# hila-chefer/Transformer-Explainability

Measured on AMD Instinct MI355X. Metric: relevance maps/sec (ViT-B/16 224^2, batch 64 per GPU, generate_LRP transformer_attribution), higher is better.
Workload: dtype f32 (3xbf16 split operands, 6 products, fp32 accumulate)

## Files before the change

### include/te_relprop.h

```cpp
#ifndef TE_RELPROP_H
#define TE_RELPROP_H

#include <stddef.h>
#include <stdint.h>

#ifdef __cplusplus
extern "C" {
#endif

typedef void* te_stream_t;
typedef uint16_t te_bf16_t;

enum {
  TE_OK = 0,
  TE_ERR_INVALID_ARG = -1,
  TE_ERR_WORKSPACE = -2,
  TE_ERR_UNSUPPORTED = -3,
  TE_ERR_NO_DEVICE = -4
};

enum { TE_VARIANT_OURS = 0, TE_VARIANT_LRP = 1, TE_IMPL_SIMPLE = 0x100 };

enum { TE_ROLLOUT_NORMALISE = 1, TE_ROLLOUT_CLS_FIXUP = 2, TE_ROLLOUT_ROW0 = 4 };

// ... 64 lines not shown
                                        const float* q, int64_t q_sb, int64_t q_sh, int64_t q_sn,
                                        const float* k, int64_t k_sb, int64_t k_sh, int64_t k_sn,
                                        const float* Z,
                                        float* cam_q, int64_t cq_sb, int64_t cq_sh, int64_t cq_sn,
                                        float* cam_k, int64_t ck_sb, int64_t ck_sh, int64_t ck_sn,
                                        int64_t B, int64_t H, int64_t N, int64_t D, float out_scale, int variant,
                                        void* ws, size_t ws_bytes, te_stream_t stream);
int te_matmul_relprop_qk_f32(const float* R_nn,
                             const float* q, int64_t q_sb, int64_t q_sh, int64_t q_sn,
                             const float* k, int64_t k_sb, int64_t k_sh, int64_t k_sn,
                             float* cam_q, int64_t cq_sb, int64_t cq_sh, int64_t cq_sn,
                             float* cam_k, int64_t ck_sb, int64_t ck_sh, int64_t ck_sn,
                             int64_t B, int64_t H, int64_t N, int64_t D, float out_scale, int variant,
                             void* ws, size_t ws_bytes, te_stream_t stream);

size_t te_add_relprop_workspace_bytes(int64_t B, int64_t n);
int te_add_relprop_f32(const float* R, const float* X0, const float* X1, float* out0, float* out1,
                       int64_t B, int64_t n, int64_t x1_batch_stride, int variant,
                       void* ws, size_t ws_bytes, te_stream_t stream);

size_t te_add_relprop_deferred_workspace_bytes(int64_t B, int64_t n);
int te_add_relprop_deferred_f32(const float* R, const float* X0, const float* X1, float* a, float* b, float* fac,
                                int64_t B, int64_t n, int64_t x1_batch_stride,
                                void* ws, size_t ws_bytes, te_stream_t stream);

size_t te_add_bcast_relprop_workspace_bytes(int64_t B, int64_t H, int64_t N);
int te_add_bcast_relprop_f32(const float* R, const float* X0, const float* mask, float* out0,
                             float* out1, int64_t B, int64_t H, int64_t N, int variant,
                             void* ws, size_t ws_bytes, te_stream_t stream);

int te_add_bcast_relprop_deferred_f32(const float* R, const float* X0, const float* mask, float* a, float* out1,
                                      float* fac, int64_t B, int64_t H, int64_t N,
                                      void* ws, size_t ws_bytes, te_stream_t stream);

int te_clone_relprop_f32(const float* R0, const float* R1, const float* R2, const float* X,
                         float* out, int64_t n, te_stream_t stream);

int te_clone_relprop_scaled_f32(const float* R0, const float* s0, int64_t s0_stride,
                                const float* R1, const float* s1, int64_t s1_stride,
                                const float* R2, const float* s2, int64_t s2_stride,
                                const float* X, float* out, int64_t B, int64_t n, te_stream_t stream);

int te_index_select_relprop_f32(const float* R, const float* X, float* out,
                                int64_t B, int64_t N, int64_t C, int64_t index, te_stream_t stream);

int te_gradcam_headmean_f32(const float* grad, const float* cam, float* out,
                            int64_t B, int64_t H, int64_t N, te_stream_t stream);

size_t te_rollout_workspace_bytes(int64_t L, int64_t B, int64_t N);
size_t te_rollout_row0_workspace_bytes(int64_t B, int64_t N);
int te_rollout_f32(const float* cams, int64_t L, int64_t start_layer, int64_t B, int64_t N,
                   int flags, float* joint, void* ws, size_t ws_bytes, te_stream_t stream);

#define TE_X6_TILE_AUTO 0
#define TE_X6_TILE_128 1
#define TE_X6_TILE_256 2
#define TE_X6_TILE_128x128 3
#define TE_X6_TEST_DROP_HANDOVER 0x200
#define TE_X6_WHOLE_TILES 0x10000
#define TE_X6_TEST_SMALL_GRID 0x4000
#define TE_X6_TILE_Z_SHIFT 10
#define TE_X6_TILE_C_SHIFT 12
#define TE_X6_PHASE_SPLIT 4
#define TE_X6_PHASE_Z 8
#define TE_X6_PHASE_C 16
#define TE_X6_PHASE_MASK 28
int te_linear_relprop_x6_supported(int64_t T, int64_t in_f, int64_t out_f);
size_t te_linear_relprop_x6_workspace_bytes(int64_t T, int64_t in_f, int64_t out_f);
size_t te_linear_x6_weight_planes_bytes(int64_t in_f, int64_t out_f);
size_t te_linear_x6_planes_bytes(int64_t rows, int64_t K);
int te_linear_x6_prepare_weights_f32(const float* W, int64_t in_f, int64_t out_f, void* planes, size_t planes_bytes,
                                     te_stream_t stream);
int te_linear_x6_split_abs_f32(const float* X, int64_t rows, int64_t K, void* planes, size_t planes_bytes,
                               te_stream_t stream);
int te_linear_relprop_x6_f32(const float* R, const float* r_scale, int64_t r_scale_stride, int64_t rows_per_sample,
                             const float* X, const float* W, const void* w_planes, const void* x_planes,
                             const float* Y, const float* bias, float* out,
                             int64_t T, int64_t in_f, int64_t out_f, int flags, unsigned* status, void* ws,
                             size_t ws_bytes, te_stream_t stream);
int te_linear_relprop_x6_check(const void* ws, int64_t T, int64_t in_f, int64_t out_f, te_stream_t stream);

int te_linear_relprop_x6_general_supported(int64_t T, int64_t in_f, int64_t out_f, int variant);
size_t te_linear_x6_weight_planes_lrp_bytes(int64_t in_f, int64_t out_f);
int te_linear_x6_prepare_weights_lrp_f32(const float* W, int64_t in_f, int64_t out_f, void* planes, size_t planes_bytes,
                                         te_stream_t stream);
size_t te_linear_relprop_x6_general_workspace_bytes(int64_t T, int64_t in_f, int64_t out_f, int variant);
int te_linear_relprop_x6_general_f32(const float* R, const float* r_scale, int64_t r_scale_stride, int64_t rows_per_sample,
                                     const float* X, const float* W, const void* w_planes, const void* w_planes_lrp,
                                     const void* x_abs_planes, const float* Y, const float* bias, float* out,
                                     int64_t T, int64_t in_f, int64_t out_f, float alpha, int variant, int flags,
                                     unsigned* status, void* ws, size_t ws_bytes, te_stream_t stream);

int te_gemm_x6_supported(int64_t T, int64_t K, int64_t M);
size_t te_gemm_x6_workspace_bytes(int64_t T, int64_t K, int64_t M);
int te_linear_x6_split_matrix_f32(const float* A, int64_t rows, int64_t K, int transposed, void* planes,
                                  size_t planes_bytes, te_stream_t stream);
int te_gemm_x6_f32(const float* X, const void* x_planes, const void* w_planes, const float* bias, float* out,
                   int64_t T, int64_t K, int64_t M, int flags, unsigned* status, void* ws, size_t ws_bytes,
                   te_stream_t stream);
int te_linear_x6_split_dual_f32(const float* A, int64_t rows, int64_t K, void* planes, void* planes_abs,
                                size_t planes_bytes, te_stream_t stream);
int te_gelu_backward_x6_planes_f32(const float* dy, const float* x, int64_t rows, int64_t K, void* planes,
                                   size_t planes_bytes, te_stream_t stream);
int te_gelu_forward_x6_planes_f32(const float* x, float* y, int64_t rows, int64_t K, void* planes, void* planes_abs,
                                  size_t planes_bytes, te_stream_t stream);

int te_attention_forward_supported(int64_t N, int64_t D);
int te_attention_forward_f32(const float* qkv, float* z_qk, float* attn, float* out,
                             int64_t B, int64_t H, int64_t N, int64_t D, float scale, te_stream_t stream);
int te_attention_forward_planes_f32(const float* qkv, float* z_qk, float* attn, float* out, void* out_planes,
                                    void* out_abs_planes, size_t planes_bytes, int64_t B, int64_t H, int64_t N, int64_t D,
                                    float scale, te_stream_t stream);
int te_attention_backward_f32(const float* d_out, const float* qkv, const float* attn, float* d_attn, float* d_qkv,
                              int64_t B, int64_t H, int64_t N, int64_t D, float scale, int need_qk, te_stream_t stream);
int te_attention_backward_out_f32(const float* d_out, const float* out, const float* qkv, const float* attn, float* d_attn,
                                  float* d_qkv, int64_t B, int64_t H, int64_t N, int64_t D, float scale, int need_qk,
                                  te_stream_t stream);

int te_attention_strided_supported(int64_t N, int64_t D);
size_t te_attention_backward_strided_workspace_bytes(int64_t B, int64_t H, int64_t N);
int te_attention_forward_strided_f32(const float* q, int64_t q_sb, int64_t q_sh, int64_t q_sn,
                                     const float* k, int64_t k_sb, int64_t k_sh, int64_t k_sn,
                                     const float* v, int64_t v_sb, int64_t v_sh, int64_t v_sn,
                                     const float* mask, float* z_qk, float* x_scaled, float* attn,
                                     float* out, int64_t o_sb, int64_t o_sh, int64_t o_sn,
                                     int64_t B, int64_t H, int64_t N, int64_t D, float scale, te_stream_t stream);
int te_attention_backward_strided_f32(const float* d_out, int64_t do_sb, int64_t do_sh, int64_t do_sn,
                                      const float* q, int64_t q_sb, int64_t q_sh, int64_t q_sn,
                                      const float* k, int64_t k_sb, int64_t k_sh, int64_t k_sn,
                                      const float* v, int64_t v_sb, int64_t v_sh, int64_t v_sn,
                                      const float* attn, float* d_attn,
                                      float* d_q, int64_t dq_sb, int64_t dq_sh, int64_t dq_sn,
                                      float* d_k, int64_t dk_sb, int64_t dk_sh, int64_t dk_sn,
                                      float* d_v, int64_t dv_sb, int64_t dv_sh, int64_t dv_sn,
                                      int64_t B, int64_t H, int64_t N, int64_t D, float scale, int need_qk,
                                      void* ws, size_t ws_bytes, te_stream_t stream);
int te_attention_backward_strided_out_f32(const float* d_out, int64_t do_sb, int64_t do_sh, int64_t do_sn,
                                          const float* out, int64_t o_sb, int64_t o_sh, int64_t o_sn,
                                          const float* q, int64_t q_sb, int64_t q_sh, int64_t q_sn,
                                          const float* k, int64_t k_sb, int64_t k_sh, int64_t k_sn,
                                          const float* v, int64_t v_sb, int64_t v_sh, int64_t v_sn,
                                          const float* attn, float* d_attn,
                                          float* d_q, int64_t dq_sb, int64_t dq_sh, int64_t dq_sn,
                                          float* d_k, int64_t dk_sb, int64_t dk_sh, int64_t dk_sn,
                                          float* d_v, int64_t dv_sb, int64_t dv_sh, int64_t dv_sn,
                                          int64_t B, int64_t H, int64_t N, int64_t D, float scale, int need_qk,
                                          void* ws, size_t ws_bytes, te_stream_t stream);

int te_layernorm_supported(int64_t C);
int te_layernorm_forward_f32(const float* x, const float* weight, const float* bias, float* y, float* mean, float* rstd,
                             int64_t T, int64_t C, float eps, te_stream_t stream);
int te_layernorm_backward_f32(const float* dy, const float* x, const float* weight, const float* mean, const float* rstd,
                              const float* add, float* dx, int64_t T, int64_t C, te_stream_t stream);
int te_gelu_forward_f32(const float* x, float* y, int64_t n, te_stream_t stream);
int te_gelu_backward_f32(const float* dy, const float* x, float* dx, int64_t n, te_stream_t stream);

int te_heatmap_f32(const float* maps, float* heat, float* fg_mask, int64_t B, int64_t g, int64_t scale,
                   int normalise, te_stream_t stream);

size_t te_seg_metrics_workspace_bytes(int64_t B, int64_t H, int64_t W);
int te_seg_metrics_f32(const float* heat, const float* fg_mask, const int64_t* labels, int64_t* counts, double* ap,
                       double* f1, int64_t B, int64_t H, int64_t W, void* ws, size_t ws_bytes, te_stream_t stream);

#define TE_RATIONALE_MAX_KS 16
#define TE_RATIONALE_CLAMP 1
size_t te_rationale_metrics_workspace_bytes(int64_t B, int64_t N, int64_t Wmax);
int te_rationale_metrics_f32(const float* scores, const int32_t* word_ids, const uint8_t* truth, float* word_scores,
                             int32_t* n_words, int32_t* order, int32_t* counts, double* soft, int64_t B, int64_t N,
                             int64_t Wmax, const int64_t* ks, int64_t n_ks, int flags, void* ws, size_t ws_bytes,
                             te_stream_t stream);

#define TE_TOKEN_ERASE_MAX_FRACTIONS 8
int te_token_erase(const int64_t* input_ids, const int64_t* attention_mask, const int32_t* word_ids,
                   const int32_t* order, const int32_t* n_words, int64_t* ids_out, int64_t* mask_out,
                   int32_t* n_rationale, int64_t B, int64_t N, int64_t Wmax, const double* fractions, int64_t n_t,
                   int64_t pad_id, te_stream_t stream);

size_t te_conv2d_zb_relprop_workspace_bytes(int64_t B, int64_t C, int64_t H, int64_t W, int64_t E, int64_t p);
int te_conv2d_zb_relprop_f32(const float* R, int64_t r_bs, const float* X, const float* W, const float* Y,
                             const float* bias, float* out, int64_t B, int64_t C, int64_t H, int64_t W_, int64_t E,
                             int64_t p, int flags, void* ws, size_t ws_bytes, te_stream_t stream);

#define TE_PERTURB_MAX_STEPS 16
#define TE_PERTURB_MAX_CHANNELS 4
size_t te_perturb_workspace_bytes(int64_t B, int64_t n_steps);
int te_perturb_f32(const float* vis, const float* data, float* out, int64_t B, int64_t C, int64_t HW,
                   const int64_t* ks, int64_t n_steps, const float* mean, const float* std_, void* ws,
                   size_t ws_bytes, te_stream_t stream);

int te_linear_relprop_bf16_supported(int64_t T, int64_t in_f, int64_t out_f);
size_t te_linear_relprop_bf16_workspace_bytes(int64_t T, int64_t in_f, int64_t out_f);
size_t te_linear_bf16_weight_planes_bytes(int64_t in_f, int64_t out_f);
int te_linear_bf16_prepare_weights(const te_bf16_t* W, int64_t in_f, int64_t out_f, void* planes, size_t planes_bytes,
                                   te_stream_t stream);
int te_linear_relprop_bf16(const float* R, int64_t r_ld, const float* r_scale, int64_t r_scale_stride,
                           int64_t rows_per_scale, const te_bf16_t* X, int64_t x_ld, const void* w_planes, float* out,
                           int64_t T, int64_t in_f, int64_t out_f, void* ws, size_t ws_bytes, te_stream_t stream);
int te_matmul_relprop_bf16_supported(int64_t N, int64_t D);
size_t te_matmul_relprop_av_bf16_workspace_bytes(int64_t B, int64_t H, int64_t N, int64_t D);
size_t te_matmul_relprop_qk_bf16_workspace_bytes(int64_t B, int64_t H, int64_t N, int64_t D);
int te_matmul_relprop_av_bf16(const float* R, int64_t r_sb, int64_t r_sh, int64_t r_sn,
                              const te_bf16_t* attn,
                              const te_bf16_t* v, int64_t v_sb, int64_t v_sh, int64_t v_sn,
                              const te_bf16_t* Z, int64_t z_sb, int64_t z_sh, int64_t z_sn,
                              float* cam_attn,
                              float* cam_v, int64_t cv_sb, int64_t cv_sh, int64_t cv_sn,
                              int64_t B, int64_t H, int64_t N, int64_t D, float out_scale, int variant,
                              void* ws, size_t ws_bytes, te_stream_t stream);
int te_matmul_relprop_qk_bf16(const float* R_nn, const float* r_scale, int64_t r_scale_stride,
                              const te_bf16_t* q, int64_t q_sb, int64_t q_sh, int64_t q_sn,
                              const te_bf16_t* k, int64_t k_sb, int64_t k_sh, int64_t k_sn,
                              const te_bf16_t* Z,
                              float* cam_q, int64_t cq_sb, int64_t cq_sh, int64_t cq_sn,
                              float* cam_k, int64_t ck_sb, int64_t ck_sh, int64_t ck_sn,
                              int64_t B, int64_t H, int64_t N, int64_t D, float out_scale, int variant,
                              void* ws, size_t ws_bytes, te_stream_t stream);
int te_add_relprop_bf16(const float* R, const te_bf16_t* X0, const te_bf16_t* X1, float* out0, float* out1, int64_t B,
                        int64_t n, int64_t x1_batch_stride, int variant, void* ws, size_t ws_bytes, te_stream_t stream);
int te_add_relprop_deferred_bf16(const float* R, const te_bf16_t* X0, const te_bf16_t* X1, float* a, float* b,
                                 float* fac, int64_t B, int64_t n, int64_t x1_batch_stride, void* ws, size_t ws_bytes,
                                 te_stream_t stream);
int te_add_bcast_relprop_bf16(const float* R, const te_bf16_t* X0, const te_bf16_t* mask, float* out0, float* out1,
                              int64_t B, int64_t H, int64_t N, int variant, void* ws, size_t ws_bytes,
                              te_stream_t stream);
int te_add_bcast_relprop_deferred_bf16(const float* R, const te_bf16_t* X0, const te_bf16_t* mask, float* a,
                                       float* out1, float* fac, int64_t B, int64_t H, int64_t N, void* ws,
                                       size_t ws_bytes, te_stream_t stream);
int te_clone_relprop_bf16(const float* R0, const float* R1, const float* R2, const te_bf16_t* X, float* out, int64_t n,
                          te_stream_t stream);
int te_clone_relprop_scaled_bf16(const float* R0, const float* s0, int64_t s0_stride, const float* R1, const float* s1,
                                 int64_t s1_stride, const float* R2, const float* s2, int64_t s2_stride,
                                 const te_bf16_t* X, float* out, int64_t B, int64_t n, te_stream_t stream);
int te_index_select_relprop_bf16(const float* R, const te_bf16_t* X, float* out, int64_t B, int64_t N, int64_t C,
                                 int64_t index, te_stream_t stream);
int te_gradcam_headmean_bf16(const te_bf16_t* grad, const float* cam, float* out, int64_t B, int64_t H, int64_t N,
                             te_stream_t stream);
enum { TE_HEADMEAN_CLAMP = 1, TE_HEADMEAN_ROW0 = 2 };
int te_attn_headmean_bf16(const te_bf16_t* attn, int64_t a_sb, int64_t a_sh, float* out, int64_t B, int64_t H, int64_t N,
                          int flags, te_stream_t stream);
int te_perturb_bf16(const float* vis, const float* data, te_bf16_t* out, int64_t B, int64_t C, int64_t HW,
                    const int64_t* ks, int64_t n_steps, const float* mean, const float* std_, void* ws,
                    size_t ws_bytes, te_stream_t stream);
int te_attention_bf16_supported(int64_t N, int64_t D);
size_t te_attention_backward_strided_bf16_workspace_bytes(int64_t B, int64_t H, int64_t N);
int te_attention_forward_strided_bf16(const te_bf16_t* q, int64_t q_sb, int64_t q_sh, int64_t q_sn,
                                      const te_bf16_t* k, int64_t k_sb, int64_t k_sh, int64_t k_sn,
                                      const te_bf16_t* v, int64_t v_sb, int64_t v_sh, int64_t v_sn,
                                      const te_bf16_t* mask, te_bf16_t* z_qk, te_bf16_t* x_scaled, te_bf16_t* attn,
                                      te_bf16_t* out, int64_t o_sb, int64_t o_sh, int64_t o_sn,
                                      int64_t B, int64_t H, int64_t N, int64_t D, float scale, te_stream_t stream);
int te_attention_backward_strided_bf16(const te_bf16_t* d_out, int64_t do_sb, int64_t do_sh, int64_t do_sn,
                                       const te_bf16_t* q, int64_t q_sb, int64_t q_sh, int64_t q_sn,
                                       const te_bf16_t* k, int64_t k_sb, int64_t k_sh, int64_t k_sn,
                                       const te_bf16_t* v, int64_t v_sb, int64_t v_sh, int64_t v_sn,
                                       const te_bf16_t* attn, te_bf16_t* d_attn,
                                       te_bf16_t* d_q, int64_t dq_sb, int64_t dq_sh, int64_t dq_sn,
                                       te_bf16_t* d_k, int64_t dk_sb, int64_t dk_sh, int64_t dk_sn,
                                       te_bf16_t* d_v, int64_t dv_sb, int64_t dv_sh, int64_t dv_sn,
                                       int64_t B, int64_t H, int64_t N, int64_t D, float scale, int need_qk,
                                       void* ws, size_t ws_bytes, te_stream_t stream);
int te_conv2d_zb_relprop_bf16_supported(int64_t C, int64_t E, int64_t p);
size_t te_conv2d_zb_relprop_bf16_workspace_bytes(int64_t B, int64_t C, int64_t H, int64_t W, int64_t E, int64_t p);
size_t te_conv2d_zb_bf16_weight_planes_bytes(int64_t C, int64_t E, int64_t p);
int te_conv2d_zb_bf16_prepare_weights(const te_bf16_t* W, int64_t C, int64_t E, int64_t p, void* planes,
                                      size_t planes_bytes, te_stream_t stream);
int te_conv2d_zb_relprop_bf16(const float* R, int64_t r_bs, const te_bf16_t* X, const te_bf16_t* W, const void* w_planes,
                              float* out, int64_t B, int64_t C, int64_t H, int64_t W_, int64_t E, int64_t p, void* ws,
                              size_t ws_bytes, te_stream_t stream);

size_t te_linear_relprop_f64_workspace_bytes(int64_t T, int64_t in_f, int64_t out_f);
int te_linear_relprop_f64(const double* R, int64_t r_ld, const double* X, int64_t x_ld, const double* W, int64_t w_ld,
                          double* out, int64_t T, int64_t in_f, int64_t out_f, void* ws, size_t ws_bytes,
                          te_stream_t stream);
size_t te_matmul_relprop_av_f64_workspace_bytes(int64_t B, int64_t H, int64_t N, int64_t D);
size_t te_matmul_relprop_qk_f64_workspace_bytes(int64_t B, int64_t H, int64_t N, int64_t D);
int te_matmul_relprop_av_f64(const double* R, int64_t r_sb, int64_t r_sh, int64_t r_sn, const double* attn,
                             const double* v, int64_t v_sb, int64_t v_sh, int64_t v_sn,
                             const double* Z, int64_t z_sb, int64_t z_sh, int64_t z_sn,
                             double* cam_attn, double* cam_v, int64_t cv_sb, int64_t cv_sh, int64_t cv_sn,
                             int64_t B, int64_t H, int64_t N, int64_t D, double out_scale,
                             void* ws, size_t ws_bytes, te_stream_t stream);
int te_matmul_relprop_qk_f64(const double* R, const double* q, int64_t q_sb, int64_t q_sh, int64_t q_sn,
                             const double* k, int64_t k_sb, int64_t k_sh, int64_t k_sn, const double* Z,
                             double* cam_q, int64_t cq_sb, int64_t cq_sh, int64_t cq_sn,
                             double* cam_k, int64_t ck_sb, int64_t ck_sh, int64_t ck_sn,
                             int64_t B, int64_t H, int64_t N, int64_t D, double out_scale,
                             void* ws, size_t ws_bytes, te_stream_t stream);
size_t te_add_relprop_f64_workspace_bytes(int64_t B, int64_t n);
int te_add_relprop_f64(const double* R, const double* X0, const double* X1, double* out0, double* out1, int64_t B,
                       int64_t n, int64_t x1_batch_stride, void* ws, size_t ws_bytes, te_stream_t stream);
size_t te_add_bcast_relprop_f64_workspace_bytes(int64_t B, int64_t H, int64_t N);
int te_add_bcast_relprop_f64(const double* R, const double* X0, const double* mask, int64_t mask_batch_stride,
                             double* out0, double* out1, int64_t B, int64_t H, int64_t N, void* ws, size_t ws_bytes,
                             te_stream_t stream);
int te_clone_relprop_f64(const double* R0, const double* R1, const double* R2, const double* X, double* out, int64_t n,
                         te_stream_t stream);
int te_index_select_relprop_f64(const double* R, const double* X, double* out, int64_t B, int64_t N, int64_t C,
                                int64_t index, te_stream_t stream);
int te_gradcam_headmean_f64(const double* grad, const double* cam, double* out, int64_t B, int64_t H, int64_t N,
                            te_stream_t stream);

#ifdef __cplusplus
}
#endif
#endif
```

### transformer-explainability_amd/_lib.py

```python
from __future__ import annotations

import ctypes
import os
from ctypes import c_char_p, c_double, c_float, c_int, c_int64, c_size_t, c_void_p

import torch

_PKG = os.path.dirname(os.path.abspath(__file__))
LIB_PATH = os.environ.get("TE_RELPROP_LIB") or os.path.join(_PKG, "lib", "libte_relprop.so")

TE_OK = 0
MIN_LIB_VERSION = 700
TE_ERR_UNSUPPORTED = -3
TE_VARIANT_OURS = 0
TE_VARIANT_LRP = 1
TE_IMPL_SIMPLE = 0x100
TE_ROLLOUT_NORMALISE = 1
TE_ROLLOUT_CLS_FIXUP = 2
TE_ROLLOUT_ROW0 = 4
TE_HEADMEAN_CLAMP = 1
TE_HEADMEAN_ROW0 = 2
TE_RATIONALE_CLAMP = 1
TE_RATIONALE_MAX_KS = 16
TE_TOKEN_ERASE_MAX_FRACTIONS = 8

_P, _I64, _F, _I, _SZ, _D = c_void_p, c_int64, c_float, c_int, c_size_t, c_double

SIGNATURES = {
    "te_version": (_I, []),
    "te_status_string": (c_char_p, [_I]),
    "te_device_check": (_I, []),
    "te_build_id": (c_char_p, []),
    "te_linear_relprop_workspace_bytes": (_SZ, [_I64, _I64, _I64, _I]),
    "te_linear_relprop_f32": (_I, [_P, _P, _P, _P, _I64, _I64, _I64, _F, _I, _P, _SZ, _P]),
    "te_linear_zpass_f32": (_I, [_P, _P, _P, _P, _I64, _I64, _I64, _P]),
    "te_linear_cpass_f32": (_I, [_P, _P, _P, _P, _I64, _I64, _I64, _P]),
    "te_linear_zpass_fwd_f32": (_I, [_P, _P, _P, _P, _P, _P, _I64, _I64, _I64, _P]),
    "te_linear_relprop_fwd_f32": (_I, [_P, _P, _P, _P, _P, _P, _I64, _I64, _I64, _P, _SZ, _P]),
    "te_linear_zpass_fwd_scaled_f32": (_I, [_P, _P, _I64, _I64, _P, _P, _P, _P, _P, _I64, _I64, _I64, _P]),
    "te_linear_relprop_fwd_scaled_f32": (_I, [_P, _P, _I64, _I64, _P, _P, _P, _P, _P, _I64, _I64, _I64, _P, _SZ, _P]),
    "te_matmul_relprop_av_workspace_bytes": (_SZ, [_I64, _I64, _I64, _I64]),
    "te_matmul_relprop_av_f32": (_I, [_P, _I64, _I64, _I64, _P, _P, _I64, _I64, _I64, _P, _P, _I64, _I64, _I64,
                                      _I64, _I64, _I64, _I64, _F, _I, _P, _SZ, _P]),
    "te_matmul_relprop_qk_workspace_bytes": (_SZ, [_I64, _I64, _I64, _I64]),
    "te_matmul_relprop_av_fwd_f32": (_I, [_P, _I64, _I64, _I64, _P, _P, _I64, _I64, _I64, _P, _P, _P, _I64, _I64, _I64,
                                          _I64, _I64, _I64, _I64, _F, _I, _P, _SZ, _P]),
    "te_matmul_relprop_av_fwdz_f32": (_I, [_P, _I64, _I64, _I64, _P, _P, _I64, _I64, _I64, _P, _I64, _I64, _I64, _P, _P,
                                           _I64, _I64, _I64, _I64, _I64, _I64, _I64, _F, _I, _P, _SZ, _P]),
    "te_attention_forward_supported": (_I, [_I64, _I64]),
    "te_attention_forward_f32": (_I, [_P, _P, _P, _P, _I64, _I64, _I64, _I64, _F, _P]),
    "te_attention_forward_planes_f32": (_I, [_P, _P, _P, _P, _P, _P, _SZ, _I64, _I64, _I64, _I64, _F, _P]),
    "te_attention_backward_f32": (_I, [_P, _P, _P, _P, _P, _I64, _I64, _I64, _I64, _F, _I, _P]),
    "te_attention_backward_out_f32": (_I, [_P, _P, _P, _P, _P, _P, _I64, _I64, _I64, _I64, _F, _I, _P]),
    "te_attention_strided_supported": (_I, [_I64, _I64]),
    "te_attention_backward_strided_workspace_bytes": (_SZ, [_I64, _I64, _I64]),
    "te_attention_forward_strided_f32": (_I, [_P, _I64, _I64, _I64, _P, _I64, _I64, _I64, _P, _I64, _I64, _I64, _P, _P, _P,
                                              _P, _P, _I64, _I64, _I64, _I64, _I64, _I64, _I64, _F, _P]),
    "te_attention_backward_strided_f32": (_I, [_P, _I64, _I64, _I64, _P, _I64, _I64, _I64, _P, _I64, _I64, _I64, _P, _I64,
                                               _I64, _I64, _P, _P, _P, _I64, _I64, _I64, _P, _I64, _I64, _I64, _P, _I64,
                                               _I64, _I64, _I64, _I64, _I64, _I64, _F, _I, _P, _SZ, _P]),
    "te_attention_backward_strided_out_f32": (_I, [_P, _I64, _I64, _I64, _P, _I64, _I64, _I64, _P, _I64, _I64, _I64, _P, _I64, _I64, _I64,
                                                   _P, _I64, _I64, _I64, _P, _P, _P, _I64, _I64, _I64, _P, _I64, _I64, _I64, _P,
                                                   _I64, _I64, _I64, _I64, _I64, _I64, _I64, _F, _I, _P, _SZ, _P]),
    "te_linear_relprop_x6_supported": (_I, [_I64, _I64, _I64]),
    "te_linear_relprop_x6_workspace_bytes": (_SZ, [_I64, _I64, _I64]),
    "te_linear_x6_weight_planes_bytes": (_SZ, [_I64, _I64]),
    "te_linear_x6_planes_bytes": (_SZ, [_I64, _I64]),
    "te_linear_x6_prepare_weights_f32": (_I, [_P, _I64, _I64, _P, _SZ, _P]),
    "te_linear_x6_split_abs_f32": (_I, [_P, _I64, _I64, _P, _SZ, _P]),
    "te_linear_relprop_x6_f32": (_I, [_P, _P, _I64, _I64, _P, _P, _P, _P, _P, _P, _P, _I64, _I64, _I64, _I, _P, _P, _SZ,
                                      _P]),
    "te_linear_relprop_x6_check": (_I, [_P, _I64, _I64, _I64, _P]),
    "te_linear_relprop_x6_general_supported": (_I, [_I64, _I64, _I64, _I]),
    "te_linear_x6_weight_planes_lrp_bytes": (_SZ, [_I64, _I64]),
    "te_linear_x6_prepare_weights_lrp_f32": (_I, [_P, _I64, _I64, _P, _SZ, _P]),
    "te_linear_relprop_x6_general_workspace_bytes": (_SZ, [_I64, _I64, _I64, _I]),
    "te_linear_relprop_x6_general_f32": (_I, [_P, _P, _I64, _I64, _P, _P, _P, _P, _P, _P, _P, _P, _I64, _I64, _I64, _F, _I,
                                              _I, _P, _P, _SZ, _P]),
    "te_gemm_x6_supported": (_I, [_I64, _I64, _I64]),
    "te_gemm_x6_workspace_bytes": (_SZ, [_I64, _I64, _I64]),
    "te_linear_x6_split_matrix_f32": (_I, [_P, _I64, _I64, _I, _P, _SZ, _P]),
    "te_linear_x6_split_dual_f32": (_I, [_P, _I64, _I64, _P, _P, _SZ, _P]),
    "te_gemm_x6_f32": (_I, [_P, _P, _P, _P, _P, _I64, _I64, _I64, _I, _P, _P, _SZ, _P]),
    "te_layernorm_supported": (_I, [_I64]),
    "te_layernorm_forward_f32": (_I, [_P, _P, _P, _P, _P, _P, _I64, _I64, _F, _P]),
    "te_layernorm_backward_f32": (_I, [_P, _P, _P, _P, _P, _P, _P, _I64, _I64, _P]),
    "te_gelu_forward_f32": (_I, [_P, _P, _I64, _P]),
    "te_gelu_backward_f32": (_I, [_P, _P, _P, _I64, _P]),
    "te_gelu_backward_x6_planes_f32": (_I, [_P, _P, _I64, _I64, _P, _SZ, _P]),
    "te_gelu_forward_x6_planes_f32": (_I, [_P, _P, _I64, _I64, _P, _P, _SZ, _P]),
    "te_matmul_relprop_qk_fwd_f32": (_I, [_P, _P, _I64, _I64, _I64, _P, _I64, _I64, _I64, _P, _P, _I64, _I64, _I64,
                                          _P, _I64, _I64, _I64, _I64, _I64, _I64, _I64, _F, _I, _P, _SZ, _P]),
    "te_matmul_relprop_qk_fwd_scaled_f32": (_I, [_P, _P, _I64, _P, _I64, _I64, _I64, _P, _I64, _I64, _I64, _P, _P, _I64,
                                                 _I64, _I64, _P, _I64, _I64, _I64, _I64, _I64, _I64, _I64, _F, _I, _P,
                                                 _SZ, _P]),
    "te_matmul_relprop_qk_f32": (_I, [_P, _P, _I64, _I64, _I64, _P, _I64, _I64, _I64, _P, _I64, _I64, _I64,
                                      _P, _I64, _I64, _I64, _I64, _I64, _I64, _I64, _F, _I, _P, _SZ, _P]),
    "te_add_relprop_workspace_bytes": (_SZ, [_I64, _I64]),
    "te_add_relprop_f32": (_I, [_P, _P, _P, _P, _P, _I64, _I64, _I64, _I, _P, _SZ, _P]),
    "te_add_relprop_deferred_workspace_bytes": (_SZ, [_I64, _I64]),
    "te_add_relprop_deferred_f32": (_I, [_P, _P, _P, _P, _P, _P, _I64, _I64, _I64, _P, _SZ, _P]),
    "te_add_bcast_relprop_workspace_bytes": (_SZ, [_I64, _I64, _I64]),
    "te_add_bcast_relprop_f32": (_I, [_P, _P, _P, _P, _P, _I64, _I64, _I64, _I, _P, _SZ, _P]),
    "te_add_bcast_relprop_deferred_f32": (_I, [_P, _P, _P, _P, _P, _P, _I64, _I64, _I64, _P, _SZ, _P]),
    "te_clone_relprop_f32": (_I, [_P, _P, _P, _P, _P, _I64, _P]),
    "te_clone_relprop_scaled_f32": (_I, [_P, _P, _I64, _P, _P, _I64, _P, _P, _I64, _P, _P, _I64, _I64, _P]),
    "te_index_select_relprop_f32": (_I, [_P, _P, _P, _I64, _I64, _I64, _I64, _P]),
    "te_gradcam_headmean_f32": (_I, [_P, _P, _P, _I64, _I64, _I64, _P]),
    "te_heatmap_f32": (_I, [_P, _P, _P, _I64, _I64, _I64, _I, _P]),
    "te_seg_metrics_workspace_bytes": (_SZ, [_I64, _I64, _I64]),
    "te_seg_metrics_f32": (_I, [_P, _P, _P, _P, _P, _P, _I64, _I64, _I64, _P, _SZ, _P]),
    "te_rationale_metrics_workspace_bytes": (_SZ, [_I64, _I64, _I64]),
    "te_rationale_metrics_f32": (_I, [_P, _P, _P, _P, _P, _P, _P, _P, _I64, _I64, _I64, _P, _I64, _I, _P, _SZ, _P]),
    "te_token_erase": (_I, [_P, _P, _P, _P, _P, _P, _P, _P, _I64, _I64, _I64, _P, _I64, _I64, _P]),
    "te_conv2d_zb_relprop_workspace_bytes": (_SZ, [_I64] * 6),
    "te_conv2d_zb_relprop_f32": (_I, [_P, _I64, _P, _P, _P, _P, _P, _I64, _I64, _I64, _I64, _I64, _I64, _I, _P, _SZ,
                                      _P]),
    "te_perturb_workspace_bytes": (_SZ, [_I64, _I64]),
    "te_perturb_f32": (_I, [_P, _P, _P, _I64, _I64, _I64, _P, _I64, _P, _P, _P, _SZ, _P]),
    "te_rollout_workspace_bytes": (_SZ, [_I64, _I64, _I64]),
    "te_rollout_row0_workspace_bytes": (_SZ, [_I64, _I64]),
    "te_rollout_f32": (_I, [_P, _I64, _I64, _I64, _I64, _I, _P, _P, _SZ, _P]),
    "te_linear_relprop_bf16_supported": (_I, [_I64, _I64, _I64]),
    "te_linear_relprop_bf16_workspace_bytes": (_SZ, [_I64, _I64, _I64]),
    "te_linear_bf16_weight_planes_bytes": (_SZ, [_I64, _I64]),
    "te_linear_bf16_prepare_weights": (_I, [_P, _I64, _I64, _P, _SZ, _P]),
    "te_linear_relprop_bf16": (_I, [_P, _I64, _P, _I64, _I64, _P, _I64, _P, _P, _I64, _I64, _I64, _P, _SZ, _P]),
    "te_matmul_relprop_bf16_supported": (_I, [_I64, _I64]),
    "te_matmul_relprop_av_bf16_workspace_bytes": (_SZ, [_I64, _I64, _I64, _I64]),
    "te_matmul_relprop_qk_bf16_workspace_bytes": (_SZ, [_I64, _I64, _I64, _I64]),
    "te_matmul_relprop_av_bf16": (_I, [_P, _I64, _I64, _I64, _P, _P, _I64, _I64, _I64, _P, _I64, _I64, _I64, _P, _P,
                                       _I64, _I64, _I64, _I64, _I64, _I64, _I64, _F, _I, _P, _SZ, _P]),
    "te_matmul_relprop_qk_bf16": (_I, [_P, _P, _I64, _P, _I64, _I64, _I64, _P, _I64, _I64, _I64, _P, _P, _I64, _I64,
                                       _I64, _P, _I64, _I64, _I64, _I64, _I64, _I64, _I64, _F, _I, _P, _SZ, _P]),
    "te_add_relprop_bf16": (_I, [_P, _P, _P, _P, _P, _I64, _I64, _I64, _I, _P, _SZ, _P]),
    "te_add_relprop_deferred_bf16": (_I, [_P, _P, _P, _P, _P, _P, _I64, _I64, _I64, _P, _SZ, _P]),
    "te_add_bcast_relprop_bf16": (_I, [_P, _P, _P, _P, _P, _I64, _I64, _I64, _I, _P, _SZ, _P]),
    "te_add_bcast_relprop_deferred_bf16": (_I, [_P, _P, _P, _P, _P, _P, _I64, _I64, _I64, _P, _SZ, _P]),
    "te_clone_relprop_bf16": (_I, [_P, _P, _P, _P, _P, _I64, _P]),
    "te_clone_relprop_scaled_bf16": (_I, [_P, _P, _I64, _P, _P, _I64, _P, _P, _I64, _P, _P, _I64, _I64, _P]),
    "te_index_select_relprop_bf16": (_I, [_P, _P, _P, _I64, _I64, _I64, _I64, _P]),
    "te_gradcam_headmean_bf16": (_I, [_P, _P, _P, _I64, _I64, _I64, _P]),
    "te_attn_headmean_bf16": (_I, [_P, _I64, _I64, _P, _I64, _I64, _I64, _I, _P]),
    "te_perturb_bf16": (_I, [_P, _P, _P, _I64, _I64, _I64, _P, _I64, _P, _P, _P, _SZ, _P]),
    "te_linear_relprop_f64_workspace_bytes": (_SZ, [_I64, _I64, _I64]),
    "te_linear_relprop_f64": (_I, [_P, _I64, _P, _I64, _P, _I64, _P, _I64, _I64, _I64, _P, _SZ, _P]),
    "te_matmul_relprop_av_f64_workspace_bytes": (_SZ, [_I64, _I64, _I64, _I64]),
    "te_matmul_relprop_qk_f64_workspace_bytes": (_SZ, [_I64, _I64, _I64, _I64]),
    "te_matmul_relprop_av_f64": (_I, [_P, _I64, _I64, _I64, _P, _P, _I64, _I64, _I64, _P, _I64, _I64, _I64, _P, _P,
                                      _I64, _I64, _I64, _I64, _I64, _I64, _I64, _D, _P, _SZ, _P]),
    "te_matmul_relprop_qk_f64": (_I, [_P, _P, _I64, _I64, _I64, _P, _I64, _I64, _I64, _P, _P, _I64, _I64, _I64, _P,
                                      _I64, _I64, _I64, _I64, _I64, _I64, _I64, _D, _P, _SZ, _P]),
    "te_add_relprop_f64_workspace_bytes": (_SZ, [_I64, _I64]),
    "te_add_relprop_f64": (_I, [_P, _P, _P, _P, _P, _I64, _I64, _I64, _P, _SZ, _P]),
    "te_add_bcast_relprop_f64_workspace_bytes": (_SZ, [_I64, _I64, _I64]),
    "te_add_bcast_relprop_f64": (_I, [_P, _P, _P, _I64, _P, _P, _I64, _I64, _I64, _P, _SZ, _P]),
    "te_clone_relprop_f64": (_I, [_P, _P, _P, _P, _P, _I64, _P]),
    "te_index_select_relprop_f64": (_I, [_P, _P, _P, _I64, _I64, _I64, _I64, _P]),
    "te_gradcam_headmean_f64": (_I, [_P, _P, _P, _I64, _I64, _I64, _P]),
    "te_conv2d_zb_relprop_bf16_supported": (_I, [_I64, _I64, _I64]),
    "te_conv2d_zb_relprop_bf16_workspace_bytes": (_SZ, [_I64] * 6),
    "te_conv2d_zb_bf16_weight_planes_bytes": (_SZ, [_I64, _I64, _I64]),
    "te_conv2d_zb_bf16_prepare_weights": (_I, [_P, _I64, _I64, _I64, _P, _SZ, _P]),
    "te_conv2d_zb_relprop_bf16": (_I, [_P, _I64, _P, _P, _P, _P, _I64, _I64, _I64, _I64, _I64, _I64, _P, _SZ, _P]),
    "te_attention_bf16_supported": (_I, [_I64, _I64]),
    "te_attention_backward_strided_bf16_workspace_bytes": (_SZ, [_I64, _I64, _I64]),
    "te_attention_forward_strided_bf16": (_I, [_P, _I64, _I64, _I64, _P, _I64, _I64, _I64, _P, _I64, _I64, _I64, _P, _P, _P,
                                               _P, _P, _I64, _I64, _I64, _I64, _I64, _I64, _I64, _F, _P]),
    "te_attention_backward_strided_bf16": (_I, [_P, _I64, _I64, _I64, _P, _I64, _I64, _I64, _P, _I64, _I64, _I64, _P, _I64,
                                                _I64, _I64, _P, _P, _P, _I64, _I64, _I64, _P, _I64, _I64, _I64, _P, _I64,
                                                _I64, _I64, _I64, _I64, _I64, _I64, _F, _I, _P, _SZ, _P]),
}


class TeError(RuntimeError):
    pass


_lib = None


def hip_runtimes_loaded():
    seen = set()
    try:
        with open("/proc/self/maps") as f:
            for line in f:
                if "libamdhip64" in line:
                    seen.add(line.split()[-1])
    except OSError:
        pass
    return sorted(seen)


def load():
    global _lib
    if _lib is not None:
        return _lib
    if not os.path.exists(LIB_PATH):
        raise TeError(
            f"{LIB_PATH} is missing: build the HIP extension first "
            f"(python transformer-explainability_amd/build.py or __graft_entry__.build()); there is no CPU fallback")
    lib = ctypes.CDLL(LIB_PATH)
    for name, (res, args) in SIGNATURES.items():
        fn = getattr(lib, name)
        fn.restype = res
        fn.argtypes = args
    if lib.te_version() < MIN_LIB_VERSION:
        raise TeError(f"{LIB_PATH} is version {lib.te_version()}, this package needs >= {MIN_LIB_VERSION}: rebuild it "
                      f"(python transformer-explainability_amd/build.py --force)")
    from ._buildid import source_hash
    bid = (lib.te_build_id() or b"").decode()
    want = source_hash()
    if bid.split("-")[0] != want and not (os.environ.get("TE_RELPROP_LIB") or os.environ.get("TE_ALLOW_STALE_LIB") == "1"):
        raise TeError(f"{LIB_PATH} was built from other sources (te_build_id() = {bid!r}, this tree hashes to {want!r}): "
                      f"rebuild it (python transformer-explainability_amd/build.py)")
    _lib = lib
    return lib


def build_id() -> str:
    return (load().te_build_id() or b"").decode()


def check(status: int, what: str):
    if status != TE_OK:
        msg = load().te_status_string(status)
        raise TeError(f"{what} failed with status {status}: {msg.decode() if msg else '?'}")


def require_device():
    if not torch.cuda.is_available():
        raise TeError("no HIP device visible to PyTorch: the relprop hot path runs only on MI355X (gfx950); "
                      "there is no CPU fallback")
    lib = load()
    rts = hip_runtimes_loaded()
    if len(rts) > 1:
        raise TeError(f"two HIP runtimes are mapped into this process: {rts}; import torch before loading "
                      f"libte_relprop so that both share torch's libamdhip64")
    check(lib.te_device_check(), "te_device_check")
# ... 1 lines not shown
```

### transformer-explainability_amd/bert.py

```python
from __future__ import annotations

import math
from types import SimpleNamespace

import torch
import torch.nn as nn

from . import ops
from . import rules as R_ours

__all__ = ["BertConfigLite", "make_bert_module", "BertModel", "BertForSequenceClassification"]


def BertConfigLite(**kw):
    d = dict(vocab_size=30522, hidden_size=768, num_hidden_layers=12, num_attention_heads=12,
             intermediate_size=3072, hidden_act="gelu", hidden_dropout_prob=0.1,
             attention_probs_dropout_prob=0.1, max_position_embeddings=512, type_vocab_size=2,
             layer_norm_eps=1e-12, pad_token_id=0, num_labels=2)
    d.update(kw)
    return SimpleNamespace(**d)


class _FusedSelfAttention(torch.autograd.Function):

    @staticmethod
    def forward(ctx, q, k, v, mask, num_heads, scale, module):
        out, attn, zqk, xsc = ops.attention_forward_qkv(q, k, v, num_heads, scale, mask=mask, want_z=True,
                                                        want_x=mask is not None)
        ctx.save_for_backward(q, k, v, attn, out)
        ctx.num_heads, ctx.scale, ctx.module = num_heads, scale, module
        if xsc is None:
            xsc = zqk.new_empty(0)
        ctx.mark_non_differentiable(attn, zqk, xsc)
        ctx.set_materialize_grads(False)
        return out, attn, zqk, xsc

    @staticmethod
    def backward(ctx, d_out, _a, _z, _x):
        q, k, v, attn, out = ctx.saved_tensors
        if d_out is None:
            return None, None, None, None, None, None, None
        stop = bool(getattr(ctx.module, "_fused_stop_backward", False))
        d_v = torch.empty_like(v)
        d_q = None if stop else torch.empty_like(q)
        d_k = None if stop else torch.empty_like(k)
        d_attn = ops.attention_backward_qkv(d_out, q, k, v, attn, ctx.num_heads, ctx.scale, d_q, d_k, d_v, need_qk=not stop, out=out)
        ctx.module.save_attn_gradients(d_attn)
        if stop:
            return None, None, None, None, None, None, None
        return d_q, d_k, d_v, None, None, None, None


def make_bert_module(L):
    ACT = {"relu": L.ReLU, "tanh": L.Tanh, "gelu": L.GELU}

    class BertEmbeddings(nn.Module):
        def __init__(self, config):
            super().__init__()
            self.word_embeddings = nn.Embedding(config.vocab_size, config.hidden_size,
                                                padding_idx=getattr(config, "pad_token_id", 0))
            self.position_embeddings = nn.Embedding(config.max_position_embeddings, config.hidden_size)
            self.token_type_embeddings = nn.Embedding(config.type_vocab_size, config.hidden_size)
            self.LayerNorm = L.LayerNorm(config.hidden_size, eps=config.layer_norm_eps)
            self.dropout = L.Dropout(config.hidden_dropout_prob)
            self.register_buffer("position_ids", torch.arange(config.max_position_embeddings).expand((1, -1)))
            self.add1 = L.Add()
            self.add2 = L.Add()

        def forward(self, input_ids=None, token_type_ids=None, position_ids=None, inputs_embeds=None):
            shape = input_ids.size() if input_ids is not None else inputs_embeds.size()[:-1]
            if position_ids is None:
                position_ids = self.position_ids[:, :shape[1]]
            if token_type_ids is None:
                token_type_ids = torch.zeros(shape, dtype=torch.long, device=self.position_ids.device)
            if inputs_embeds is None:
                inputs_embeds = self.word_embeddings(input_ids)
            pos = self.position_embeddings(position_ids).expand(shape[0], -1, -1)
            emb = self.add1([self.token_type_embeddings(token_type_ids), pos])
            emb = self.add2([emb, inputs_embeds])
            return self.dropout(self.LayerNorm(emb))

        def relprop(self, cam, **kwargs):
            return self.add2.relprop(cam, **kwargs)

    class BertSelfAttention(nn.Module):
        def __init__(self, config):
            super().__init__()
            if config.hidden_size % config.num_attention_heads != 0:
                raise ValueError("hidden size must be a multiple of the number of attention heads")
            self.num_attention_heads = config.num_attention_heads
            self.attention_head_size = config.hidden_size // config.num_attention_heads
            self.all_head_size = config.hidden_size
            self.query = L.Linear(config.hidden_size, self.all_head_size)
            self.key = L.Linear(config.hidden_size, self.all_head_size)
            self.value = L.Linear(config.hidden_size, self.all_head_size)
            self.dropout = L.Dropout(config.attention_probs_dropout_prob)
            self.matmul1 = L.MatMul()
            self.matmul2 = L.MatMul()
            self.softmax = L.Softmax(dim=-1)
            self.add = L.Add()
            self.mul = L.Mul()
            self.clone = L.Clone()
            self.head_mask = self.attention_mask = None
            self.attn_cam = self.attn = self.attn_gradients = None

        def get_attn(self): return self.attn
        def save_attn(self, attn): self.attn = attn
        def save_attn_cam(self, cam): self.attn_cam = cam
        def get_attn_cam(self): return self.attn_cam
        def save_attn_gradients(self, g): self.attn_gradients = g
        def get_attn_gradients(self): return self.attn_gradients

        def transpose_for_scores(self, x):
            return x.view(*x.shape[:-1], self.num_attention_heads, self.attention_head_size).permute(0, 2, 1, 3)

        def transpose_for_scores_relprop(self, x):
            return x.permute(0, 2, 1, 3).flatten(2)

        def forward(self, hidden_states, attention_mask=None, head_mask=None, **unused):
            if head_mask is not None:
                raise NotImplementedError("head_mask is off the accelerated path")
            self.head_mask, self.attention_mask = head_mask, attention_mask
            h1, h2, h3 = self.clone(hidden_states, 3)
            self._fused_anchor = None
            B, N, _ = hidden_states.shape
            dt = hidden_states.dtype
            if (ops.USE_FUSED_PRODUCERS and hidden_states.is_cuda and not self.training
                    and ((dt == torch.float32 and ops.attention_forward_supported(N, self.attention_head_size))
                         or (dt == torch.bfloat16 and ops.attention_forward_bf16_supported(N, self.attention_head_size)))
                    and (attention_mask is None
                         or (tuple(attention_mask.shape) == (B, 1, 1, N)
                             and (dt == torch.float32 or attention_mask.dtype == dt)))):
                return self._forward_fused(h1, h2, h3, attention_mask)
            q = self.transpose_for_scores(self.query(h1))
            k = self.transpose_for_scores(self.key(h2))
            v = self.transpose_for_scores(self.value(h3))
            scores = self.matmul1([q, k.transpose(-1, -2)]) / math.sqrt(self.attention_head_size)
            if attention_mask is not None:
                scores = self.add([scores, attention_mask])
            probs = self.softmax(scores)
            self.save_attn(probs)
            if probs.requires_grad:
                probs.register_hook(self.save_attn_gradients)
            ctx = self.matmul2([self.dropout(probs), v])
            ctx = ctx.permute(0, 2, 1, 3).contiguous()
            return (ctx.view(*ctx.shape[:-2], self.all_head_size),)

        def _forward_fused(self, h1, h2, h3, attention_mask):
            B, N, C = h1.shape
            H, D = self.num_attention_heads, self.attention_head_size
            ql, kl, vl = self.query(h1), self.key(h2), self.value(h3)
            ctx, probs, zqk, xsc = _FusedSelfAttention.apply(ql, kl, vl, attention_mask, H, 1.0 / math.sqrt(D), self)
            self._fused_anchor = ql if ql.requires_grad else None
            heads = lambda t: t.detach().view(B, N, H, D).permute(0, 2, 1, 3)
            q, k, v = heads(ql), heads(kl), heads(vl)
            self.save_attn(probs)
            caches = [(self.matmul1, [q, k.transpose(-1, -2)], zqk), (self.matmul2, [probs, v], heads(ctx))]
            if attention_mask is not None:
                caches.append((self.add, [xsc, attention_mask], None))
            for mod, X, Y in caches:
                mod.X, mod.Y = X, Y
                mod._y_version = Y._version if Y is not None else None
                mod._w_version = (None, None)
            return (ctx,)

        def relprop(self, cam, **kwargs):
            B, N, C = cam.shape
            H, D = self.num_attention_heads, self.attention_head_size
            var = self.matmul2.variant
            probs, v = self.matmul2.X
            q, kt = self.matmul1.X
            rq = torch.empty((B, N, C), dtype=cam.dtype, device=cam.device)
            rk, rv = torch.empty_like(rq), torch.empty_like(rq)
            as_heads = lambda t: t.view(B, N, H, D).permute(0, 2, 1, 3)
            cam1, _ = ops.matmul_relprop_av(as_heads(cam), probs, v, out_scale=0.5, cam_v_out=as_heads(rv), variant=var,
                                            z=R_ours._cached_y(self.matmul2))
            self.save_attn_cam(cam1)
            if getattr(self, "_stop_after_attn_cam", False):
                raise L.StopRelprop()
            if self.attention_mask is not None:
                cam1, _ = self.add.relprop(cam1, deferred=True, **kwargs)
            ops.matmul_relprop_qk(cam1, q, kt.transpose(-1, -2), out_scale=0.5, cam_q_out=as_heads(rq),
                                  cam_k_out=as_heads(rk), variant=var, z=R_ours._cached_y(self.matmul1))
            rq = self.query.relprop(rq, **kwargs)
            rk = self.key.relprop(rk, **kwargs)
            rv = self.value.relprop(rv, **kwargs)
            return self.clone.relprop((rq, rk, rv), **kwargs)

    class BertSelfOutput(nn.Module):
        def __init__(self, config):
            super().__init__()
            self.dense = L.Linear(config.hidden_size, config.hidden_size)
            self.LayerNorm = L.LayerNorm(config.hidden_size, eps=config.layer_norm_eps)
            self.dropout = L.Dropout(config.hidden_dropout_prob)
            self.add = L.Add()

        def forward(self, hidden_states, input_tensor):
            return self.LayerNorm(self.add([self.dropout(self.dense(hidden_states)), input_tensor]))

        def relprop(self, cam, **kwargs):
            cam1, cam2 = self.add.relprop(cam, deferred=True, **kwargs)
            return self.dense.relprop(cam1, **kwargs), cam2

    class BertAttention(nn.Module):
        def __init__(self, config):
            super().__init__()
            self.self = BertSelfAttention(config)
            self.output = BertSelfOutput(config)
            self.clone = L.Clone()

        def forward(self, hidden_states, attention_mask=None, head_mask=None, **unused):
            h1, h2 = self.clone(hidden_states, 2)
            return (self.output(self.self(h1, attention_mask, head_mask)[0], h2),)

        def relprop(self, cam, **kwargs):
            cam1, cam2 = self.output.relprop(cam, **kwargs)
            cam1 = self.self.relprop(cam1, **kwargs)
            return self.clone.relprop((cam1, cam2), **kwargs)

    class BertIntermediate(nn.Module):
        def __init__(self, config):
            super().__init__()
            self.dense = L.Linear(config.hidden_size, config.intermediate_size)
            act = config.hidden_act
            self.intermediate_act_fn = ACT[act]() if isinstance(act, str) else act

        def forward(self, hidden_states):
            return self.intermediate_act_fn(self.dense(hidden_states))

        def relprop(self, cam, **kwargs):
            return self.dense.relprop(cam, **kwargs)

    class BertOutput(nn.Module):
        def __init__(self, config):
            super().__init__()
            self.dense = L.Linear(config.intermediate_size, config.hidden_size)
            self.LayerNorm = L.LayerNorm(config.hidden_size, eps=config.layer_norm_eps)
            self.dropout = L.Dropout(config.hidden_dropout_prob)
            self.add = L.Add()

        def forward(self, hidden_states, input_tensor):
            return self.LayerNorm(self.add([self.dropout(self.dense(hidden_states)), input_tensor]))

        def relprop(self, cam, **kwargs):
            cam1, cam2 = self.add.relprop(cam, deferred=True, **kwargs)
            return self.dense.relprop(cam1, **kwargs), cam2

    class BertLayer(nn.Module):
        def __init__(self, config):
            super().__init__()
            self.attention = BertAttention(config)
            self.intermediate = BertIntermediate(config)
            self.output = BertOutput(config)
            self.clone = L.Clone()
            act = self.intermediate.intermediate_act_fn
            if hasattr(act, "feeds"):
                act.feeds(self.output.dense)

        def forward(self, hidden_states, attention_mask=None, head_mask=None, **unused):
            att = self.attention(hidden_states, attention_mask, head_mask)[0]
            a1, a2 = self.clone(att, 2)
            return (self.output(self.intermediate(a1), a2),)

        def relprop(self, cam, **kwargs):
            cam1, cam2 = self.output.relprop(cam, **kwargs)
            cam1 = self.intermediate.relprop(cam1, **kwargs)
            cam = self.clone.relprop((cam1, cam2), **kwargs)
            return self.attention.relprop(cam, **kwargs)

        def relprop_cls_only(self, cam_cls, **kwargs):
            alpha = kwargs.get("alpha", 1)
            var = self.clone.variant
            cls = lambda t: t[:, :1]
            dfr = ops.USE_DEFERRED_ADD
            c1, c2 = ops.add_relprop(cam_cls, cls(self.output.add.X[0]), cls(self.output.add.X[1]), variant=var,
                                     deferred=dfr)
            c1 = R_ours.linear_rule(self.output.dense, c1, alpha, cls, var)
            c1 = R_ours.linear_rule(self.intermediate.dense, c1, alpha, cls, var)
            cam = ops.clone_relprop((c1, c2), cls(self.clone.X))
            att = self.attention
            a1, a2 = ops.add_relprop(cam, cls(att.output.add.X[0]), cls(att.output.add.X[1]), variant=var, deferred=dfr)
            a1 = R_ours.linear_rule(att.output.dense, a1, alpha, cls, var)
            B, N, C = att.clone.X.shape
            dense = torch.zeros((2, B, N, C), dtype=a1.dtype, device=a1.device)
            dense[0, :, 0] = a1[:, 0]
            if isinstance(a2, ops.Deferred):
                a2 = a2.materialise()
            dense[1, :, 0] = a2[:, 0]
            cam1 = att.self.relprop(dense[0], **kwargs)
            return att.clone.relprop((cam1, dense[1]), **kwargs)

    class BertEncoder(nn.Module):
        def __init__(self, config):
            super().__init__()
            self.config = config
            self.layer = nn.ModuleList([BertLayer(config) for _ in range(config.num_hidden_layers)])

        def forward(self, hidden_states, attention_mask=None, head_mask=None, **unused):
            for i, layer in enumerate(self.layer):
                hidden_states = layer(hidden_states, attention_mask, None if head_mask is None else head_mask[i])[0]
            return (hidden_states,)

        def relprop(self, cam, **kwargs):
            for layer in reversed(self.layer):
                cam = layer.relprop(cam, **kwargs)
            return cam

    class BertPooler(nn.Module):
        def __init__(self, config):
            super().__init__()
            self.dense = L.Linear(config.hidden_size, config.hidden_size)
            self.activation = L.Tanh()
            self.pool = L.IndexSelect()
            self.register_buffer("_cls_index", torch.zeros((), dtype=torch.long), persistent=False)

        def forward(self, hidden_states):
            first = self.pool(hidden_states, 1, self._cls_index).squeeze(1)
            return self.activation(self.dense(first))

        def relprop(self, cam, **kwargs):
            cam = self.dense.relprop(cam, **kwargs)
            return self.pool.relprop(cam.unsqueeze(1), **kwargs)

    class BertModel(nn.Module):
        def __init__(self, config):
            super().__init__()
            self.config = config
            self.embeddings = BertEmbeddings(config)
            self.encoder = BertEncoder(config)
            self.pooler = BertPooler(config)

        def get_input_embeddings(self):
            return self.embeddings.word_embeddings

        def forward(self, input_ids=None, attention_mask=None, token_type_ids=None, position_ids=None,
                    head_mask=None, inputs_embeds=None, **unused):
            shape = input_ids.size() if input_ids is not None else inputs_embeds.size()[:-1]
            device = input_ids.device if input_ids is not None else inputs_embeds.device
            if attention_mask is None:
                attention_mask = torch.ones(shape, device=device)
            ext = (1.0 - attention_mask[:, None, None, :].to(next(self.parameters()).dtype)) * -10000.0
            emb = self.embeddings(input_ids=input_ids, position_ids=position_ids, token_type_ids=token_type_ids,
                                  inputs_embeds=inputs_embeds)
            seq = self.encoder(emb, attention_mask=ext, head_mask=head_mask)[0]
            return (seq, self.pooler(seq))

        exploit_cls_sparsity = True

        def relprop(self, cam, **kwargs):
            if not self.exploit_cls_sparsity:
                return self.encoder.relprop(self.pooler.relprop(cam, **kwargs), **kwargs)
            cam = self.pooler.dense.relprop(cam, **kwargs)
            cam = ops.index_select_relprop(cam.unsqueeze(1), self.pooler.pool.X[:, :1], 0)
            layers = list(self.encoder.layer)
            cam = layers[-1].relprop_cls_only(cam, **kwargs)
            for layer in reversed(layers[:-1]):
                cam = layer.relprop(cam, **kwargs)
            return cam

    class BertForSequenceClassification(nn.Module):
        def __init__(self, config):
            super().__init__()
            self.config = config
            self.num_labels = config.num_labels
            self.bert = BertModel(config)
            self.dropout = L.Dropout(config.hidden_dropout_prob)
            self.classifier = L.Linear(config.hidden_size, config.num_labels)
            self.apply(self._init_weights)

        def _init_weights(self, m):
            if isinstance(m, (nn.Linear, nn.Embedding)):
                m.weight.data.normal_(mean=0.0, std=getattr(self.config, "initializer_range", 0.02))
            elif isinstance(m, nn.LayerNorm):
                m.bias.data.zero_()
                m.weight.data.fill_(1.0)
            if isinstance(m, nn.Linear) and m.bias is not None:
                m.bias.data.zero_()

        def forward(self, input_ids=None, attention_mask=None, token_type_ids=None, position_ids=None,
                    head_mask=None, inputs_embeds=None, labels=None, **unused):
            pooled = self.bert(input_ids, attention_mask=attention_mask, token_type_ids=token_type_ids,
                               position_ids=position_ids, head_mask=head_mask, inputs_embeds=inputs_embeds)[1]
            logits = self.classifier(self.dropout(pooled))
            if labels is not None:
                if self.num_labels == 1:
                    loss = nn.functional.mse_loss(logits.view(-1), labels.view(-1))
                else:
                    loss = nn.functional.cross_entropy(logits.view(-1, self.num_labels), labels.view(-1))
                return (loss, logits)
            return (logits,)

        def relprop(self, cam=None, **kwargs):
            cam = self.classifier.relprop(cam, **kwargs)
            return self.bert.relprop(cam, **kwargs)

    return dict(BertEmbeddings=BertEmbeddings, BertSelfAttention=BertSelfAttention, BertSelfOutput=BertSelfOutput,
                BertAttention=BertAttention, BertIntermediate=BertIntermediate, BertOutput=BertOutput,
                BertLayer=BertLayer, BertEncoder=BertEncoder, BertPooler=BertPooler, BertModel=BertModel,
                BertForSequenceClassification=BertForSequenceClassification)


_ns = make_bert_module(R_ours)
BertModel = _ns["BertModel"]
BertForSequenceClassification = _ns["BertForSequenceClassification"]
```

### transformer-explainability_amd/csrc/te_linear_x6.hip

```cpp
#include <algorithm>
#include <cmath>
#include <type_traits>

#include "te_x6.h"

namespace {

constexpr int kRB = 3 * kFrag;
constexpr int kMinFrag = 4;
constexpr float kCancelTol = 0.0078125f;
constexpr int kSpinMillis = 250;
constexpr int kErrWord = 1023;


enum { MODE_Z = 0, MODE_C = 1, MODE_G = 2, MODE_ZI = 3, MODE_Z1 = 4, MODE_CI = 5, MODE_X = 6 };

__device__ __forceinline__ float bf16_f32(unsigned b) { return __uint_as_float(b << 16); }

enum { OP_ABS = 0, OP_POS = 1, OP_NEG = 2, OP_ID = 3 };
template <int OP>
__device__ __forceinline__ float apply_op(float x) {
  if constexpr (OP == OP_ID) return x;
  if constexpr (OP == OP_ABS) return __int_as_float(__float_as_int(x) & 0x7fffffff);
  const int b = __float_as_int(x);
  if constexpr (OP == OP_POS) return __int_as_float(b > 0 ? b : 0);
  return __int_as_float(b < 0 ? b : 0);
}

template <int OP, bool TRANSPOSE>
__global__ __launch_bounds__(256) void split_kernel(const float* __restrict__ src, unsigned char* __restrict__ dst,
                                                    int64_t R, int64_t K, int group, int sign,
                                                    unsigned char* __restrict__ dst_abs = nullptr) {
  const int r = threadIdx.x & 31, sl = threadIdx.x >> 5;
  const int64_t rb = blockIdx.x;
  const int64_t ks = (int64_t)blockIdx.y * 8 + sl;
  const int64_t nks = K >> 4;
  if (ks >= nks) return;
  const int64_t row = rb * 32 + r;
  float v[16];
  if (row < R) {
    if constexpr (!TRANSPOSE) {
      const float* s = src + row * K + ks * 16;
#pragma unroll
      for (int c = 0; c < 4; ++c) {
        const f32x4 q = *reinterpret_cast<const f32x4*>(s + 4 * c);
#pragma unroll
        for (int e = 0; e < 4; ++e) v[4 * c + e] = q[e];
      }
    } else {
#pragma unroll
      for (int e = 0; e < 16; ++e) v[e] = src[(ks * 16 + e) * R + row];
    }
  } else {
#pragma unroll
    for (int e = 0; e < 16; ++e) v[e] = 0.0f;
  }
  unsigned p[8][3];
#pragma unroll
  for (int e = 0; e < 8; ++e) split3_pk(apply_op<OP>(v[2 * e]), apply_op<OP>(v[2 * e + 1]), p[e]);
  unsigned char* d = dst + ((rb * nks + ks) * group + sign * 3) * kFrag + r * 16;
#pragma unroll
  for (int q = 0; q < 3; ++q)
#pragma unroll
    for (int kh = 0; kh < 2; ++kh) {
      u32x4 w;
#pragma unroll
      for (int e = 0; e < 4; ++e) w[e] = p[4 * kh + e][q];
      *reinterpret_cast<u32x4*>(d + q * kFrag + kh * 512) = w;
    }
  if constexpr (OP == OP_ID) {
    if (dst_abs) {
#pragma unroll
      for (int e = 0; e < 8; ++e) {
        const unsigned m = p[e][0] & 0x80008000u;
        p[e][0] &= 0x7fff7fffu;
        p[e][1] ^= m & (((p[e][1] & 0x7fff7fffu) + 0x7fff7fffu) & 0x80008000u);
        p[e][2] ^= m & (((p[e][2] & 0x7fff7fffu) + 0x7fff7fffu) & 0x80008000u);
      }
      unsigned char* da = dst_abs + ((rb * nks + ks) * 3) * kFrag + r * 16;
#pragma unroll
      for (int q = 0; q < 3; ++q)
#pragma unroll
        for (int kh = 0; kh < 2; ++kh) {
          u32x4 w;
#pragma unroll
          for (int e = 0; e < 4; ++e) w[e] = p[4 * kh + e][q];
          *reinterpret_cast<u32x4*>(da + q * kFrag + kh * 512) = w;
        }
    }
  }
}

enum { SRC_GELU_BWD = 0, SRC_GELU_FWD = 1 };
constexpr int kGsPitch = 132;
template <int SRC>
__global__ __launch_bounds__(256) void gelu_split_lds_kernel(const float* __restrict__ g, const float* __restrict__ x,
                                                             float* __restrict__ y, unsigned char* __restrict__ dst,
                                                             unsigned char* __restrict__ dst_abs, int64_t R, int64_t K) {
  __shared__ __attribute__((aligned(16))) float tile[32 * kGsPitch];
  const int64_t rb = blockIdx.x;
  const int64_t k0 = (int64_t)blockIdx.y * 128;
#pragma unroll
  for (int j = 0; j < 4; ++j) {
    const int i = threadIdx.x + 256 * j;
    const int tr = i >> 5, c4 = i & 31;
    const int64_t row = rb * 32 + tr, col = k0 + 4 * c4;
    f32x4 o = {0.0f, 0.0f, 0.0f, 0.0f};
    if (row < R && col < K) {
      const int64_t at = row * K + col;
      const f32x4 xv = __builtin_nontemporal_load(reinterpret_cast<const f32x4*>(x + at));
      if constexpr (SRC == SRC_GELU_BWD) {
        const f32x4 gv = __builtin_nontemporal_load(reinterpret_cast<const f32x4*>(g + at));
#pragma unroll
        for (int e = 0; e < 4; ++e) o[e] = te_gelu_grad(gv[e], xv[e]);
      } else {
#pragma unroll
        for (int e = 0; e < 4; ++e) o[e] = te_gelu(xv[e]);
        *reinterpret_cast<f32x4*>(y + at) = o;
      }
    }
    *reinterpret_cast<f32x4*>(&tile[tr * kGsPitch + 4 * c4]) = o;
  }
  __syncthreads();
  const int r = threadIdx.x & 31, sl = threadIdx.x >> 5;
  const int64_t ks = (int64_t)blockIdx.y * 8 + sl;
  const int64_t nks = K >> 4;
  if (ks >= nks) return;
  float v[16];
#pragma unroll
  for (int c = 0; c < 4; ++c) {
    const f32x4 q = *reinterpret_cast<const f32x4*>(&tile[r * kGsPitch + sl * 16 + 4 * c]);
#pragma unroll
    for (int e = 0; e < 4; ++e) v[4 * c + e] = q[e];
  }
  unsigned p[8][3];
#pragma unroll
  for (int e = 0; e < 8; ++e) split3_pk(v[2 * e], v[2 * e + 1], p[e]);
  auto store = [&](unsigned char* d) __attribute__((always_inline)) {
#pragma unroll
    for (int q = 0; q < 3; ++q)
#pragma unroll
      for (int kh = 0; kh < 2; ++kh) {
        u32x4 w;
#pragma unroll
        for (int e = 0; e < 4; ++e) w[e] = p[4 * kh + e][q];
        *reinterpret_cast<u32x4*>(d + q * kFrag + kh * 512) = w;
      }
  };
  store(dst + ((rb * nks + ks) * 3) * kFrag + r * 16);
  if constexpr (SRC == SRC_GELU_FWD) {
#pragma unroll
    for (int e = 0; e < 8; ++e) {
      const unsigned m = p[e][0] & 0x80008000u;
      p[e][0] &= 0x7fff7fffu;
      p[e][1] ^= m & (((p[e][1] & 0x7fff7fffu) + 0x7fff7fffu) & 0x80008000u);
      p[e][2] ^= m & (((p[e][2] & 0x7fff7fffu) + 0x7fff7fffu) & 0x80008000u);
    }
    store(dst_abs + ((rb * nks + ks) * 3) * kFrag + r * 16);
  }
}

__global__ __launch_bounds__(256) void zero_words_kernel(u32x4* __restrict__ p) {
  p[(size_t)blockIdx.x * 256 + threadIdx.x] = u32x4{0u, 0u, 0u, 0u};
}

__device__ __forceinline__ float exact_z(const float* __restrict__ x, const float* __restrict__ w, int64_t K) {
  float z1 = 0.0f, z2 = 0.0f;
  for (int64_t k = 0; k < K; ++k) {
    const float xv = x[k], wv = w[k];
    z1 = fmaf(fmaxf(xv, 0.0f), fmaxf(wv, 0.0f), z1);
    z2 = fmaf(fminf(xv, 0.0f), fminf(wv, 0.0f), z2);
  }
  return z1 + z2;
}

__device__ __forceinline__ float exact_zi(const float* __restrict__ x, const float* __restrict__ w, int64_t K) {
  float z1 = 0.0f, z2 = 0.0f;
  for (int64_t k = 0; k < K; ++k) {
    const float xv = x[k], wv = w[k];
    z1 = fmaf(fmaxf(xv, 0.0f), fminf(wv, 0.0f), z1);
    z2 = fmaf(fminf(xv, 0.0f), fmaxf(wv, 0.0f), z2);
  }
  return z1 + z2;
}

struct X6Params {
  const unsigned char* A;
  const unsigned char* B;
  int64_t a_group_stride;
  int64_t b_rb_stride;
  int nks;
  unsigned char pad0_[20];
  int ntm, ntn;
  int rows_w;
  int t_fast;
  int whole_tiles;
  int pad1_;
  int ncb;
  int64_t T;
  int in_f, out_f;
  float* partial;
  unsigned* flags;
  unsigned* status;
  long long spin_ticks;
  int drop_handover;
  int small_grid;
  int prefer_whole;
  const float* R;
  const float* Y;
  const float* bias;
  const float* X;
  const float* W;
  unsigned char* S;
  const float* rs;
  int64_t rs_stride;
  int rps;
  float* out;
  float scale;
  int accum;
  int x_sign;
};

#if defined(__HIP_DEVICE_COMPILE__)
#define X6_PASS4(a, b, c, d) asm volatile("" : "+v"(a), "+v"(b), "+v"(c), "+v"(d))
#else
#define X6_PASS4(a, b, c, d) (void)0
#endif

__device__ __forceinline__ void glds16(const unsigned char* src, unsigned char* lds_wave_base) {
  __builtin_amdgcn_global_load_lds((const __attribute__((address_space(1))) void*)src,
                                   (__attribute__((address_space(3))) void*)lds_wave_base, 16, 0, 0);
}

constexpr int kStages = 2;
template <int WM>
struct X6Geo {
  static constexpr int NWM = (WM == 1) ? 1 : 2, NWN = (WM == 0) ? 2 : 4, MI = (WM == 0) ? 2 : 4;
  static constexpr int NW = NWM * NWN, THREADS = 64 * NW, WPS = (WM == 0) ? 3 : 2;
  static constexpr int TM = NWM * MI * 32, TT = NWN * 64;
  static constexpr int NPA = 3 * NWM * MI, NPB = 3 * NWN * 2;
  static constexpr int ACC = MI * 2 * 16;
  static constexpr int MAX_SPX = (WM == 2) ? 32 : (WM == 1) ? 64 : 96;
};

template <int WM, int MODE>
struct X6Lds {
  using GEO = X6Geo<WM>;
  static constexpr bool STAGED = (MODE == MODE_Z || MODE == MODE_ZI || MODE == MODE_Z1) && GEO::MI == 4;
  static constexpr int STAGES = kStages * (GEO::NPA + GEO::NPB) * kFrag;
  static constexpr int MAIN = (STAGED && GEO::NW * 16384 > STAGES) ? GEO::NW * 16384 : STAGES;
  static constexpr int TOTAL = MAIN + GEO::NW * 512 + 16;
};

template <int WM, int MODE>
__global__ __launch_bounds__(X6Geo<WM>::THREADS, X6Geo<WM>::WPS) void x6_kernel(const X6Params p) {
  using GEO = X6Geo<WM>;
  constexpr int NW = GEO::NW, NWM = GEO::NWM, NWN = GEO::NWN, MI = GEO::MI;
  constexpr bool IS_Z = (MODE == MODE_Z || MODE == MODE_ZI || MODE == MODE_Z1);
  constexpr bool IS_C = (MODE == MODE_C || MODE == MODE_CI);
  constexpr int G = IS_C ? 6 : 3;
  constexpr int NPA = GEO::NPA, NPB = GEO::NPB;
  constexpr int NP = NPA + NPB;
  static_assert(NPA / 3 == NW, "each wave stages one weight-side block");
  constexpr int PBW = NPB / 3 / NW;
  constexpr int STAGE = NP * kFrag;
  constexpr int GROUPS = NPA / G;
  constexpr int LDS_MAIN = X6Lds<WM, MODE>::MAIN;
  extern __shared__ __attribute__((aligned(16))) unsigned char smem[];

  const int lane = threadIdx.x & 63;
  const int wave = __builtin_amdgcn_readfirstlane(threadIdx.x >> 6);
  const int wm = wave / NWN, wn = wave % NWN;
  const int lane16 = lane * 16;

  const int bid = blockIdx.x, spx = gridDim.x >> 3;
  const int xcd = bid & 7, slot = bid >> 3;
  const int nks = p.nks;
  const int tiles = p.ntm * p.ntn;
  const int tx0 = (int)((int64_t)tiles * xcd / 8), tx1 = (int)((int64_t)tiles * (xcd + 1) / 8);
  const int ntx = tx1 - tx0;
  const int64_t iters = (int64_t)ntx * nks;
  auto cut = [&](int s) -> int64_t {
    int64_t b = iters * s / spx;
    const int r = (int)(b % nks);
    if (p.whole_tiles) return (2 * r < nks) ? b - r : b + (nks - r);
    if (r < kMinFrag) b -= r;
    else if (nks - r < kMinFrag) b += nks - r;
    return b;
  };
  const int64_t ib = cut(slot), ie = cut(slot + 1);
  if (ib >= ie) return;
  const int f_tile = (int)(ib / nks), kb = (int)(ib - (int64_t)f_tile * nks);
  const int l_tile = (int)((ie - 1) / nks), ke = (int)(ie - (int64_t)l_tile * nks);
  const bool tail = kb > 0;
  const bool head = (ke < nks) && !(f_tile == l_tile && tail);
  const int full0 = tail ? f_tile + 1 : f_tile, full1 = (ke < nks) ? l_tile - 1 : l_tile;
  const int nseq = (head ? 1 : 0) + (full1 >= full0 ? full1 - full0 + 1 : 0) + (tail ? 1 : 0);

  float* my_part = p.partial + (size_t)bid * GEO::THREADS * GEO::ACC;
  const float* in_part = p.partial + (size_t)(bid - 8) * GEO::THREADS * GEO::ACC;

  for (int seq = 0; seq < nseq; ++seq) {
    int tile, k0, k1;
    if (head && seq == 0) {
      tile = l_tile, k0 = 0, k1 = ke;
    } else if (tail && seq == nseq - 1) {
      tile = f_tile, k0 = kb, k1 = (f_tile == l_tile) ? ke : nks;
    } else {
      tile = full0 + seq - (head ? 1 : 0), k0 = 0, k1 = nks;
    }
    tile += tx0;
// ... 1065 lines not shown
```

### transformer-explainability_amd/csrc/te_norm_act.hip

```cpp
#include "te_common.h"

namespace {

constexpr int kThreads = 256;
constexpr int kRowsPerBlock = kThreads / 64;
constexpr int kMaxChunks = 8;

__device__ __forceinline__ float wave_sum_all(float v) {
#pragma unroll
  for (int off = 32; off > 0; off >>= 1) v = v + __shfl_xor(v, off, 64);
  return v;
}

template <int NV>
__global__ __launch_bounds__(kThreads) void ln_fwd_kernel(const float* __restrict__ x, const float* __restrict__ w,
                                                          const float* __restrict__ b, float* __restrict__ y,
                                                          float* __restrict__ mean, float* __restrict__ rstd, int64_t T,
                                                          int C, float eps) {
  const int lane = threadIdx.x & 63;
  const int64_t row = (int64_t)blockIdx.x * kRowsPerBlock + (threadIdx.x >> 6);
  if (row >= T) return;
  const int nc = C >> 2;
  const float* xr = x + row * C;
  f32x4 v[NV];
  float s = 0.0f;
#pragma unroll
  for (int i = 0; i < NV; ++i) {
    const int c = lane + 64 * i;
    v[i] = f32x4{0.f, 0.f, 0.f, 0.f};
    if (c < nc) v[i] = *reinterpret_cast<const f32x4*>(xr + (c << 2));
    s = s + ((v[i][0] + v[i][1]) + (v[i][2] + v[i][3]));
  }
  const float m = wave_sum_all(s) / (float)C;
  float q = 0.0f;
#pragma unroll
  for (int i = 0; i < NV; ++i) {
    const int c = lane + 64 * i;
    if (c < nc) {
#pragma unroll
      for (int e = 0; e < 4; ++e) {
        const float d = v[i][e] - m;
        q = q + d * d;
      }
    }
  }
  const float r = 1.0f / sqrtf(wave_sum_all(q) / (float)C + eps);
  float* yr = y + row * C;
#pragma unroll
  for (int i = 0; i < NV; ++i) {
    const int c = lane + 64 * i;
    if (c < nc) {
      const f32x4 wv = *reinterpret_cast<const f32x4*>(w + (c << 2));
      const f32x4 bv = b ? *reinterpret_cast<const f32x4*>(b + (c << 2)) : f32x4{0.f, 0.f, 0.f, 0.f};
      f32x4 o;
#pragma unroll
      for (int e = 0; e < 4; ++e) o[e] = ((v[i][e] - m) * r) * wv[e] + bv[e];
      __builtin_nontemporal_store(o, reinterpret_cast<f32x4*>(yr + (c << 2)));
    }
  }
  if (lane == 0) {
    mean[row] = m;
    rstd[row] = r;
  }
}

template <int NV>
__global__ __launch_bounds__(kThreads) void ln_bwd_kernel(const float* __restrict__ dy, const float* __restrict__ x,
                                                          const float* __restrict__ w, const float* __restrict__ mean,
                                                          const float* __restrict__ rstd, const float* __restrict__ add,
                                                          float* __restrict__ dx, int64_t T, int C) {
  const int lane = threadIdx.x & 63;
  const int64_t row = (int64_t)blockIdx.x * kRowsPerBlock + (threadIdx.x >> 6);
  if (row >= T) return;
  const int nc = C >> 2;
  const float m = mean[row], r = rstd[row];
  const float* xr = x + row * C;
  const float* gr = dy + row * C;
  f32x4 a[NV], xh[NV];
  float s1 = 0.0f, s2 = 0.0f;
#pragma unroll
  for (int i = 0; i < NV; ++i) {
    const int c = lane + 64 * i;
    a[i] = f32x4{0.f, 0.f, 0.f, 0.f};
    xh[i] = f32x4{0.f, 0.f, 0.f, 0.f};
    if (c < nc) {
      const f32x4 g = __builtin_nontemporal_load(reinterpret_cast<const f32x4*>(gr + (c << 2)));
      const f32x4 xv = __builtin_nontemporal_load(reinterpret_cast<const f32x4*>(xr + (c << 2)));
      const f32x4 wv = *reinterpret_cast<const f32x4*>(w + (c << 2));
#pragma unroll
      for (int e = 0; e < 4; ++e) {
        a[i][e] = g[e] * wv[e];
        xh[i][e] = (xv[e] - m) * r;
        s1 = s1 + a[i][e];
        s2 = s2 + a[i][e] * xh[i][e];
      }
    }
  }
  const float c1 = wave_sum_all(s1) / (float)C, c2 = wave_sum_all(s2) / (float)C;
  float* dr = dx + row * C;
#pragma unroll
  for (int i = 0; i < NV; ++i) {
    const int c = lane + 64 * i;
    if (c < nc) {
      f32x4 o;
#pragma unroll
      for (int e = 0; e < 4; ++e) o[e] = r * ((a[i][e] - c1) - xh[i][e] * c2);
      if (add) {
        const f32x4 av = __builtin_nontemporal_load(reinterpret_cast<const f32x4*>(add + row * C + (c << 2)));
#pragma unroll
        for (int e = 0; e < 4; ++e) o[e] = av[e] + o[e];
      }
      __builtin_nontemporal_store(o, reinterpret_cast<f32x4*>(dr + (c << 2)));
    }
  }
}

__global__ __launch_bounds__(kThreads) void gelu_fwd_kernel(const float* __restrict__ x, float* __restrict__ y, int64_t n4) {
  const int64_t i = (int64_t)blockIdx.x * kThreads + threadIdx.x;
  if (i >= n4) return;
  const f32x4 v = __builtin_nontemporal_load(reinterpret_cast<const f32x4*>(x) + i);
  f32x4 o;
#pragma unroll
  for (int e = 0; e < 4; ++e) o[e] = te_gelu(v[e]);
  __builtin_nontemporal_store(o, reinterpret_cast<f32x4*>(y) + i);
}

__global__ __launch_bounds__(kThreads) void gelu_bwd_kernel(const float* __restrict__ dy, const float* __restrict__ x,
                                                            float* __restrict__ dx, int64_t n4) {
  const int64_t i = (int64_t)blockIdx.x * kThreads + threadIdx.x;
  if (i >= n4) return;
  const f32x4 g = __builtin_nontemporal_load(reinterpret_cast<const f32x4*>(dy) + i);
  const f32x4 v = __builtin_nontemporal_load(reinterpret_cast<const f32x4*>(x) + i);
  f32x4 o;
#pragma unroll
  for (int e = 0; e < 4; ++e) o[e] = te_gelu_grad(g[e], v[e]);
  __builtin_nontemporal_store(o, reinterpret_cast<f32x4*>(dx) + i);
}

template <typename F>
inline int for_chunks(int64_t C, F&& launch) {
  const int nv = (int)((C / 4 + 63) / 64);
  switch (nv) {
    case 1: launch(std::integral_constant<int, 1>{}); break;
    case 2: launch(std::integral_constant<int, 2>{}); break;
    case 3: launch(std::integral_constant<int, 3>{}); break;
    case 4: launch(std::integral_constant<int, 4>{}); break;
    case 5: case 6: launch(std::integral_constant<int, 6>{}); break;
    case 7: case 8: launch(std::integral_constant<int, 8>{}); break;
    default: return TE_ERR_UNSUPPORTED;
  }
  return TE_OK;
}

}

extern "C" int te_layernorm_supported(int64_t C) { return (C >= 4 && C % 4 == 0 && C <= 64 * 4 * kMaxChunks) ? 1 : 0; }

extern "C" int te_layernorm_forward_f32(const float* x, const float* weight, const float* bias, float* y, float* mean,
                                        float* rstd, int64_t T, int64_t C, float eps, te_stream_t stream_) {
  if (!x || !weight || !y || !mean || !rstd || T <= 0) return TE_ERR_INVALID_ARG;
  if (!te_layernorm_supported(C) || (T + kRowsPerBlock - 1) / kRowsPerBlock > 0x7fffffff) return TE_ERR_UNSUPPORTED;
  if (!te_aligned16(x) || !te_aligned16(weight) || !te_aligned16(y) || (bias && !te_aligned16(bias))) return TE_ERR_UNSUPPORTED;
  hipStream_t stream = (hipStream_t)stream_;
  const dim3 grid((unsigned)((T + kRowsPerBlock - 1) / kRowsPerBlock)), blk(kThreads);
  const int rc = for_chunks(C, [&](auto nv) {
    ln_fwd_kernel<decltype(nv)::value><<<grid, blk, 0, stream>>>(x, weight, bias, y, mean, rstd, T, (int)C, eps);
  });
  if (rc != TE_OK) return rc;
  TE_RETURN_IF_LAUNCH_FAILED();
  return TE_OK;
}

extern "C" int te_layernorm_backward_f32(const float* dy, const float* x, const float* weight, const float* mean,
                                         const float* rstd, const float* add, float* dx, int64_t T, int64_t C,
                                         te_stream_t stream_) {
  if (!dy || !x || !weight || !mean || !rstd || !dx || T <= 0) return TE_ERR_INVALID_ARG;
  if (!te_layernorm_supported(C) || (T + kRowsPerBlock - 1) / kRowsPerBlock > 0x7fffffff) return TE_ERR_UNSUPPORTED;
  if (!te_aligned16(dy) || !te_aligned16(x) || !te_aligned16(weight) || !te_aligned16(dx) || (add && !te_aligned16(add)))
    return TE_ERR_UNSUPPORTED;
  hipStream_t stream = (hipStream_t)stream_;
  const dim3 grid((unsigned)((T + kRowsPerBlock - 1) / kRowsPerBlock)), blk(kThreads);
  const int rc = for_chunks(C, [&](auto nv) {
    ln_bwd_kernel<decltype(nv)::value><<<grid, blk, 0, stream>>>(dy, x, weight, mean, rstd, add, dx, T, (int)C);
  });
  if (rc != TE_OK) return rc;
  TE_RETURN_IF_LAUNCH_FAILED();
  return TE_OK;
}

extern "C" int te_gelu_forward_f32(const float* x, float* y, int64_t n, te_stream_t stream_) {
  if (!x || !y || n <= 0) return TE_ERR_INVALID_ARG;
  if (n % 4 || !te_aligned16(x) || !te_aligned16(y) || n / 4 / kThreads > 0x7ffffffe) return TE_ERR_UNSUPPORTED;
  const int64_t n4 = n / 4;
  gelu_fwd_kernel<<<dim3((unsigned)((n4 + kThreads - 1) / kThreads)), dim3(kThreads), 0, (hipStream_t)stream_>>>(x, y, n4);
  TE_RETURN_IF_LAUNCH_FAILED();
  return TE_OK;
}

extern "C" int te_gelu_backward_f32(const float* dy, const float* x, float* dx, int64_t n, te_stream_t stream_) {
  if (!dy || !x || !dx || n <= 0) return TE_ERR_INVALID_ARG;
  if (n % 4 || !te_aligned16(dy) || !te_aligned16(x) || !te_aligned16(dx) || n / 4 / kThreads > 0x7ffffffe) return TE_ERR_UNSUPPORTED;
  const int64_t n4 = n / 4;
  gelu_bwd_kernel<<<dim3((unsigned)((n4 + kThreads - 1) / kThreads)), dim3(kThreads), 0, (hipStream_t)stream_>>>(dy, x, dx, n4);
  TE_RETURN_IF_LAUNCH_FAILED();
  return TE_OK;
}
```

### transformer-explainability_amd/csrc/te_x6.h

```cpp
#pragma once

#include "te_common.h"

#define TE_MFMA_BF16(a, b, c) __builtin_amdgcn_mfma_f32_32x32x16_bf16((a), (b), (c), 0, 0, 0)

constexpr int kFrag = 1024;

__device__ __forceinline__ void split3_pk(float x0, float x1, unsigned (&p)[3]) {
#pragma unroll
  for (int q = 0; q < 3; ++q) {
    const unsigned u = __builtin_bit_cast(unsigned, __builtin_convertvector(f32x2{x0, x1}, bf16x2));
    p[q] = u;
    x0 = x0 - __uint_as_float(u << 16);
    x1 = x1 - __uint_as_float(u & 0xffff0000u);
  }
}
__device__ __forceinline__ void split3(float x, unsigned (&p)[3]) {
  unsigned pk[3];
  split3_pk(x, 0.0f, pk);
#pragma unroll
  for (int q = 0; q < 3; ++q) p[q] = pk[q] & 0xffffu;
}
__device__ __forceinline__ void planes_of8(const float (&x)[8], bf16x8 (&b)[3]) {
  unsigned pk[4][3];
#pragma unroll
  for (int t2 = 0; t2 < 4; ++t2) split3_pk(x[2 * t2], x[2 * t2 + 1], pk[t2]);
#pragma unroll
  for (int q = 0; q < 3; ++q) b[q] = __builtin_bit_cast(bf16x8, u32x4{pk[0][q], pk[1][q], pk[2][q], pk[3][q]});
}

constexpr int PA[6] = {1, 0, 2, 0, 1, 0}, PB[6] = {1, 2, 0, 1, 0, 0};
__device__ __forceinline__ void mfma_x6(f32x16& acc, const bf16x8 (&a)[3], const bf16x8 (&b)[3]) {
#pragma unroll
  for (int i = 0; i < 6; ++i) acc = TE_MFMA_BF16(a[PA[i]], b[PB[i]], acc);
}

__device__ __forceinline__ f32x2 sd2(f32x2 a, f32x2 b) {
  f32x2 den = b + f32x2{1e-9f, 1e-9f};
  den[0] = (den[0] == 0.0f) ? 1e-9f : den[0];
  den[1] = (den[1] == 0.0f) ? 1e-9f : den[1];
  f32x2 rc = {__builtin_amdgcn_rcpf(den[0]), __builtin_amdgcn_rcpf(den[1])};
  const f32x2 e = __builtin_elementwise_fma(-den, rc, f32x2{1.0f, 1.0f});
  rc = __builtin_elementwise_fma(e, rc, rc);
  f32x2 q = a * rc;
  const f32x2 r = __builtin_elementwise_fma(-den, q, a);
  q = __builtin_elementwise_fma(r, rc, q);
  q[0] = (b[0] != 0.0f) ? q[0] : 0.0f;
  q[1] = (b[1] != 0.0f) ? q[1] : 0.0f;
  return q;
}

__device__ __forceinline__ f32x2 div2(f32x2 e, float s, float rcs) {
  f32x2 q = e * f32x2{rcs, rcs};
  const f32x2 r = __builtin_elementwise_fma(f32x2{-s, -s}, q, e);
  return __builtin_elementwise_fma(r, f32x2{rcs, rcs}, q);
}

__device__ __forceinline__ void swap_halves(unsigned& lo_keep, unsigned& hi_keep) {
  const u32x2 r = __builtin_amdgcn_permlane32_swap(lo_keep, hi_keep, false, false);
  lo_keep = r[0];
  hi_keep = r[1];
}
```

### transformer-explainability_amd/ops.py

```python
from __future__ import annotations

import contextlib
import os
from typing import Optional, Sequence, Tuple

import torch

from . import _lib
from ._lib import (TE_HEADMEAN_CLAMP, TE_HEADMEAN_ROW0, TE_IMPL_SIMPLE, TE_RATIONALE_CLAMP, TE_ROLLOUT_CLS_FIXUP,
                   TE_ROLLOUT_NORMALISE, TE_ROLLOUT_ROW0, TE_VARIANT_LRP, TE_VARIANT_OURS)

Tensor = torch.Tensor
_VARIANTS = {"ours": TE_VARIANT_OURS, "lrp": TE_VARIANT_LRP}

FORCE_SIMPLE = False
KERNEL_TIMER = None
_NULL = contextlib.nullcontext()


def _timed(name: str, flops: float = 0.0, nbytes: float = 0.0):
    return _NULL if KERNEL_TIMER is None else KERNEL_TIMER(name, float(flops), float(nbytes))


class Deferred:
# ... 174 lines not shown
        raise _lib.TeError("an x6 Linear kernel waited in vain for the accumulators of a tile it shares with another "
                           "workgroup (bounded stream-K hand-over expired): the affected outputs were poisoned with NaN and "
                           "every map computed since the last check is invalid.  Typical causes: several persistent x6 "
                           "launches competing for the CUs (more than one step in flight), a profiler or another process "
                           "holding CUs.  Re-run the step; set TE_LINEAR_X6=0 to use the fp32-MFMA kernels instead")


_x6_posted = {}


def x6_post(device):
    if not torch.cuda.is_available() or torch.cuda.is_current_stream_capturing():
        return
    idx = _x6_device_index(device)
    t = _x6_status.get(idx)
    if t is None:
        return
    ent = _x6_posted.get(idx)
    if ent is None:
        ent = _x6_posted[idx] = [torch.zeros(4, dtype=torch.int32).pin_memory(), torch.cuda.Event(), False]
    elif ent[2] and not ent[1].query():
        return
    with torch.cuda.device(idx):
        ent[0].copy_(t, non_blocking=True)
        ent[1].record()
    ent[2] = True


def x6_poll(device):
    if not _x6_posted or torch.cuda.is_current_stream_capturing():
        return
    ent = _x6_posted.get(_x6_device_index(device))
    if ent is None or not ent[2] or not ent[1].query():
        return
    ent[2] = False
    if int(ent[0][0]) != 0:
        x6_raise_if_failed(device)


def _weight_key(W: Tensor):
    return (W.data_ptr(), W._version, tuple(W.shape), tuple(W.stride()), str(W.device))


def x6_invalidate(obj) -> int:
    mods = obj.modules() if hasattr(obj, "modules") else [obj]
    n = 0
    for m in mods:
        c = getattr(m, "__dict__", {}).get("_te_cache")
        if c:
            c.clear()
            n += 1
    return n


def _cached_planes(W: Tensor, cache: Optional[dict], name: str, build) -> tuple:
    key = _weight_key(W)
    hit = None if cache is None else cache.get(name)
    if hit is None or hit[0] != key:
        hit = (key, *build(W.detach()))
        if cache is not None:
            cache[name] = hit
    return hit[1:]


def _prepare_planes(Wc: Tensor, bytes_fn: str, prepare_fn: str, dims: tuple, *extra) -> Tensor:
    with _on_device(Wc) as lib:
        planes = _ws(getattr(lib, bytes_fn)(*dims), Wc)
        _lib.check(getattr(lib, prepare_fn)(_ptr(Wc), *dims, *extra, _ptr(planes), planes.numel(), _stream(Wc)), prepare_fn)
    return planes


def x6_weight_planes(W: Tensor, cache: Optional[dict] = None) -> Tensor:
    out_f, in_f = W.shape
    return _cached_planes(W, cache, "x6_planes", lambda Wd: (_prepare_planes(
        _c(Wd), "te_linear_x6_weight_planes_bytes", "te_linear_x6_prepare_weights_f32", (in_f, out_f)),))[0]


X6_GEMM = {"": "all", "1": "all", "0": "off"}.get(os.environ.get("TE_X6_GEMM", "all"), os.environ.get("TE_X6_GEMM", "all"))
if X6_GEMM not in ("all", "auto", "off"):
    raise ValueError(f"TE_X6_GEMM={X6_GEMM!r}: expected all / auto / off (or 1 / 0)")


def gemm_x6_wanted(T: int, K: int, M: int) -> bool:
    if X6_GEMM == "off" or T < 256 or not gemm_x6_supported(T, K, M):
        return False
    return X6_GEMM == "all" or (K <= 1024 and M >= 2 * K)


def x6_weight_planes_lrp(W: Tensor, cache: Optional[dict] = None) -> Tensor:
    out_f, in_f = W.shape
    return _cached_planes(W, cache, "x6_planes_lrp", lambda Wd: (_prepare_planes(
        _c(Wd), "te_linear_x6_weight_planes_lrp_bytes", "te_linear_x6_prepare_weights_lrp_f32", (in_f, out_f)),))[0]


def x6_matrix_planes(W: Tensor, transposed: bool, cache: Optional[dict] = None) -> Tensor:
    out_f, in_f = W.shape
    dims = (in_f, out_f) if transposed else (out_f, in_f)
    return _cached_planes(W, cache, "x6_gemm_planes_T" if transposed else "x6_gemm_planes", lambda Wd: (_prepare_planes(
        _c(Wd), "te_linear_x6_planes_bytes", "te_linear_x6_split_matrix_f32", dims, int(transposed)),))[0]


def linear_relprop_x6_supported(T: int, in_f: int, out_f: int) -> bool:
    return bool(_lib.load().te_linear_relprop_x6_supported(int(T), int(in_f), int(out_f)))


def gemm_x6_supported(T: int, K: int, M: int) -> bool:
    return bool(_lib.load().te_gemm_x6_supported(int(T), int(K), int(M)))


X6_KEEP_ABS = os.environ.get("TE_X6_KEEP_ABS", "1") not in ("", "0")


def _x_abs_key(X: Tensor, T: int, K: int):
    return (X.data_ptr(), X._version, T, K, str(X.device))


def post_x_planes(cache: dict, X: Tensor, xs: Tensor, xa: Tensor):
    K = X.shape[-1]
    cache["x_planes_from_producer"] = (_x_abs_key(X, X.numel() // K, K), xs, xa, X)


def take_x_planes(cache: dict, X: Tensor, T: int, K: int):
    hit = cache.pop("x_planes_from_producer", None)
    if hit is not None and hit[0] == _x_abs_key(X, T, K) and hit[3].data_ptr() == X.data_ptr():
        return hit[1], hit[2]
    return None


def drop_x_planes(cache: dict, with_abs: bool = False):
    cache.pop("x_planes_from_producer", None)
    if with_abs:
        cache.pop("x_abs_planes", None)


def post_x_abs_planes(cache: dict, X: Tensor, T: int, K: int, xa: Tensor):
    cache["x_abs_planes"] = (_x_abs_key(X, T, K), xa)


def take_x_abs_planes(cache: dict, X: Tensor, T: int, K: int) -> Optional[Tensor]:
    hit = cache.pop("x_abs_planes", None)
    return hit[1] if hit is not None and hit[0] == _x_abs_key(X, T, K) else None


def post_dy_planes(cache: dict, planes: Tensor, like: Tensor) -> Tensor:
    base = torch.full((1,), float("nan"), dtype=like.dtype, device=like.device)
    cache["dy_planes_from_consumer"] = (base, tuple(like.shape), planes)
    return base.expand(like.shape)


def take_dy_planes(cache: dict, dy: Tensor) -> Optional[Tensor]:
    hit = cache.pop("dy_planes_from_consumer", None)
    if hit is not None and dy.data_ptr() == hit[0].data_ptr() and tuple(dy.shape) == hit[1] and not any(dy.stride()):
        return hit[2]
    return None


def rule_takes_abs_planes(T: int, in_f: int, out_f: int) -> bool:
    return bool(USE_LINEAR_X6 and X6_KEEP_ABS and linear_relprop_x6_supported(T, in_f, out_f))


def gemm_x6(X: Tensor, w_planes: Tensor, bias: Optional[Tensor], M: int, timer_name: str = "gemm_x6",
            keep_abs: Optional[dict] = None, x_planes: Optional[Tensor] = None) -> Tensor:
    K = X.shape[-1]
    lead = X.shape[:-1]
    T = X.numel() // K
    Xc = None if x_planes is not None else _c(X).reshape(-1, K)
    like = X if Xc is None else Xc
    out = torch.empty((T, M), dtype=torch.float32, device=X.device)
    bc = None if bias is None else _c(bias.detach())
    with _on_device(like) as lib:
        ws = _ws(lib.te_gemm_x6_workspace_bytes(T, K, M), like)
        x_bytes = (6.0 if x_planes is not None else 10.0) * T * K
        xs = x_planes
        if xs is None and keep_abs is not None:
            got = take_x_planes(keep_abs, X, T, K)
            if got is not None:
                xs, x_bytes = got[0], 6.0 * T * K
                post_x_abs_planes(keep_abs, X, T, K, got[1])
        if xs is not None and xs.numel() * xs.element_size() < lib.te_linear_x6_planes_bytes(T, K):
            raise _lib.TeError(f"gemm_x6: the operand planes handed in hold {xs.numel() * xs.element_size()} bytes, "
                               f"[{T}, {K}] needs {lib.te_linear_x6_planes_bytes(T, K)}")
        with _timed(timer_name, 12.0 * T * K * M, x_bytes + 6.0 * K * M + 4.0 * T * M):
            if xs is None and keep_abs is not None and rule_takes_abs_planes(T, K, M):
                nb = lib.te_linear_x6_planes_bytes(T, K)
                xs, xa = _ws(nb, Xc), _ws(nb, Xc)
                _lib.check(lib.te_linear_x6_split_dual_f32(_ptr(Xc), T, K, _ptr(xs), _ptr(xa), nb, _stream(Xc)),
                           "te_linear_x6_split_dual_f32")
                post_x_abs_planes(keep_abs, X, T, K, xa)
            _lib.check(lib.te_gemm_x6_f32(_ptr(Xc) if Xc is not None else None, _ptr(xs), _ptr(w_planes), _ptr(bc), _ptr(out),
                                          T, K, M, (X6_TILE | X6_FLAGS) & ~0x3c00, _ptr(x6_status(X.device)), _ptr(ws),
                                          ws.numel(), _stream(like)), "te_gemm_x6_f32")
    return out.reshape(*lead, M)


def linear_relprop(R: Tensor, X: Tensor, W: Tensor, alpha: float = 1.0, variant="ours",
                   Y: Optional[Tensor] = None, bias: Optional[Tensor] = None, cache: Optional[dict] = None) -> Tensor:
    if _any_f64(R, X, W):
        return linear_relprop_f64(R, X, W, alpha=alpha, variant=variant)
    if _is_bf16(X) or _is_bf16(W):
        return linear_relprop_bf16(R, X, W, alpha=alpha, variant=variant, cache=cache)
    out_f, in_f = W.shape
    lead = X.shape[:-1]
    R, r_scale = _split_deferred(R)
    Rc, Xc, Wc = _c(R).reshape(-1, out_f), _c(X).reshape(-1, in_f), _c(W)
    T = Xc.shape[0]
    if Rc.shape[0] != T:
        raise _lib.TeError(f"Linear.relprop: R has {Rc.shape[0]} rows, X has {T}")
    out = torch.empty((T, in_f), dtype=torch.float32, device=X.device)
    var = _variant(variant)
    fast_ok = (var == TE_VARIANT_OURS and alpha == 1 and in_f % 4 == 0 and out_f % 4 == 0 and
               all(t.data_ptr() % 16 == 0 for t in (Rc, Xc, Wc)))
    fwd = fast_ok and USE_FORWARD_OUTPUT and Y is not None
    if r_scale is not None and not fwd:
        Rc = _c(Deferred(R, r_scale).materialise()).reshape(-1, out_f)
        r_scale = None
    rs_ptr, rs_stride, rps = None, 0, 1
    if r_scale is not None:
        rs_ptr, rs_stride, rps = r_scale.data_ptr(), r_scale.stride(0), T // r_scale.shape[0]
    var_code = var & 0xff
    general = (USE_LINEAR_X6 and not (var & TE_IMPL_SIMPLE) and not (var_code == TE_VARIANT_OURS and alpha == 1)
               and all(t.data_ptr() % 16 == 0 for t in (Rc, Xc, Wc))
               and (var_code == TE_VARIANT_LRP or (USE_FORWARD_OUTPUT and Y is not None))
               and bool(_lib.load().te_linear_relprop_x6_general_supported(T, in_f, out_f, var_code)))
    if general:
        Yg = bg = None
        if var_code == TE_VARIANT_OURS:
            Yg = _c(Y.detach()).reshape(-1, out_f)
            bg = None if bias is None else _c(bias.detach())
            general = Yg.shape[0] == T and Yg.data_ptr() % 16 == 0 and (bg is None or bg.data_ptr() % 16 == 0)
    if general:
        wp = x6_weight_planes(W, cache) if var_code == TE_VARIANT_OURS else None
        wpl = x6_weight_planes_lrp(W, cache) if var_code == TE_VARIANT_LRP else None
        xa = take_x_abs_planes(cache, X, T, in_f) if cache is not None and var_code == TE_VARIANT_OURS else None
        gemm = 2.0 * T * in_f * out_f
        halves = 2 if alpha != 1 else 1
        units = (18.0 if var_code == TE_VARIANT_OURS else 24.0) * halves
        with _on_device(Xc) as lib, _timed("linear_x6_general", units * gemm,
                                           halves * (6.0 * (2 * T * in_f + 3 * in_f * out_f + 2 * T * out_f) + 16.0 * T * in_f)):
            ws = _ws(lib.te_linear_relprop_x6_general_workspace_bytes(T, in_f, out_f, var_code), Xc)
            _lib.check(lib.te_linear_relprop_x6_general_f32(_ptr(Rc), rs_ptr, rs_stride, rps, _ptr(Xc), _ptr(Wc), _ptr(wp),
                                                            _ptr(wpl), _ptr(xa), _ptr(Yg), _ptr(bg), _ptr(out), T, in_f,
                                                            out_f, float(alpha), var_code, (X6_TILE | X6_FLAGS) & ~0x3c00,
                                                            _ptr(x6_status(Xc.device)), _ptr(ws), ws.numel(), _stream(Xc)),
                       "te_linear_relprop_x6_general_f32")
            if X6_CHECK:
                x6_raise_if_failed(Xc.device)
        return out.reshape(*lead, in_f)
    if fwd:
        Yc = _c(Y.detach()).reshape(-1, out_f)
        bc = None if bias is None else _c(bias.detach())
        if Yc.shape[0] != T:
            raise _lib.TeError(f"Linear.relprop: Y has {Yc.shape[0]} rows, X has {T}")
    if (fwd and USE_LINEAR_X6 and Yc.data_ptr() % 16 == 0 and (bc is None or bc.data_ptr() % 16 == 0)
            and _lib.load().te_linear_relprop_x6_supported(T, in_f, out_f)):
        planes = x6_weight_planes(W, cache)
        xa = take_x_abs_planes(cache, X, T, in_f) if cache is not None else None
        with _on_device(Xc) as lib:
            ws = _ws(lib.te_linear_relprop_x6_workspace_bytes(T, in_f, out_f), Xc)
            status = x6_status(Xc.device)

            def call(flags):
                _lib.check(lib.te_linear_relprop_x6_f32(_ptr(Rc), rs_ptr, rs_stride, rps, _ptr(Xc), _ptr(Wc), _ptr(planes),
                                                        _ptr(xa), _ptr(Yc), _ptr(bc), _ptr(out), T, in_f, out_f,
                                                        X6_TILE | X6_FLAGS | flags, _ptr(status), _ptr(ws), ws.numel(),
                                                        _stream(Xc)),
                           "te_linear_relprop_x6_f32")
            if KERNEL_TIMER is None:
                call(0)
            else:
                gemm = 2.0 * T * in_f * out_f
                if xa is None:
                    with _timed("linear_x6_split", 0.0, 10.0 * T * in_f):
                        call(TE_X6_PHASE_SPLIT)
                else:
                    call(TE_X6_PHASE_SPLIT)
                with _timed("linear_x6_zpass", 6.0 * gemm, 6.0 * (T * in_f + in_f * out_f + T * out_f) + 8.0 * T * out_f):
                    call(TE_X6_PHASE_Z)
                with _timed("linear_x6_cpass", 12.0 * gemm, 6.0 * (T * out_f + 2 * in_f * out_f) + 8.0 * T * in_f):
                    call(TE_X6_PHASE_C)
            if X6_CHECK:
                rc = lib.te_linear_relprop_x6_check(_ptr(ws), T, in_f, out_f, _stream(Xc))
                if rc != 0:
                    status.zero_()
                    raise _lib.TeError(f"te_linear_relprop_x6_f32({T},{in_f},{out_f}): a workgroup waited in vain for the "
                                       f"accumulators of a shared tile (status {rc}); the result is invalid")
                x6_raise_if_failed(Xc.device)
        return out.reshape(*lead, in_f)
    if KERNEL_TIMER is not None and fast_ok:
        with _on_device(Xc) as lib:
            S = torch.empty((T, out_f), dtype=torch.float32, device=X.device)
            st = _stream(Xc)
            if fwd:
                with _timed("linear_zpass_fwd", 2.0 * T * in_f * out_f, 4.0 * (T * in_f + 3 * T * out_f + in_f * out_f)):
                    _lib.check(lib.te_linear_zpass_fwd_scaled_f32(_ptr(Rc), rs_ptr, rs_stride, rps, _ptr(Xc), _ptr(Wc),
                                                                  _ptr(Yc), _ptr(bc), _ptr(S), T, in_f, out_f, st),
                               "te_linear_zpass_fwd_scaled_f32")
            else:
                with _timed("linear_zpass", 2.0 * T * (2 * in_f) * out_f, 4.0 * (T * in_f + 2 * T * out_f + in_f * out_f)):
                    _lib.check(lib.te_linear_zpass_f32(_ptr(Rc), _ptr(Xc), _ptr(Wc), _ptr(S), T, in_f, out_f, st),
                               "te_linear_zpass_f32")
            with _timed("linear_cpass", 2.0 * T * (2 * in_f) * out_f, 4.0 * (T * out_f + 2 * T * in_f + in_f * out_f)):
                _lib.check(lib.te_linear_cpass_f32(_ptr(S), _ptr(Xc), _ptr(Wc), _ptr(out), T, in_f, out_f, st),
                           "te_linear_cpass_f32")
        return out.reshape(*lead, in_f)
    with _on_device(Xc) as lib:
        ws = _ws(lib.te_linear_relprop_workspace_bytes(T, in_f, out_f, var), Xc)
# ... 166 lines not shown
    d_attn = torch.empty_like(attn)
    hd = lambda t: (None, 0, 0, 0) if t is None else _heads(_prep_bf16(t), H)
    (q, qb, qh, qn), (k, kb, kh, kn), (v, vb, vh, vn) = hd(q), hd(k), hd(v)
    (dq, dqb, dqh, dqn), (dk, dkb, dkh, dkn), (dv, dvb, dvh, dvn) = hd(d_q), hd(d_k), hd(d_v)
    with _on_device(d_out) as lib, _timed("attention_backward", (8.0 if need_qk else 4.0) * B * H * N * N * D,
                                          2.0 * B * ((5 if need_qk else 2) * H * N * N + 8 * N * C)):
        ws = _ws(lib.te_attention_backward_strided_bf16_workspace_bytes(B, H, N), d_out)
        _lib.check(lib.te_attention_backward_strided_bf16(_ptr(d_out), N * C, 64, C, _ptr(q), qb, qh, qn, _ptr(k), kb, kh, kn,
                                                          _ptr(v), vb, vh, vn, _ptr(attn), _ptr(d_attn), _ptr(dq), dqb, dqh,
                                                          dqn, _ptr(dk), dkb, dkh, dkn, _ptr(dv), dvb, dvh, dvn, B, H, N, D,
                                                          float(scale), int(bool(need_qk)), _ptr(ws), ws.numel(),
                                                          _stream(d_out)), "te_attention_backward_strided_bf16")
    return d_attn


def attention_backward_qkv(d_out: Tensor, q: Tensor, k: Tensor, v: Tensor, attn: Tensor, num_heads: int, scale: float,
                           d_q: Optional[Tensor], d_k: Optional[Tensor], d_v: Tensor, need_qk: bool = True,
                           out: Optional[Tensor] = None) -> Tensor:
    if any(_is_bf16(t) for t in (d_out, q, k, v, attn)):
        return attention_backward_qkv_bf16(d_out, q, k, v, attn, num_heads, scale, d_q, d_k, d_v, need_qk=need_qk)
    B, N, C = d_out.shape
    H, D = num_heads, C // num_heads
    d_out, attn = _c(d_out), _c(attn)
    d_attn = torch.empty_like(attn)
    hd = lambda t: (None, 0, 0, 0) if t is None else _heads(_prep(t), H)
    (q, qb, qh, qn), (k, kb, kh, kn), (v, vb, vh, vn) = hd(q), hd(k), hd(v)
    (dq, dqb, dqh, dqn), (dk, dkb, dkh, dkn), (dv, dvb, dvh, dvn) = hd(d_q), hd(d_k), hd(d_v)
    with _on_device(d_out) as lib, _timed("attention_backward", (8.0 if need_qk else 4.0) * B * H * N * N * D,
                                          4.0 * B * ((4 if need_qk else 2) * H * N * N + 8 * N * C)):
        ws = _ws(lib.te_attention_backward_strided_workspace_bytes(B, H, N), d_out)
        if out is not None and tuple(out.shape) == (B, N, C) and out.dtype == d_out.dtype and out.stride(-1) == 1:
            (o, ob, oh, on) = _heads(_prep(out), H)
            _lib.check(lib.te_attention_backward_strided_out_f32(_ptr(d_out), N * C, 64, C, _ptr(o), ob, oh, on, _ptr(q), qb, qh, qn,
                                                                 _ptr(k), kb, kh, kn, _ptr(v), vb, vh, vn, _ptr(attn), _ptr(d_attn),
                                                                 _ptr(dq), dqb, dqh, dqn, _ptr(dk), dkb, dkh, dkn, _ptr(dv), dvb, dvh,
                                                                 dvn, B, H, N, D, float(scale), int(bool(need_qk)), _ptr(ws),
                                                                 ws.numel(), _stream(d_out)), "te_attention_backward_strided_out_f32")
            return d_attn
        _lib.check(lib.te_attention_backward_strided_f32(_ptr(d_out), N * C, 64, C, _ptr(q), qb, qh, qn, _ptr(k), kb, kh, kn,
                                                         _ptr(v), vb, vh, vn, _ptr(attn), _ptr(d_attn), _ptr(dq), dqb, dqh,
                                                         dqn, _ptr(dk), dkb, dkh, dkn, _ptr(dv), dvb, dvh, dvn, B, H, N, D,
                                                         float(scale), int(bool(need_qk)), _ptr(ws), ws.numel(),
                                                         _stream(d_out)), "te_attention_backward_strided_f32")
    return d_attn


def attention_forward_planes_supported(qkv: Tensor, num_heads: int) -> bool:
    B, N, C3 = qkv.shape
    C = C3 // 3
    return (qkv.is_cuda and qkv.dtype == torch.float32 and C % num_heads == 0 and C // num_heads == 64 and N <= 224
            and bool(_lib.load().te_attention_forward_supported(N, 64)))


def attention_forward(qkv: Tensor, num_heads: int, scale: float, planes: bool = False):
    if _is_bf16(qkv):
        if planes:
            raise _lib.TeError("attention_forward(planes=True): operand planes are emitted from float32 activations only")
        qkv = _c16(qkv)
        C = qkv.shape[-1] // 3
        out, attn, zqk, _ = attention_forward_qkv_bf16(qkv[..., :C], qkv[..., C:2 * C], qkv[..., 2 * C:], num_heads, scale)
        return out, attn, zqk
    qkv = _c(qkv)
    B, N, C3 = qkv.shape
    C = C3 // 3
    H, D = num_heads, C // num_heads
    if not _lib.load().te_attention_forward_supported(N, D):
        if planes:
            raise _lib.TeError("attention_forward(planes=True): shape not served by te_attention_forward_planes_f32")
        out, attn, zqk, _ = attention_forward_qkv(qkv[..., :C], qkv[..., C:2 * C], qkv[..., 2 * C:], num_heads, scale)
        return out, attn, zqk
    out = torch.empty((B, N, C), dtype=torch.float32, device=qkv.device)
    attn = torch.empty((B, H, N, N), dtype=torch.float32, device=qkv.device)
    zqk = torch.empty((B, H, N, N), dtype=torch.float32, device=qkv.device)
    extra = 12.0 * B * N * C if planes else 0.0
    with _on_device(qkv) as lib, _timed("attention_forward", 4.0 * B * H * N * N * D, 4.0 * B * (2 * H * N * N + 4 * N * C) + extra):
        if planes:
            nb = lib.te_linear_x6_planes_bytes(B * N, C)
            xs, xa = _ws(nb, qkv), _ws(nb, qkv)
            _lib.check(lib.te_attention_forward_planes_f32(_ptr(qkv), _ptr(zqk), _ptr(attn), _ptr(out), _ptr(xs), _ptr(xa), nb,
                                                           B, H, N, D, float(scale), _stream(qkv)),
                       "te_attention_forward_planes_f32")
            return out, attn, zqk, xs, xa
        _lib.check(lib.te_attention_forward_f32(_ptr(qkv), _ptr(zqk), _ptr(attn), _ptr(out), B, H, N, D, float(scale),
                                                _stream(qkv)), "te_attention_forward_f32")
    return out, attn, zqk


def attention_backward(d_out: Tensor, qkv: Tensor, attn: Tensor, num_heads: int, scale: float,
                       need_qk: bool = True, out: Optional[Tensor] = None) -> Tuple[Tensor, Optional[Tensor]]:
    if _is_bf16(d_out) or _is_bf16(qkv) or _is_bf16(attn):
        qkv = _c16(qkv)
        C = qkv.shape[-1] // 3
        d_qkv = torch.empty_like(qkv)
        th = lambda t, i: t[..., i * C:(i + 1) * C]
        d_attn = attention_backward_qkv_bf16(d_out, th(qkv, 0), th(qkv, 1), th(qkv, 2), attn, num_heads, scale,
                                             th(d_qkv, 0), th(d_qkv, 1), th(d_qkv, 2), need_qk=need_qk)
        return d_attn, d_qkv
    d_out, qkv, attn = _c(d_out), _c(qkv), _c(attn)
    B, N, C3 = qkv.shape
    C = C3 // 3
    H, D = num_heads, C // num_heads
    d_qkv = torch.empty_like(qkv)
    if not _lib.load().te_attention_forward_supported(N, D):
        th = lambda t, i: t[..., i * C:(i + 1) * C]
        d_attn = attention_backward_qkv(d_out, th(qkv, 0), th(qkv, 1), th(qkv, 2), attn, num_heads, scale,
                                        th(d_qkv, 0), th(d_qkv, 1), th(d_qkv, 2), need_qk=need_qk, out=out)
        return d_attn, d_qkv
    d_attn = torch.empty_like(attn)
    with _on_device(qkv) as lib, _timed("attention_backward", (8.0 if need_qk else 4.0) * B * H * N * N * D,
                                        4.0 * B * ((4 if need_qk else 2) * H * N * N + 8 * N * C)):
        if out is not None and need_qk and tuple(out.shape) == tuple(d_out.shape) and out.is_contiguous() and out.dtype == d_out.dtype:
            _lib.check(lib.te_attention_backward_out_f32(_ptr(d_out), _ptr(out), _ptr(qkv), _ptr(attn), _ptr(d_attn), _ptr(d_qkv),
                                                         B, H, N, D, float(scale), 1, _stream(qkv)),
                       "te_attention_backward_out_f32")
        else:
            _lib.check(lib.te_attention_backward_f32(_ptr(d_out), _ptr(qkv), _ptr(attn), _ptr(d_attn), _ptr(d_qkv), B, H, N,
                                                     D, float(scale), int(bool(need_qk)), _stream(qkv)),
                       "te_attention_backward_f32")
    return d_attn, d_qkv


def layernorm_supported(x: Tensor) -> bool:
    return (x.is_cuda and x.dtype == torch.float32 and x.dim() >= 2
            and bool(_lib.load().te_layernorm_supported(int(x.shape[-1]))))


def layernorm_forward(x: Tensor, weight: Tensor, bias: Optional[Tensor], eps: float) -> Tuple[Tensor, Tensor, Tensor]:
    x = _c(x)
    C = x.shape[-1]
    T = x.numel() // C
    y = torch.empty_like(x)
    mean = torch.empty((T,), dtype=torch.float32, device=x.device)
    rstd = torch.empty((T,), dtype=torch.float32, device=x.device)
    with _on_device(x) as lib, _timed("layernorm_forward", 0.0, 4.0 * 2 * T * C):
        _lib.check(lib.te_layernorm_forward_f32(_ptr(x), _ptr(_c(weight)), _ptr(_c(bias)) if bias is not None else None,
                                                _ptr(y), _ptr(mean), _ptr(rstd), T, C, float(eps), _stream(x)),
                   "te_layernorm_forward_f32")
    return y, mean, rstd


def layernorm_backward(dy: Tensor, x: Tensor, weight: Tensor, mean: Tensor, rstd: Tensor,
                       add: Optional[Tensor] = None) -> Tensor:
    dy, x = _c(dy), _c(x)
    C = x.shape[-1]
    T = x.numel() // C
    dx = torch.empty_like(x)
    with _on_device(x) as lib, _timed("layernorm_backward", 0.0, 4.0 * (3 + (add is not None)) * T * C):
        _lib.check(lib.te_layernorm_backward_f32(_ptr(dy), _ptr(x), _ptr(_c(weight)), _ptr(mean), _ptr(rstd),
                                                 _ptr(_c(add)) if add is not None else None, _ptr(dx), T, C, _stream(x)),
                   "te_layernorm_backward_f32")
    return dx


def gelu_forward(x: Tensor) -> Tensor:
    x = _c(x)
    y = torch.empty_like(x)
    with _on_device(x) as lib, _timed("gelu_forward", 0.0, 4.0 * 2 * x.numel()):
        _lib.check(lib.te_gelu_forward_f32(_ptr(x), _ptr(y), x.numel(), _stream(x)), "te_gelu_forward_f32")
    return y


X6_FUSE_GELU = os.environ.get("TE_X6_FUSE_GELU", "1") not in ("", "0")


_GELU_BWD_HANDOFF = 0


class gelu_backward_plane_handoff:

    def __enter__(self):
        global _GELU_BWD_HANDOFF
        _GELU_BWD_HANDOFF += 1
        return self

    def __exit__(self, *exc):
        global _GELU_BWD_HANDOFF
        _GELU_BWD_HANDOFF -= 1


def gelu_backward_handoff_active() -> bool:
    return _GELU_BWD_HANDOFF > 0


def gelu_planes_supported(x: Tensor) -> bool:
    return bool(X6_FUSE_GELU and x.dim() >= 2 and x.shape[-1] >= 16 and x.shape[-1] % 16 == 0)


def gelu_forward_planes(x: Tensor):
    x = _c(x)
    K = x.shape[-1]
    T = x.numel() // K
    y = torch.empty_like(x)
    with _on_device(x) as lib, _timed("gelu_forward", 0.0, (4.0 * 2 + 12.0) * x.numel()):
        nb = lib.te_linear_x6_planes_bytes(T, K)
        xs, xa = _ws(nb, x), _ws(nb, x)
        _lib.check(lib.te_gelu_forward_x6_planes_f32(_ptr(x), _ptr(y), T, K, _ptr(xs), _ptr(xa), nb, _stream(x)),
                   "te_gelu_forward_x6_planes_f32")
    return y, xs, xa


def gelu_backward_planes(dy: Tensor, x: Tensor) -> Tensor:
    dy, x = _c(dy), _c(x)
    K = x.shape[-1]
    T = x.numel() // K
    with _on_device(x) as lib, _timed("gelu_backward", 0.0, (4.0 * 2 + 6.0) * x.numel()):
        nb = lib.te_linear_x6_planes_bytes(T, K)
        planes = _ws(nb, x)
        _lib.check(lib.te_gelu_backward_x6_planes_f32(_ptr(dy), _ptr(x), T, K, _ptr(planes), nb, _stream(x)),
                   "te_gelu_backward_x6_planes_f32")
    return planes


def gelu_backward(dy: Tensor, x: Tensor) -> Tensor:
    dy, x = _c(dy), _c(x)
    dx = torch.empty_like(x)
    with _on_device(x) as lib, _timed("gelu_backward", 0.0, 4.0 * 3 * x.numel()):
        _lib.check(lib.te_gelu_backward_f32(_ptr(dy), _ptr(x), _ptr(dx), x.numel(), _stream(x)), "te_gelu_backward_f32")
    return dx


USE_DEFERRED_ADD = True


def _is_bcast_mask(X0: Tensor, X1: Tensor) -> bool:
    return X1.dim() == 4 and X0.dim() == 4 and X1.shape[1] == 1 and X1.shape[2] == 1 and X0.shape[1] * X0.shape[2] != 1


def add_relprop(R: Tensor, X0: Tensor, X1: Tensor, variant="ours", deferred: bool = False):
    if _any_f64(R, X0, X1):
        return add_relprop_f64(R, X0, X1, variant, deferred)
    if _is_bf16(X0) or _is_bf16(X1):
        return add_relprop_bf16(R, X0, X1, variant, deferred)
    B = X0.shape[0]
    R, X0 = _c(R), _c(X0)
    n = X0[0].numel()
    if _is_bcast_mask(X0, X1):
        H, N = X0.shape[1], X0.shape[3]
        mask = _c(X1).reshape(X1.shape[0], N)
        if mask.shape[0] == 1 and B > 1:
            mask = mask.expand(B, N).contiguous()
        out0 = torch.empty_like(X0)
        out1 = torch.empty((B, 1, 1, N), dtype=torch.float32, device=X0.device)
        if deferred and _variant(variant) == TE_VARIANT_OURS:
            fac = torch.empty((B, 2), dtype=torch.float32, device=X0.device)
            with _on_device(X0) as lib, _timed("add_bcast_mask_deferred", 0.0, 4.0 * B * (3 * H * N * N + 2 * N)):
                ws = _ws(lib.te_add_bcast_relprop_workspace_bytes(B, H, N), X0)
                _lib.check(lib.te_add_bcast_relprop_deferred_f32(_ptr(R), _ptr(X0), _ptr(mask), _ptr(out0), _ptr(out1),
                                                                 _ptr(fac), B, H, N, _ptr(ws), ws.numel(), _stream(X0)),
                           "te_add_bcast_relprop_deferred_f32")
            return Deferred(out0, fac[:, 0]), out1
        with _on_device(X0) as lib, _timed("add_bcast_mask", 0.0, 4.0 * B * (3 * H * N * N + 2 * N)):
            ws = _ws(lib.te_add_bcast_relprop_workspace_bytes(B, H, N), X0)
            _lib.check(lib.te_add_bcast_relprop_f32(_ptr(R), _ptr(X0), _ptr(mask), _ptr(out0), _ptr(out1), B, H, N,
                                                    _variant(variant), _ptr(ws), ws.numel(), _stream(X0)),
                       "te_add_bcast_relprop_f32")
        return out0, out1
    X1 = _c(X1)
    if X1.shape == X0.shape:
        x1_bs = n
    elif X1.shape[0] == 1 and X1.shape[1:] == X0.shape[1:]:
        x1_bs = 0
    else:
        raise _lib.TeError(f"Add.relprop: unsupported operand shapes {tuple(X0.shape)} + {tuple(X1.shape)}")
    out0, out1 = torch.empty_like(X0), torch.empty_like(X0)
    var = _variant(variant)
    x1_elems = n if x1_bs else n / B
    if deferred and var == TE_VARIANT_OURS:
        fac = torch.empty((B, 2), dtype=torch.float32, device=X0.device)
        with _on_device(X0) as lib, _timed("add_deferred", 0.0, 4.0 * B * (4 * n + x1_elems)):
            ws = _ws(lib.te_add_relprop_deferred_workspace_bytes(B, n), X0)
            _lib.check(lib.te_add_relprop_deferred_f32(_ptr(R), _ptr(X0), _ptr(X1), _ptr(out0), _ptr(out1), _ptr(fac), B,
                                                       n, x1_bs, _ptr(ws), ws.numel(), _stream(X0)),
                       "te_add_relprop_deferred_f32")
        return Deferred(out0, fac[:, 0]), Deferred(out1, fac[:, 1])
    with _on_device(X0) as lib, _timed("add", 0.0, 4.0 * B * (4 * n + x1_elems)):
        ws = _ws(lib.te_add_relprop_workspace_bytes(B, n), X0)
        _lib.check(lib.te_add_relprop_f32(_ptr(R), _ptr(X0), _ptr(X1), _ptr(out0), _ptr(out1), B, n, x1_bs,
                                          var, _ptr(ws), ws.numel(), _stream(X0)), "te_add_relprop_f32")
    return out0, out1


def clone_relprop(Rs: Sequence, X: Tensor) -> Tensor:
    if len(Rs) not in (2, 3):
        raise _lib.TeError(f"Clone.relprop supports 2 or 3 aliases, got {len(Rs)}")
    if _any_f64(X, *Rs):
        return clone_relprop_f64(Rs, X)
    bf = _is_bf16(X)
    X = _c16(X) if bf else _c(X)
    sfx = "bf16" if bf else "f32"
    pairs = [_split_deferred(r) for r in Rs]
    Rs = [_c(r) for r, _ in pairs]
    scales = [sc for _, sc in pairs]
    for r in Rs:
        if r.numel() != X.numel():
            raise _lib.TeError("Clone.relprop: relevance / input size mismatch")
    out = torch.empty(X.shape, dtype=torch.float32, device=X.device)
    nb = 4.0 * X.numel() * (len(Rs) + 1) + X.element_size() * X.numel()
    if any(sc is not None for sc in scales):
        B = X.shape[0]
        sp = [(None, 0) if sc is None else (sc.data_ptr(), sc.stride(0)) for sc in scales] + [(None, 0)]
        with _on_device(X) as lib, _timed("clone", 0.0, nb):
            _lib.check(getattr(lib, "te_clone_relprop_scaled_" + sfx)(
                _ptr(Rs[0]), sp[0][0], sp[0][1], _ptr(Rs[1]), sp[1][0], sp[1][1], _ptr(Rs[2]) if len(Rs) == 3 else None,
                sp[2][0], sp[2][1], _ptr(X), _ptr(out), B, X.numel() // B, _stream(X)), "te_clone_relprop_scaled_" + sfx)
        return out
    with _on_device(X) as lib, _timed("clone", 0.0, nb):
# ... 675 lines not shown
```

### transformer-explainability_amd/producers.py

```python
from __future__ import annotations

import torch

from . import ops


def usable(x: torch.Tensor) -> bool:
    return ops.USE_FUSED_PRODUCERS and torch.is_tensor(x) and ops.layernorm_supported(x)


def gelu_usable(x: torch.Tensor) -> bool:
    return (ops.USE_FUSED_PRODUCERS and torch.is_tensor(x) and x.is_cuda and x.dtype == torch.float32
            and x.numel() > 0 and x.numel() % 4 == 0)


def norm_usable(x: torch.Tensor, norm) -> bool:
    return (usable(x) and not norm.training and getattr(norm, "weight", None) is not None
            and tuple(norm.normalized_shape) == (x.shape[-1],))


class _LayerNorm(torch.autograd.Function):
    @staticmethod
    def forward(ctx, x, weight, bias, eps):
        y, mean, rstd = ops.layernorm_forward(x, weight, bias, eps)
        ctx.save_for_backward(x, weight, mean, rstd)
        return y

    @staticmethod
    def backward(ctx, dy):
        x, weight, mean, rstd = ctx.saved_tensors
        return ops.layernorm_backward(dy, x, weight, mean, rstd), None, None, None


class _ResidualLayerNorm(torch.autograd.Function):

    @staticmethod
    def forward(ctx, x, weight, bias, eps):
        y, mean, rstd = ops.layernorm_forward(x, weight, bias, eps)
        ctx.save_for_backward(x, weight, mean, rstd)
        return x.view_as(x), y

    @staticmethod
    def backward(ctx, d_bypass, dy):
        x, weight, mean, rstd = ctx.saved_tensors
        if dy is None:
            return d_bypass, None, None, None
        return ops.layernorm_backward(dy, x, weight, mean, rstd, add=d_bypass), None, None, None


class _Gelu(torch.autograd.Function):

    @staticmethod
    def forward(ctx, x, feeds, source):
        ctx.save_for_backward(x)
        ctx.source = source
        if feeds is not None:
            y, xs, xa = ops.gelu_forward_planes(x)
            ops.post_x_planes(feeds, y, xs, xa)
            return y
        return ops.gelu_forward(x)

    @staticmethod
    def backward(ctx, dy):
        (x,) = ctx.saved_tensors
        if ctx.source is not None:
            return ops.post_dy_planes(ctx.source, ops.gelu_backward_planes(dy, x), x), None, None
        return ops.gelu_backward(dy, x), None, None


class _Linear(torch.autograd.Function):

    @staticmethod
    def forward(ctx, x, weight, bias, cache, fwd_x6, bwd_x6):
        ctx.weight, ctx.cache, ctx.bwd_x6 = weight, cache, bwd_x6
        if fwd_x6:
            return ops.gemm_x6(x, ops.x6_matrix_planes(weight, False, cache), bias, weight.shape[0], "linear_forward_x6",
                               keep_abs=cache)
        return torch.nn.functional.linear(x, weight, bias)

    @staticmethod
    def backward(ctx, dy):
        w = ctx.weight
        if ctx.bwd_x6:
            dx = ops.gemm_x6(dy, ops.x6_matrix_planes(w, True, ctx.cache), None, w.shape[1], "linear_backward_x6",
                             x_planes=ops.take_dy_planes(ctx.cache, dy))
        else:
            dx = torch.matmul(dy, w)
        return dx, None, None, None, None, None


def linear_plan(x: torch.Tensor, lin):
    if not (ops.USE_FUSED_PRODUCERS and ops.X6_GEMM != "off" and torch.is_tensor(x) and x.is_cuda
            and x.dtype == torch.float32 and not lin.training and x.dim() >= 2):
        return False, False
    out_f, in_f = lin.weight.shape
    T = x.numel() // in_f
    return ops.gemm_x6_wanted(T, in_f, out_f), ops.gemm_x6_wanted(T, out_f, in_f)


def takes_producer_planes(lin, T: int, K: int) -> bool:
    out_f, in_f = lin.weight.shape
    return bool(K == in_f and ops.USE_FUSED_PRODUCERS and ops.X6_GEMM != "off" and not lin.training
                and ops.gemm_x6_wanted(T, in_f, out_f) and ops.rule_takes_abs_planes(T, in_f, out_f))


def _d(t):
    return None if t is None else t.detach()


def linear(x, lin, cache, plan):
    out = _Linear.apply(x, _d(lin.weight), _d(lin.bias), cache, plan[0], plan[1])
    if plan[1]:
        out._te_bwd_x6_cache = cache
    return out


def layer_norm(x, norm):
    return _LayerNorm.apply(x, _d(norm.weight), _d(norm.bias), norm.eps)


def residual_layer_norm(x, norm):
    return _ResidualLayerNorm.apply(x, _d(norm.weight), _d(norm.bias), norm.eps)


def gelu(x, consumer=None, consumer_cache=None):
    feeds = source = None
    if ops.gelu_planes_supported(x):
        K = x.shape[-1]
        if consumer is not None and takes_producer_planes(consumer, x.numel() // K, K):
            feeds = consumer_cache
        if ops.gelu_backward_handoff_active():
            source = getattr(x, "_te_bwd_x6_cache", None)
    if feeds is None and consumer_cache is not None:
        ops.drop_x_planes(consumer_cache)
    return _Gelu.apply(x, feeds, source)
```

### transformer-explainability_amd/rules.py

```python
from __future__ import annotations

import torch
import torch.nn as nn

from . import ops

__all__ = ['forward_hook', 'Clone', 'Add', 'Cat', 'ReLU', 'GELU', 'Dropout', 'BatchNorm2d', 'Linear', 'MaxPool2d',
           'AdaptiveAvgPool2d', 'AvgPool2d', 'Conv2d', 'Sequential', 'safe_divide', 'einsum', 'Softmax',
           'IndexSelect', 'LayerNorm', 'AddEye', 'Tanh', 'MatMul', 'Mul']


def safe_divide(a, b):
    den = b.clamp(min=1e-9) + b.clamp(max=1e-9)
    den = den + den.eq(0).type(den.type()) * 1e-9
    return a / den * b.ne(0).type(b.type())


def forward_hook(self, input, output):
    if type(input[0]) in (list, tuple):
        self.X = [i.detach() for i in input[0]]
    else:
        self.X = input[0].detach()
    self.Y = output
    self._y_version = output._version if torch.is_tensor(output) else None
    w = getattr(self, "weight", None)
    b = getattr(self, "bias", None)
    self._w_version = (w._version if torch.is_tensor(w) else None, b._version if torch.is_tensor(b) else None)


class StopRelprop(Exception):
    """Raised by an attention module whose ``_stop_after_attn_cam`` flag is set, right after it stored its attn_cam:
    the model-level relprop loop catches it (extension: ``prune_below_start_layer``, see vit.VisionTransformer)."""


def _cached_y(module):
    y = getattr(module, "Y", None)
    if not torch.is_tensor(y) or getattr(module, "_y_version", None) != y._version:
        return None
    w = getattr(module, "weight", None)
    b = getattr(module, "bias", None)
    now = (w._version if torch.is_tensor(w) else None, b._version if torch.is_tensor(b) else None)
    if getattr(module, "_w_version", now) != now:
        return None
    return y


class RelProp(nn.Module):
    variant = "ours"

    def __init__(self):
        super(RelProp, self).__init__()
        self.register_forward_hook(forward_hook)

    def relprop(self, R, alpha):
        return R


class _Identity(RelProp):
    """Rules that pass relevance through unchanged (layers_ours.py:67-80,86-87) need no cached input."""


def _no_cache_hook(self, input, output):
    self.Y = output


class ReLU(nn.ReLU, RelProp):
    pass


class GELU(nn.GELU, RelProp):
    def feeds(self, linear):
        self.__dict__["_te_feeds"] = (linear,)
        return self

    def forward(self, x):
        from . import producers
        if getattr(self, "approximate", "none") == "none" and not self.training and producers.gelu_usable(x):
            nxt = self.__dict__.get("_te_feeds", (None,))[0]
            return producers.gelu(x, nxt, x6_cache(nxt) if isinstance(nxt, Linear) else None)
        return super().forward(x)


class Softmax(nn.Softmax, RelProp):
    pass


class LayerNorm(nn.LayerNorm, RelProp):
    def forward(self, x):
        from . import producers
        if producers.norm_usable(x, self):
            return producers.layer_norm(x, self)
        return super().forward(x)


class Dropout(nn.Dropout, RelProp):
    pass


class Tanh(nn.Tanh, RelProp):
    pass


def x6_cache(module) -> dict:
    c = module.__dict__.get("_te_cache")
    if c is None:
        c = module.__dict__["_te_cache"] = {}
    return c


class _ScratchCache:

    def __getstate__(self):
        state = self.__dict__.copy()
        state.pop("_te_cache", None)
        return state

    def _load_from_state_dict(self, *args, **kwargs):
        super()._load_from_state_dict(*args, **kwargs)
        ops.x6_invalidate(self)

    def _apply(self, fn, *args, **kwargs):
        ops.x6_invalidate(self)
        return super()._apply(fn, *args, **kwargs)


class Linear(_ScratchCache, nn.Linear, RelProp):

    def forward(self, x):
        from . import producers
        plan = producers.linear_plan(x, self)
        if not plan[0]:
            ops.drop_x_planes(x6_cache(self), with_abs=True)
        if plan[0] or plan[1]:
            return producers.linear(x, self, x6_cache(self), plan)
        return super().forward(x)

    def relprop(self, R, alpha):
        return linear_rule(self, R, alpha)


def linear_rule(m, R, alpha, rows=None, variant=None):
    X, Y = m.X, _cached_y(m)
    if Y is not None and Y.shape[:-1] != X.shape[:-1]:
        Y = None
    if rows is not None:
        X, Y = rows(X), None if Y is None else rows(Y)
    return ops.linear_relprop(R, X, m.weight.detach(), alpha=alpha, variant=variant or m.variant, Y=Y, bias=m.bias,
                              cache=x6_cache(m))


class Add(RelProp):

    def forward(self, inputs):
        return torch.add(*inputs)

    def relprop(self, R, alpha, deferred=False):
        x0, x1 = self.X
        bcast_mask = x0.dim() == 4 and x1.dim() == 4 and x1.shape[1] == 1 and x1.shape[2] == 1
        a, b = ops.add_relprop(R, x0, x1, variant=self.variant,
                               deferred=deferred and ops.USE_DEFERRED_ADD and (x0.shape == x1.shape or bcast_mask))
        return [a, b]


class einsum(RelProp):

    def __init__(self, equation):
        super().__init__()
        self.equation = equation

    def forward(self, *operands):
        ops_ = operands[0] if (len(operands) == 1 and isinstance(operands[0], (list, tuple))) else operands
        eq = self.equation.replace(" ", "")
        if eq == 'bhid,bhjd->bhij' and len(ops_) == 2:
            return torch.matmul(ops_[0], ops_[1].transpose(-1, -2))
        if eq == 'bhij,bhjd->bhid' and len(ops_) == 2:
            return torch.matmul(ops_[0], ops_[1])
        return torch.einsum(self.equation, *operands)

    def relprop(self, R, alpha):
        eq = self.equation.replace(" ", "")
        if eq == 'bhij,bhjd->bhid':
            cam_attn, cam_v = ops.matmul_relprop_av(R, self.X[0], self.X[1], variant=self.variant, z=_cached_y(self))
            return [cam_attn, cam_v]
        if eq == 'bhid,bhjd->bhij':
            cam_q, cam_k = ops.matmul_relprop_qk(R, self.X[0], self.X[1], variant=self.variant, z=_cached_y(self))
            return [cam_q, cam_k]
        raise NotImplementedError(f"einsum.relprop: equation {self.equation!r} is not on the accelerated path")


class MatMul(RelProp):

    def forward(self, inputs):
        return torch.matmul(*inputs)

    def relprop(self, R, alpha):
        x0, x1 = self.X
        if x0.dim() != 4 or x1.dim() != 4:
            raise NotImplementedError("MatMul.relprop: only [B,H,.,.] attention products are accelerated")
        if x1.stride(-1) != 1 and x1.stride(-2) == 1:
            k = x1.transpose(-1, -2)
            cam_q, cam_k = ops.matmul_relprop_qk(R, x0, k, variant=self.variant, z=_cached_y(self))
            return [cam_q, cam_k.transpose(-1, -2)]
        if x0.shape[-1] == x0.shape[-2] == x1.shape[-2]:
            cam_attn, cam_v = ops.matmul_relprop_av(R, x0, x1, variant=self.variant, z=_cached_y(self))
            return [cam_attn, cam_v]
        if x0.shape[-1] == x1.shape[-2]:
            k = x1.transpose(-1, -2).contiguous()
            cam_q, cam_k = ops.matmul_relprop_qk(R, x0, k, variant=self.variant, z=_cached_y(self))
            return [cam_q, cam_k.transpose(-1, -2)]
        raise NotImplementedError("MatMul.relprop: operand shapes are not an attention product")


class Clone(RelProp):

    def forward(self, input, num):
        self.__setattr__('num', num)
        return [input for _ in range(num)]

    def relprop(self, R, alpha):
        return ops.clone_relprop(list(R), self.X)


class IndexSelect(RelProp):

    def forward(self, inputs, dim, indices):
        self.__setattr__('dim', dim)
        self.__setattr__('indices', indices)
        if not torch.is_tensor(indices):
            self._index_host = int(indices)
        elif indices.numel() == 1 and (not indices.is_cuda or getattr(self, "_index_src", None) is not indices
                                       or getattr(self, "_index_version", None) != indices._version):
            if not (indices.is_cuda and torch.cuda.is_current_stream_capturing()):
                self._index_host = int(indices)
                self._index_src = indices
                self._index_version = indices._version
        return torch.index_select(inputs, dim, indices.reshape(-1) if torch.is_tensor(indices) else indices)

    def relprop(self, R, alpha):
        idx = self.indices
        if self.dim != 1 or self.X.dim() != 3 or (torch.is_tensor(idx) and idx.numel() != 1):
# ... 65 lines not shown
```

### transformer-explainability_amd/vit.py

```python
from __future__ import annotations

import torch
import torch.nn as nn

from . import ops, producers
from . import rules as R_ours

__all__ = ["VisionTransformer", "vit_base_patch16_224", "vit_large_patch16_224", "deit_base_patch16_224",
           "compute_rollout_attention", "make_vit_module"]


def compute_rollout_attention(all_layer_matrices, start_layer=0):
    return ops.rollout(torch.stack(list(all_layer_matrices), 0), start_layer=start_layer, normalise=False)


def _trunc_normal_(t, std=.02):
    with torch.no_grad():
        return nn.init.trunc_normal_(t, mean=0., std=std, a=-2., b=2.)


class _SplitQKV(torch.autograd.Function):

    @staticmethod
    def forward(ctx, qkv, num_heads):
# ... 45 lines not shown
        return (None if stop else d_qkv), None, None, None, None


PRETRAINED_URLS = {
    "vit_base_patch16_224": "https://github.com/rwightman/pytorch-image-models/releases/download/v0.1-vitjx/"
                            "jx_vit_base_p16_224-80ecf9dd.pth",
    "vit_large_patch16_224": "https://github.com/rwightman/pytorch-image-models/releases/download/v0.1-vitjx/"
                             "jx_vit_large_p16_224-4ee7a4dc.pth",
    "deit_base_patch16_224": "https://dl.fbaipublicfiles.com/deit/deit_base_patch16_224-b5f2ef4d.pth",
}


def load_pretrained_weights(model, url, patch_size=16, key=None):
    import os
    name = os.path.basename(url)
    try:
        state = torch.hub.load_state_dict_from_url(url, map_location="cpu", progress=False)
    except Exception as exc:
        where = os.path.join(torch.hub.get_dir(), "checkpoints", name)
        raise RuntimeError(f"pretrained=True: {name} is not in the torch hub cache and could not be downloaded "
                           f"({type(exc).__name__}: {exc}); place the checkpoint at {where}") from exc
    if key is not None:
        state = state[key]
    state = dict(state)
    w = state.get("patch_embed.proj.weight")
    if w is not None and w.dim() == 2:
        state["patch_embed.proj.weight"] = w.reshape(w.shape[0], 3, patch_size, patch_size)
    strict = True
    if "head.weight" in state and state["head.weight"].shape[0] != model.head.weight.shape[0]:
        del state["head.weight"], state["head.bias"]
        strict = False
    model.load_state_dict(state, strict=strict)
    return model


def make_vit_module(L):

    class Mlp(nn.Module):
        def __init__(self, in_features, hidden_features=None, out_features=None, drop=0.):
            super().__init__()
            out_features = out_features or in_features
            hidden_features = hidden_features or in_features
            self.fc1 = L.Linear(in_features, hidden_features)
            self.act = L.GELU()
            self.fc2 = L.Linear(hidden_features, out_features)
            self.drop = L.Dropout(drop)
            if hasattr(self.act, "feeds"):
                self.act.feeds(self.fc2)

        def forward(self, x):
            return self.drop(self.fc2(self.drop(self.act(self.fc1(x)))))

        def relprop(self, cam, **kwargs):
            cam = self.fc2.relprop(cam, **kwargs)
            return self.fc1.relprop(cam, **kwargs)

    class Attention(nn.Module):
        def __init__(self, dim, num_heads=8, qkv_bias=False, attn_drop=0., proj_drop=0.):
            super().__init__()
            self.num_heads = num_heads
            self.scale = (dim // num_heads) ** -0.5
            self.matmul1 = L.einsum('bhid,bhjd->bhij')
            self.matmul2 = L.einsum('bhij,bhjd->bhid')
            self.qkv = L.Linear(dim, dim * 3, bias=qkv_bias)
            self.attn_drop = L.Dropout(attn_drop)
            self.proj = L.Linear(dim, dim)
            self.proj_drop = L.Dropout(proj_drop)
            self.softmax = L.Softmax(dim=-1)
            self.attn_cam = self.attn = self.v = self.v_cam = self.attn_gradients = None

        def get_attn(self): return self.attn
        def save_attn(self, attn): self.attn = attn
        def get_attention_map(self): return self.attn
        def save_attention_map(self, attn): self.attn = attn
        def save_attn_cam(self, cam): self.attn_cam = cam
        def get_attn_cam(self): return self.attn_cam
        def get_v(self): return self.v
        def save_v(self, v): self.v = v
        def save_v_cam(self, cam): self.v_cam = cam
        def get_v_cam(self): return self.v_cam
        def save_attn_gradients(self, g): self.attn_gradients = g
        def get_attn_gradients(self): return self.attn_gradients

        def forward(self, x):
            B, N, C = x.shape
            H = self.num_heads
            self._fused_anchor = None
            if ops.USE_FUSED_PRODUCERS and x.is_cuda and not self.training and (
                    (x.dtype == torch.float32 and ops.attention_forward_supported(N, C // H))
                    or (x.dtype == torch.bfloat16 and ops.attention_forward_bf16_supported(N, C // H))):
                return self._forward_fused(x)
            q, k, v = split_qkv(self.qkv(x), H)
            self.save_v(v)
            attn = self.attn_drop(self.softmax(self.matmul1([q, k]) * self.scale))
            self.save_attn(attn)
            if attn.requires_grad:
                attn.register_hook(self.save_attn_gradients)
            out = self.matmul2([attn, v]).permute(0, 2, 1, 3).reshape(B, N, C)
            return self.proj_drop(self.proj(out))

        def _forward_fused(self, x):
            B, N, C = x.shape
            H, D = self.num_heads, C // self.num_heads
            qkv = self.qkv(x)
            feeds = None
            if (isinstance(self.proj, L.Linear) and ops.attention_forward_planes_supported(qkv, H)
                    and producers.takes_producer_planes(self.proj, B * N, C)):
                feeds = R_ours.x6_cache(self.proj)
            out, attn, zqk = _FusedAttention.apply(qkv, H, self.scale, self, feeds)
            self._fused_anchor = qkv if qkv.requires_grad else None
            q, k, v = qkv.detach().view(B, N, 3, H, D).permute(2, 0, 3, 1, 4)
            self.save_v(v)
            self.save_attn(attn)
            zav = out.detach().view(B, N, H, D).permute(0, 2, 1, 3)
            for mod, X, Y in ((self.matmul1, [q, k], zqk), (self.matmul2, [attn, v], zav)):
                mod.X, mod.Y = X, Y
                mod._y_version, mod._w_version = Y._version, (None, None)
            return self.proj_drop(self.proj(out))

        def relprop(self, cam, **kwargs):
            return self.relprop_after_proj(self.proj.relprop(cam, **kwargs), **kwargs)

        def relprop_after_proj(self, cam, **kwargs):
            B, N, C = cam.shape
            H = self.num_heads
            D = C // H
            r_heads = cam.view(B, N, H, D).permute(0, 2, 1, 3)
            attn, v = self.matmul2.X
            q, k = self.matmul1.X
            cam_qkv = torch.empty((B, N, 3 * C), dtype=cam.dtype, device=cam.device)
            slots = cam_qkv.view(B, N, 3, H, D).permute(2, 0, 3, 1, 4)
            var = self.matmul2.variant
            cam1, cam_v = ops.matmul_relprop_av(r_heads, attn, v, out_scale=0.5, cam_v_out=slots[2], variant=var,
                                                z=R_ours._cached_y(self.matmul2))
            self.save_v_cam(cam_v)
            self.save_attn_cam(cam1)
            if getattr(self, "_stop_after_attn_cam", False):
                raise L.StopRelprop()
            ops.matmul_relprop_qk(cam1, q, k, out_scale=0.5, cam_q_out=slots[0], cam_k_out=slots[1], variant=var,
                                  z=R_ours._cached_y(self.matmul1))
            return self.qkv.relprop(cam_qkv, **kwargs)

    class Block(nn.Module):
        def __init__(self, dim, num_heads, mlp_ratio=4., qkv_bias=False, drop=0., attn_drop=0., norm_eps=1e-6):
            super().__init__()
            self.norm1 = L.LayerNorm(dim, eps=norm_eps)
            self.attn = Attention(dim, num_heads=num_heads, qkv_bias=qkv_bias, attn_drop=attn_drop, proj_drop=drop)
            self.norm2 = L.LayerNorm(dim, eps=norm_eps)
            self.mlp = Mlp(in_features=dim, hidden_features=int(dim * mlp_ratio), drop=drop)
            self.add1 = L.Add()
            self.add2 = L.Add()
            self.clone1 = L.Clone()
            self.clone2 = L.Clone()

        def forward(self, x):
            x1, n = self._clone_norm(self.clone1, self.norm1, x)
            x = self.add1([x1, self.attn(n)])
            x1, n = self._clone_norm(self.clone2, self.norm2, x)
            return self.add2([x1, self.mlp(n)])

        @staticmethod
        def _clone_norm(clone, norm, x):
            if producers.norm_usable(x, norm):
                x1, n = producers.residual_layer_norm(x, norm)
                clone.X, clone.num = x.detach(), 2
                norm.X, norm.Y = clone.X, n
                return x1, n
            x1, x2 = clone(x, 2)
            return x1, norm(x2)

        def relprop(self, cam, **kwargs):
            cam1, cam2 = self.add2.relprop(cam, deferred=True, **kwargs)
            cam2 = self.mlp.relprop(cam2, **kwargs)
            cam = self.clone2.relprop((cam1, cam2), **kwargs)
            cam1, cam2 = self.add1.relprop(cam, deferred=True, **kwargs)
            cam2 = self.attn.relprop(cam2, **kwargs)
            return self.clone1.relprop((cam1, cam2), **kwargs)

        def relprop_cls_only(self, cam_cls, **kwargs):
            alpha = kwargs.get("alpha", 1)
            var = self.add2.variant
            cls = lambda t: t[:, :1]
            dfr = ops.USE_DEFERRED_ADD
            c1, c2 = ops.add_relprop(cam_cls, cls(self.add2.X[0]), cls(self.add2.X[1]), variant=var, deferred=dfr)
            c2 = R_ours.linear_rule(self.mlp.fc2, c2, alpha, cls, var)
            c2 = R_ours.linear_rule(self.mlp.fc1, c2, alpha, cls, var)
            cam = ops.clone_relprop((c1, c2), cls(self.clone2.X))
            c1, c2 = ops.add_relprop(cam, cls(self.add1.X[0]), cls(self.add1.X[1]), variant=var, deferred=dfr)
            c2 = R_ours.linear_rule(self.attn.proj, c2, alpha, cls, var)
            if isinstance(c1, ops.Deferred):
                c1 = c1.materialise()
            B, N, C = self.clone1.X.shape
            dense = torch.zeros((2, B, N, C), dtype=c2.dtype, device=c2.device)
            dense[0, :, 0] = c1[:, 0]
            dense[1, :, 0] = c2[:, 0]
            cam2 = self.attn.relprop_after_proj(dense[1], **kwargs)
            return self.clone1.relprop((dense[0], cam2), **kwargs)

    class PatchEmbed(nn.Module):
        def __init__(self, img_size=224, patch_size=16, in_chans=3, embed_dim=768):
            super().__init__()
            img_size = (img_size, img_size) if isinstance(img_size, int) else tuple(img_size)
            patch_size = (patch_size, patch_size) if isinstance(patch_size, int) else tuple(patch_size)
            self.img_size, self.patch_size = img_size, patch_size
            self.num_patches = (img_size[1] // patch_size[1]) * (img_size[0] // patch_size[0])
            self.proj = L.Conv2d(in_chans, embed_dim, kernel_size=patch_size, stride=patch_size)

        def forward(self, x):
            B, C, Hh, Ww = x.shape
            assert Hh == self.img_size[0] and Ww == self.img_size[1], \
                f"Input image size ({Hh}*{Ww}) doesn't match model ({self.img_size[0]}*{self.img_size[1]})."
            return self.proj(x).flatten(2).transpose(1, 2)

        def relprop(self, cam, **kwargs):
            cam = cam.unflatten(1, (self.img_size[0] // self.patch_size[0], self.img_size[1] // self.patch_size[1]))
            return self.proj.relprop(cam.permute(0, 3, 1, 2), **kwargs)

    class VisionTransformer(nn.Module):
        default_method = "transformer_attribution" if L.RelProp.variant == "ours" else "grad"

        def __init__(self, img_size=224, patch_size=16, in_chans=3, num_classes=1000, embed_dim=768, depth=12,
                     num_heads=12, mlp_ratio=4., qkv_bias=False, mlp_head=False, drop_rate=0., attn_drop_rate=0.,
                     block_norm_eps=1e-6, final_norm_eps=1e-5):
            super().__init__()
            self.num_classes = num_classes
            self.num_features = self.embed_dim = embed_dim
            self.patch_embed = PatchEmbed(img_size=img_size, patch_size=patch_size, in_chans=in_chans,
                                          embed_dim=embed_dim)
            num_patches = self.patch_embed.num_patches
            self.pos_embed = nn.Parameter(torch.zeros(1, num_patches + 1, embed_dim))
            self.cls_token = nn.Parameter(torch.zeros(1, 1, embed_dim))
            self.blocks = nn.ModuleList([
                Block(dim=embed_dim, num_heads=num_heads, mlp_ratio=mlp_ratio, qkv_bias=qkv_bias, drop=drop_rate,
                      attn_drop=attn_drop_rate, norm_eps=block_norm_eps) for _ in range(depth)])
            self.norm = L.LayerNorm(embed_dim, eps=final_norm_eps)
            self.head = Mlp(embed_dim, int(embed_dim * mlp_ratio), num_classes) if mlp_head \
                else L.Linear(embed_dim, num_classes)
            _trunc_normal_(self.pos_embed, std=.02)
            _trunc_normal_(self.cls_token, std=.02)
            self.apply(self._init_weights)
            self.pool = L.IndexSelect()
            self.add = L.Add()
            self.inp_grad = None
            self.exploit_cls_sparsity = True
            self.prune_below_start_layer = False
            self.register_buffer("_cls_index", torch.zeros((), dtype=torch.long), persistent=False)

        def save_inp_grad(self, grad): self.inp_grad = grad
        def get_inp_grad(self): return self.inp_grad

        def _init_weights(self, m):
            if isinstance(m, nn.Linear):
                _trunc_normal_(m.weight, std=.02)
                if m.bias is not None:
                    nn.init.constant_(m.bias, 0)
            elif isinstance(m, nn.LayerNorm):
                nn.init.constant_(m.bias, 0)
                nn.init.constant_(m.weight, 1.0)

        @property
        def no_weight_decay(self):
            return {'pos_embed', 'cls_token'}

        def forward(self, x, register_hook=False):
            B = x.shape[0]
            x = self.patch_embed(x)
            x = torch.cat((self.cls_token.expand(B, -1, -1), x), dim=1)
            x = self.add([x, self.pos_embed])
            if x.requires_grad:
                x.register_hook(self.save_inp_grad)
            for blk in self.blocks:
                x = blk(x)
            x = self.norm(x)
            x = self.pool(x, dim=1, indices=self._cls_index).squeeze(1)
            return self.head(x)

        def relprop(self, cam=None, method=None, is_ablation=False, start_layer=0, **kwargs):
            if method is None:
                method = self.default_method
            if method == "full" and ops._is_f64(cam):
                raise ops._lib.TeError(f"{ops.DTYPES_MSG}; method='full' (the z^B patch rule) is not implemented for "
                                       "torch.float64 relevance: run it on a float32 or bfloat16 model")
            prune = self.prune_below_start_layer and method in ("transformer_attribution", "grad")
            stop_at = self.blocks[start_layer].attn if prune else None
            if stop_at is not None:
                stop_at._stop_after_attn_cam = True
            try:
                cam = self.head.relprop(cam, **kwargs)
                if self.exploit_cls_sparsity and isinstance(self.head, nn.Linear):
                    cam = ops.index_select_relprop(cam.unsqueeze(1), self.pool.X[:, :1], 0)
                    cam = self.blocks[-1].relprop_cls_only(cam, **kwargs)
                    rest = list(self.blocks)[:-1]
                else:
                    cam = self.pool.relprop(cam.unsqueeze(1), **kwargs)
                    rest = list(self.blocks)
                for blk in reversed(rest):
                    cam = blk.relprop(cam, **kwargs)
            except L.StopRelprop:
                cam = None
            finally:
                if stop_at is not None:
                    stop_at._stop_after_attn_cam = False

            hook = getattr(self, "_before_tail", None)
            if hook is not None:
                hook()

            if method == "full":
                cam, _ = self.add.relprop(cam, **kwargs)
                cam = self.patch_embed.relprop(cam[:, 1:], **kwargs)
                return cam.sum(dim=1)

# ... 61 lines not shown
```

Measured before the change: 1035.

## Emit split bf16 operand planes directly from LayerNorm kernels for consuming linears

Adds LayerNorm forward and backward kernels that also write the 3xbf16 split planes, and their abs versions, that the next x6 linear layer would otherwise produce in a separate split pass. LayerNorm modules are wired to their consumer linears (qkv, fc1, BERT intermediate) and post the planes into that linear's cache. The split step and the extra reads of the activation it needed are dropped. A backward variant that hands gradient planes to the upstream linear is added but off by default behind an env flag. The plane-emitting forward uses an LDS tile transpose with block syncs and more registers per thread, which may lower occupancy.

Measured after the change: 1034. About the same (-0.1%).

```diff
diff --git a/include/te_relprop.h b/include/te_relprop.h
--- a/include/te_relprop.h
+++ b/include/te_relprop.h
@@ -240,6 +240,13 @@
                              int64_t T, int64_t C, float eps, te_stream_t stream);
 int te_layernorm_backward_f32(const float* dy, const float* x, const float* weight, const float* mean, const float* rstd,
                               const float* add, float* dx, int64_t T, int64_t C, te_stream_t stream);
+int te_layernorm_planes_supported(int64_t C);
+int te_layernorm_forward_x6_planes_f32(const float* x, const float* weight, const float* bias, float* y, float* mean,
+                                       float* rstd, int64_t T, int64_t C, float eps, void* planes, void* planes_abs,
+                                       size_t planes_bytes, te_stream_t stream);
+int te_layernorm_backward_x6_planes_f32(const float* dy, const float* x, const float* weight, const float* mean,
+                                        const float* rstd, const float* add, float* dx, int64_t T, int64_t C, void* planes,
+                                        size_t planes_bytes, te_stream_t stream);
 int te_gelu_forward_f32(const float* x, float* y, int64_t n, te_stream_t stream);
 int te_gelu_backward_f32(const float* dy, const float* x, float* dx, int64_t n, te_stream_t stream);
 
diff --git a/transformer-explainability_amd/_lib.py b/transformer-explainability_amd/_lib.py
--- a/transformer-explainability_amd/_lib.py
+++ b/transformer-explainability_amd/_lib.py
@@ -85,6 +85,9 @@
     "te_layernorm_supported": (_I, [_I64]),
     "te_layernorm_forward_f32": (_I, [_P, _P, _P, _P, _P, _P, _I64, _I64, _F, _P]),
     "te_layernorm_backward_f32": (_I, [_P, _P, _P, _P, _P, _P, _P, _I64, _I64, _P]),
+    "te_layernorm_planes_supported": (_I, [_I64]),
+    "te_layernorm_forward_x6_planes_f32": (_I, [_P, _P, _P, _P, _P, _P, _I64, _I64, _F, _P, _P, _SZ, _P]),
+    "te_layernorm_backward_x6_planes_f32": (_I, [_P, _P, _P, _P, _P, _P, _P, _I64, _I64, _P, _SZ, _P]),
     "te_gelu_forward_f32": (_I, [_P, _P, _I64, _P]),
     "te_gelu_backward_f32": (_I, [_P, _P, _P, _I64, _P]),
     "te_gelu_backward_x6_planes_f32": (_I, [_P, _P, _I64, _I64, _P, _SZ, _P]),
diff --git a/transformer-explainability_amd/bert.py b/transformer-explainability_amd/bert.py
--- a/transformer-explainability_amd/bert.py
+++ b/transformer-explainability_amd/bert.py
@@ -6,7 +6,7 @@
 import torch
 import torch.nn as nn
 
-from . import ops
+from . import ops, producers
 from . import rules as R_ours
 
 __all__ = ["BertConfigLite", "make_bert_module", "BertModel", "BertForSequenceClassification"]
@@ -196,7 +196,8 @@
             self.add = L.Add()
 
         def forward(self, hidden_states, input_tensor):
-            return self.LayerNorm(self.add([self.dropout(self.dense(hidden_states)), input_tensor]))
+            d = self.dropout(self.dense(hidden_states))
+            return self.LayerNorm(producers.carry_bwd_cache(d, self.add([d, input_tensor])))
 
         def relprop(self, cam, **kwargs):
             cam1, cam2 = self.add.relprop(cam, deferred=True, **kwargs)
@@ -240,7 +241,8 @@
             self.add = L.Add()
 
         def forward(self, hidden_states, input_tensor):
-            return self.LayerNorm(self.add([self.dropout(self.dense(hidden_states)), input_tensor]))
+            d = self.dropout(self.dense(hidden_states))
+            return self.LayerNorm(producers.carry_bwd_cache(d, self.add([d, input_tensor])))
 
         def relprop(self, cam, **kwargs):
             cam1, cam2 = self.add.relprop(cam, deferred=True, **kwargs)
@@ -256,6 +258,9 @@
             act = self.intermediate.intermediate_act_fn
             if hasattr(act, "feeds"):
                 act.feeds(self.output.dense)
+            norm = self.attention.output.LayerNorm
+            if hasattr(norm, "feeds"):
+                norm.feeds(self.intermediate.dense)
 
         def forward(self, hidden_states, attention_mask=None, head_mask=None, **unused):
             att = self.attention(hidden_states, attention_mask, head_mask)[0]
diff --git a/transformer-explainability_amd/csrc/te_linear_x6.hip b/transformer-explainability_amd/csrc/te_linear_x6.hip
--- a/transformer-explainability_amd/csrc/te_linear_x6.hip
+++ b/transformer-explainability_amd/csrc/te_linear_x6.hip
@@ -58,35 +58,12 @@
   unsigned p[8][3];
 #pragma unroll
   for (int e = 0; e < 8; ++e) split3_pk(apply_op<OP>(v[2 * e]), apply_op<OP>(v[2 * e + 1]), p[e]);
-  unsigned char* d = dst + ((rb * nks + ks) * group + sign * 3) * kFrag + r * 16;
-#pragma unroll
-  for (int q = 0; q < 3; ++q)
-#pragma unroll
-    for (int kh = 0; kh < 2; ++kh) {
-      u32x4 w;
-#pragma unroll
-      for (int e = 0; e < 4; ++e) w[e] = p[4 * kh + e][q];
-      *reinterpret_cast<u32x4*>(d + q * kFrag + kh * 512) = w;
-    }
+  store_step_planes(dst + ((rb * nks + ks) * group + sign * 3) * kFrag + r * 16, p);
   if constexpr (OP == OP_ID) {
     if (dst_abs) {
 #pragma unroll
-      for (int e = 0; e < 8; ++e) {
-        const unsigned m = p[e][0] & 0x80008000u;
-        p[e][0] &= 0x7fff7fffu;
-        p[e][1] ^= m & (((p[e][1] & 0x7fff7fffu) + 0x7fff7fffu) & 0x80008000u);
-        p[e][2] ^= m & (((p[e][2] & 0x7fff7fffu) + 0x7fff7fffu) & 0x80008000u);
-      }
-      unsigned char* da = dst_abs + ((rb * nks + ks) * 3) * kFrag + r * 16;
-#pragma unroll
-      for (int q = 0; q < 3; ++q)
-#pragma unroll
-        for (int kh = 0; kh < 2; ++kh) {
-          u32x4 w;
-#pragma unroll
-          for (int e = 0; e < 4; ++e) w[e] = p[4 * kh + e][q];
-          *reinterpret_cast<u32x4*>(da + q * kFrag + kh * 512) = w;
-        }
+      for (int e = 0; e < 8; ++e) abs_planes_pk(p[e]);
+      store_step_planes(dst_abs + ((rb * nks + ks) * 3) * kFrag + r * 16, p);
     }
   }
 }
@@ -136,27 +113,11 @@
   unsigned p[8][3];
 #pragma unroll
   for (int e = 0; e < 8; ++e) split3_pk(v[2 * e], v[2 * e + 1], p[e]);
-  auto store = [&](unsigned char* d) __attribute__((always_inline)) {
-#pragma unroll
-    for (int q = 0; q < 3; ++q)
-#pragma unroll
-      for (int kh = 0; kh < 2; ++kh) {
-        u32x4 w;
-#pragma unroll
-        for (int e = 0; e < 4; ++e) w[e] = p[4 * kh + e][q];
-        *reinterpret_cast<u32x4*>(d + q * kFrag + kh * 512) = w;
-      }
-  };
-  store(dst + ((rb * nks + ks) * 3) * kFrag + r * 16);
+  store_step_planes(dst + ((rb * nks + ks) * 3) * kFrag + r * 16, p);
   if constexpr (SRC == SRC_GELU_FWD) {
 #pragma unroll
-    for (int e = 0; e < 8; ++e) {
-      const unsigned m = p[e][0] & 0x80008000u;
-      p[e][0] &= 0x7fff7fffu;
-      p[e][1] ^= m & (((p[e][1] & 0x7fff7fffu) + 0x7fff7fffu) & 0x80008000u);
-      p[e][2] ^= m & (((p[e][2] & 0x7fff7fffu) + 0x7fff7fffu) & 0x80008000u);
-    }
-    store(dst_abs + ((rb * nks + ks) * 3) * kFrag + r * 16);
+    for (int e = 0; e < 8; ++e) abs_planes_pk(p[e]);
+    store_step_planes(dst_abs + ((rb * nks + ks) * 3) * kFrag + r * 16, p);
   }
 }
 
diff --git a/transformer-explainability_amd/csrc/te_norm_act.hip b/transformer-explainability_amd/csrc/te_norm_act.hip
--- a/transformer-explainability_amd/csrc/te_norm_act.hip
+++ b/transformer-explainability_amd/csrc/te_norm_act.hip
@@ -1,4 +1,4 @@
-#include "te_common.h"
+#include "te_x6.h"
 
 namespace {
 
@@ -10,6 +10,102 @@
 #pragma unroll
   for (int off = 32; off > 0; off >>= 1) v = v + __shfl_xor(v, off, 64);
   return v;
+}
+
+template <int NV>
+__device__ __forceinline__ void ln_load_row(const float* __restrict__ xr, int lane, int nc, f32x4 (&v)[NV]) {
+#pragma unroll
+  for (int i = 0; i < NV; ++i) {
+    const int c = lane + 64 * i;
+    v[i] = f32x4{0.f, 0.f, 0.f, 0.f};
+    if (c < nc) v[i] = *reinterpret_cast<const f32x4*>(xr + (c << 2));
+  }
+}
+
+template <int NV>
+__device__ __forceinline__ void ln_row_stats(const f32x4 (&v)[NV], int lane, int nc, int C, float eps, float& m, float& r) {
+  float s = 0.0f;
+#pragma unroll
+  for (int i = 0; i < NV; ++i) s = s + ((v[i][0] + v[i][1]) + (v[i][2] + v[i][3]));
+  m = wave_sum_all(s) / (float)C;
+  float q = 0.0f;
+#pragma unroll
+  for (int i = 0; i < NV; ++i) {
+    const int c = lane + 64 * i;
+    if (c < nc) {
+#pragma unroll
+      for (int e = 0; e < 4; ++e) {
+        const float d = v[i][e] - m;
+        q = q + d * d;
+      }
+    }
+  }
+  r = 1.0f / sqrtf(wave_sum_all(q) / (float)C + eps);
+}
+
+template <int NV>
+__device__ __forceinline__ void ln_row_out(f32x4 (&v)[NV], int lane, int nc, float m, float r, const float* __restrict__ w,
+                                           const float* __restrict__ b, float* __restrict__ yr) {
+#pragma unroll
+  for (int i = 0; i < NV; ++i) {
+    const int c = lane + 64 * i;
+    if (c < nc) {
+      const f32x4 wv = *reinterpret_cast<const f32x4*>(w + (c << 2));
+      const f32x4 bv = b ? *reinterpret_cast<const f32x4*>(b + (c << 2)) : f32x4{0.f, 0.f, 0.f, 0.f};
+      f32x4 o;
+#pragma unroll
+      for (int e = 0; e < 4; ++e) o[e] = ((v[i][e] - m) * r) * wv[e] + bv[e];
+      __builtin_nontemporal_store(o, reinterpret_cast<f32x4*>(yr + (c << 2)));
+      v[i] = o;
+    }
+  }
+}
+
+template <int NV>
+__device__ __forceinline__ void ln_bwd_load_row(const float* __restrict__ gr, const float* __restrict__ xr,
+                                                const float* __restrict__ w, int lane, int nc, float m, float r,
+                                                f32x4 (&a)[NV], f32x4 (&xh)[NV], float& s1, float& s2) {
+  s1 = 0.0f;
+  s2 = 0.0f;
+#pragma unroll
+  for (int i = 0; i < NV; ++i) {
+    const int c = lane + 64 * i;
+    a[i] = f32x4{0.f, 0.f, 0.f, 0.f};
+    xh[i] = f32x4{0.f, 0.f, 0.f, 0.f};
+    if (c < nc) {
+      const f32x4 g = __builtin_nontemporal_load(reinterpret_cast<const f32x4*>(gr + (c << 2)));
+      const f32x4 xv = __builtin_nontemporal_load(reinterpret_cast<const f32x4*>(xr + (c << 2)));
+      const f32x4 wv = *reinterpret_cast<const f32x4*>(w + (c << 2));
+#pragma unroll
+      for (int e = 0; e < 4; ++e) {
+        a[i][e] = g[e] * wv[e];
+        xh[i][e] = (xv[e] - m) * r;
+        s1 = s1 + a[i][e];
+        s2 = s2 + a[i][e] * xh[i][e];
+      }
+    }
+  }
+}
+
+template <int NV>
+__device__ __forceinline__ void ln_bwd_row_out(f32x4 (&a)[NV], const f32x4 (&xh)[NV], int lane, int nc, float r, float c1,
+                                               float c2, const float* __restrict__ ar, float* __restrict__ dr) {
+#pragma unroll
+  for (int i = 0; i < NV; ++i) {
+    const int c = lane + 64 * i;
+    if (c < nc) {
+      f32x4 o;
+#pragma unroll
+      for (int e = 0; e < 4; ++e) o[e] = r * ((a[i][e] - c1) - xh[i][e] * c2);
+      if (ar) {
+        const f32x4 av = __builtin_nontemporal_load(reinterpret_cast<const f32x4*>(ar + (c << 2)));
+#pragma unroll
+        for (int e = 0; e < 4; ++e) o[e] = av[e] + o[e];
+      }
+      __builtin_nontemporal_store(o, reinterpret_cast<f32x4*>(dr + (c << 2)));
+      a[i] = o;
+    }
+  }
 }
 
 template <int NV>
@@ -21,43 +117,11 @@
   const int64_t row = (int64_t)blockIdx.x * kRowsPerBlock + (threadIdx.x >> 6);
   if (row >= T) return;
   const int nc = C >> 2;
-  const float* xr = x + row * C;
   f32x4 v[NV];
-  float s = 0.0f;
-#pragma unroll
-  for (int i = 0; i < NV; ++i) {
-    const int c = lane + 64 * i;
-    v[i] = f32x4{0.f, 0.f, 0.f, 0.f};
-    if (c < nc) v[i] = *reinterpret_cast<const f32x4*>(xr + (c << 2));
-    s = s + ((v[i][0] + v[i][1]) + (v[i][2] + v[i][3]));
-  }
-  const float m = wave_sum_all(s) / (float)C;
-  float q = 0.0f;
-#pragma unroll
-  for (int i = 0; i < NV; ++i) {
-    const int c = lane + 64 * i;
-    if (c < nc) {
-#pragma unroll
-      for (int e = 0; e < 4; ++e) {
-        const float d = v[i][e] - m;
-        q = q + d * d;
-      }
-    }
-  }
-  const float r = 1.0f / sqrtf(wave_sum_all(q) / (float)C + eps);
-  float* yr = y + row * C;
-#pragma unroll
-  for (int i = 0; i < NV; ++i) {
-    const int c = lane + 64 * i;
-    if (c < nc) {
-      const f32x4 wv = *reinterpret_cast<const f32x4*>(w + (c << 2));
-      const f32x4 bv = b ? *reinterpret_cast<const f32x4*>(b + (c << 2)) : f32x4{0.f, 0.f, 0.f, 0.f};
-      f32x4 o;
-#pragma unroll
-      for (int e = 0; e < 4; ++e) o[e] = ((v[i][e] - m) * r) * wv[e] + bv[e];
-      __builtin_nontemporal_store(o, reinterpret_cast<f32x4*>(yr + (c << 2)));
-    }
-  }
+  ln_load_row<NV>(x + row * C, lane, nc, v);
+  float m, r;
+  ln_row_stats<NV>(v, lane, nc, C, eps, m, r);
+  ln_row_out<NV>(v, lane, nc, m, r, w, b, y + row * C);
   if (lane == 0) {
     mean[row] = m;
     rstd[row] = r;
@@ -74,45 +138,122 @@
   if (row >= T) return;
   const int nc = C >> 2;
   const float m = mean[row], r = rstd[row];
-  const float* xr = x + row * C;
-  const float* gr = dy + row * C;
   f32x4 a[NV], xh[NV];
-  float s1 = 0.0f, s2 = 0.0f;
-#pragma unroll
-  for (int i = 0; i < NV; ++i) {
-    const int c = lane + 64 * i;
-    a[i] = f32x4{0.f, 0.f, 0.f, 0.f};
-    xh[i] = f32x4{0.f, 0.f, 0.f, 0.f};
-    if (c < nc) {
-      const f32x4 g = __builtin_nontemporal_load(reinterpret_cast<const f32x4*>(gr + (c << 2)));
-      const f32x4 xv = __builtin_nontemporal_load(reinterpret_cast<const f32x4*>(xr + (c << 2)));
-      const f32x4 wv = *reinterpret_cast<const f32x4*>(w + (c << 2));
-#pragma unroll
-      for (int e = 0; e < 4; ++e) {
-        a[i][e] = g[e] * wv[e];
-        xh[i][e] = (xv[e] - m) * r;
-        s1 = s1 + a[i][e];
-        s2 = s2 + a[i][e] * xh[i][e];
-      }
-    }
-  }
+  float s1, s2;
+  ln_bwd_load_row<NV>(dy + row * C, x + row * C, w, lane, nc, m, r, a, xh, s1, s2);
   const float c1 = wave_sum_all(s1) / (float)C, c2 = wave_sum_all(s2) / (float)C;
-  float* dr = dx + row * C;
-#pragma unroll
-  for (int i = 0; i < NV; ++i) {
-    const int c = lane + 64 * i;
-    if (c < nc) {
-      f32x4 o;
-#pragma unroll
-      for (int e = 0; e < 4; ++e) o[e] = r * ((a[i][e] - c1) - xh[i][e] * c2);
-      if (add) {
-        const f32x4 av = __builtin_nontemporal_load(reinterpret_cast<const f32x4*>(add + row * C + (c << 2)));
-#pragma unroll
-        for (int e = 0; e < 4; ++e) o[e] = av[e] + o[e];
-      }
-      __builtin_nontemporal_store(o, reinterpret_cast<f32x4*>(dr + (c << 2)));
-    }
-  }
+  ln_bwd_row_out<NV>(a, xh, lane, nc, r, c1, c2, add ? add + row * C : nullptr, dx + row * C);
+}
+
+constexpr int kPlRows = 32;
+constexpr int kPlWaveRows = kPlRows / (kThreads / 64);
+constexpr int kPlPitch = 132;
+
+template <int NV, bool ABS>
+__device__ __forceinline__ void ln_emit_planes(const f32x4 (&vals)[kPlWaveRows][NV], float* __restrict__ tile, int64_t rb, int C,
+                                               unsigned char* __restrict__ dst, unsigned char* __restrict__ dst_abs) {
+  const int lane = threadIdx.x & 63, wave = threadIdx.x >> 6;
+  const int r = threadIdx.x & 31, sl = threadIdx.x >> 5;
+  const int nks = C >> 4, nslab = (nks + 7) >> 3;
+#pragma unroll
+  for (int s = 0; s < 2 * NV; ++s) {
+    if (s < nslab) {
+      if ((lane >> 5) == (s & 1)) {
+#pragma unroll
+        for (int j = 0; j < kPlWaveRows; ++j)
+          *reinterpret_cast<f32x4*>(&tile[(wave * kPlWaveRows + j) * kPlPitch + 4 * (lane & 31)]) = vals[j][s >> 1];
+      }
+      __syncthreads();
+      const int ks = s * 8 + sl;
+      if (ks < nks) {
+        float v[16];
+#pragma unroll
+        for (int c = 0; c < 4; ++c) {
+          const f32x4 q = *reinterpret_cast<const f32x4*>(&tile[r * kPlPitch + sl * 16 + 4 * c]);
+#pragma unroll
+          for (int e = 0; e < 4; ++e) v[4 * c + e] = q[e];
+        }
+        unsigned p[8][3];
+#pragma unroll
+        for (int e = 0; e < 8; ++e) split3_pk(v[2 * e], v[2 * e + 1], p[e]);
+        const int64_t at = ((rb * nks + ks) * 3) * kFrag + r * 16;
+        store_step_planes(dst + at, p);
+        if constexpr (ABS) {
+#pragma unroll
+          for (int e = 0; e < 8; ++e) abs_planes_pk(p[e]);
+          store_step_planes(dst_abs + at, p);
+        }
+      }
+      __syncthreads();
+    }
+  }
+}
+
+template <int NV>
+__global__ __launch_bounds__(kThreads) void ln_fwd_planes_kernel(const float* __restrict__ x, const float* __restrict__ w,
+                                                                 const float* __restrict__ b, float* __restrict__ y,
+                                                                 float* __restrict__ mean, float* __restrict__ rstd,
+                                                                 unsigned char* __restrict__ dst,
+                                                                 unsigned char* __restrict__ dst_abs, int64_t T, int C, float eps) {
+  __shared__ __attribute__((aligned(16))) float tile[kPlRows * kPlPitch];
+  const int lane = threadIdx.x & 63;
+  const int64_t rb = blockIdx.x;
+  const int64_t row0 = rb * kPlRows + (threadIdx.x >> 6) * kPlWaveRows;
+  const int nc = C >> 2;
+  f32x4 vals[kPlWaveRows][NV];
+#pragma unroll
+  for (int j = 0; j < kPlWaveRows; ++j) {
+    if (row0 + j < T) {
+      ln_load_row<NV>(x + (row0 + j) * C, lane, nc, vals[j]);
+    } else {
+#pragma unroll
+      for (int i = 0; i < NV; ++i) vals[j][i] = f32x4{0.f, 0.f, 0.f, 0.f};
+    }
+  }
+#pragma unroll
+  for (int j = 0; j < kPlWaveRows; ++j) {
+    const int64_t row = row0 + j;
+    if (row < T) {
+      float m, r;
+      ln_row_stats<NV>(vals[j], lane, nc, C, eps, m, r);
+      ln_row_out<NV>(vals[j], lane, nc, m, r, w, b, y + row * C);
+      if (lane == 0) {
+        mean[row] = m;
+        rstd[row] = r;
+      }
+    }
+  }
+  ln_emit_planes<NV, true>(vals, tile, rb, C, dst, dst_abs);
+}
+
+template <int NV>
+__global__ __launch_bounds__(kThreads) void ln_bwd_planes_kernel(const float* __restrict__ dy, const float* __restrict__ x,
+                                                                 const float* __restrict__ w, const float* __restrict__ mean,
+                                                                 const float* __restrict__ rstd, const float* __restrict__ add,
+                                                                 float* __restrict__ dx, unsigned char* __restrict__ dst,
+                                                                 int64_t T, int C) {
+  __shared__ __attribute__((aligned(16))) float tile[kPlRows * kPlPitch];
+  const int lane = threadIdx.x & 63;
+  const int64_t rb = blockIdx.x;
+  const int64_t row0 = rb * kPlRows + (threadIdx.x >> 6) * kPlWaveRows;
+  const int nc = C >> 2;
+  f32x4 vals[kPlWaveRows][NV];
+#pragma unroll
+  for (int j = 0; j < kPlWaveRows; ++j) {
+    const int64_t row = row0 + j;
+    if (row < T) {
+      const float m = mean[row], r = rstd[row];
+      f32x4 xh[NV];
+      float s1, s2;
+      ln_bwd_load_row<NV>(dy + row * C, x + row * C, w, lane, nc, m, r, vals[j], xh, s1, s2);
+      const float c1 = wave_sum_all(s1) / (float)C, c2 = wave_sum_all(s2) / (float)C;
+      ln_bwd_row_out<NV>(vals[j], xh, lane, nc, r, c1, c2, add ? add + row * C : nullptr, dx + row * C);
+    } else {
+#pragma unroll
+      for (int i = 0; i < NV; ++i) vals[j][i] = f32x4{0.f, 0.f, 0.f, 0.f};
+    }
+  }
+  ln_emit_planes<NV, false>(vals, tile, rb, C, dst, nullptr);
 }
 
 __global__ __launch_bounds__(kThreads) void gelu_fwd_kernel(const float* __restrict__ x, float* __restrict__ y, int64_t n4) {
@@ -188,6 +329,45 @@
   return TE_OK;
 }
 
+extern "C" int te_layernorm_planes_supported(int64_t C) { return (te_layernorm_supported(C) && C % 16 == 0) ? 1 : 0; }
+
+static size_t ln_planes_bytes(int64_t T, int64_t C) { return (size_t)te_ceil_div(T, (int64_t)kPlRows) * kPlRows * (size_t)C * 6; }
+
+extern "C" int te_layernorm_forward_x6_planes_f32(const float* x, const float* weight, const float* bias, float* y, float* mean,
+                                                  float* rstd, int64_t T, int64_t C, float eps, void* planes, void* planes_abs,
+                                                  size_t planes_bytes_, te_stream_t stream_) {
+  if (!x || !weight || !y || !mean || !rstd || !planes || !planes_abs || T <= 0) return TE_ERR_INVALID_ARG;
+  if (!te_layernorm_planes_supported(C) || te_ceil_div(T, (int64_t)kPlRows) > 0x7fffffff) return TE_ERR_UNSUPPORTED;
+  if (!te_aligned16(x) || !te_aligned16(weight) || !te_aligned16(y) || (bias && !te_aligned16(bias))) return TE_ERR_UNSUPPORTED;
+  if (planes_bytes_ < ln_planes_bytes(T, C) || !te_aligned16(planes) || !te_aligned16(planes_abs)) return TE_ERR_WORKSPACE;
+  const dim3 grid((unsigned)te_ceil_div(T, (int64_t)kPlRows)), blk(kThreads);
+  const int rc = for_chunks(C, [&](auto nv) {
+    ln_fwd_planes_kernel<decltype(nv)::value><<<grid, blk, 0, (hipStream_t)stream_>>>(
+        x, weight, bias, y, mean, rstd, (unsigned char*)planes, (unsigned char*)planes_abs, T, (int)C, eps);
+  });
+  if (rc != TE_OK) return rc;
+  TE_RETURN_IF_LAUNCH_FAILED();
+  return TE_OK;
+}
+
+extern "C" int te_layernorm_backward_x6_planes_f32(const float* dy, const float* x, const float* weight, const float* mean,
+                                                   const float* rstd, const float* add, float* dx, int64_t T, int64_t C,
+                                                   void* planes, size_t planes_bytes_, te_stream_t stream_) {
+  if (!dy || !x || !weight || !mean || !rstd || !dx || !planes || T <= 0) return TE_ERR_INVALID_ARG;
+  if (!te_layernorm_planes_supported(C) || te_ceil_div(T, (int64_t)kPlRows) > 0x7fffffff) return TE_ERR_UNSUPPORTED;
+  if (!te_aligned16(dy) || !te_aligned16(x) || !te_aligned16(weight) || !te_aligned16(dx) || (add && !te_aligned16(add)))
+    return TE_ERR_UNSUPPORTED;
+  if (planes_bytes_ < ln_planes_bytes(T, C) || !te_aligned16(planes)) return TE_ERR_WORKSPACE;
+  const dim3 grid((unsigned)te_ceil_div(T, (int64_t)kPlRows)), blk(kThreads);
+  const int rc = for_chunks(C, [&](auto nv) {
+    ln_bwd_planes_kernel<decltype(nv)::value><<<grid, blk, 0, (hipStream_t)stream_>>>(dy, x, weight, mean, rstd, add, dx,
+                                                                                     (unsigned char*)planes, T, (int)C);
+  });
+  if (rc != TE_OK) return rc;
+  TE_RETURN_IF_LAUNCH_FAILED();
+  return TE_OK;
+}
+
 extern "C" int te_gelu_forward_f32(const float* x, float* y, int64_t n, te_stream_t stream_) {
   if (!x || !y || n <= 0) return TE_ERR_INVALID_ARG;
   if (n % 4 || !te_aligned16(x) || !te_aligned16(y) || n / 4 / kThreads > 0x7ffffffe) return TE_ERR_UNSUPPORTED;
diff --git a/transformer-explainability_amd/csrc/te_x6.h b/transformer-explainability_amd/csrc/te_x6.h
--- a/transformer-explainability_amd/csrc/te_x6.h
+++ b/transformer-explainability_amd/csrc/te_x6.h
@@ -27,6 +27,24 @@
   for (int t2 = 0; t2 < 4; ++t2) split3_pk(x[2 * t2], x[2 * t2 + 1], pk[t2]);
 #pragma unroll
   for (int q = 0; q < 3; ++q) b[q] = __builtin_bit_cast(bf16x8, u32x4{pk[0][q], pk[1][q], pk[2][q], pk[3][q]});
+}
+
+__device__ __forceinline__ void abs_planes_pk(unsigned (&p)[3]) {
+  const unsigned m = p[0] & 0x80008000u;
+  p[0] &= 0x7fff7fffu;
+  p[1] ^= m & (((p[1] & 0x7fff7fffu) + 0x7fff7fffu) & 0x80008000u);
+  p[2] ^= m & (((p[2] & 0x7fff7fffu) + 0x7fff7fffu) & 0x80008000u);
+}
+__device__ __forceinline__ void store_step_planes(unsigned char* d, const unsigned (&p)[8][3]) {
+#pragma unroll
+  for (int q = 0; q < 3; ++q)
+#pragma unroll
+    for (int kh = 0; kh < 2; ++kh) {
+      u32x4 w;
+#pragma unroll
+      for (int e = 0; e < 4; ++e) w[e] = p[4 * kh + e][q];
+      *reinterpret_cast<u32x4*>(d + q * kFrag + kh * 512) = w;
+    }
 }
 
 constexpr int PA[6] = {1, 0, 2, 0, 1, 0}, PB[6] = {1, 2, 0, 1, 0, 0};
diff --git a/transformer-explainability_amd/ops.py b/transformer-explainability_amd/ops.py
--- a/transformer-explainability_amd/ops.py
+++ b/transformer-explainability_amd/ops.py
@@ -350,6 +350,21 @@
     hit = cache.pop("dy_planes_from_consumer", None)
     if hit is not None and dy.data_ptr() == hit[0].data_ptr() and tuple(dy.shape) == hit[1] and not any(dy.stride()):
         return hit[2]
+    return None
+
+
+def _dy_key(dy: Tensor):
+    return (dy.data_ptr(), dy._version, tuple(dy.shape), str(dy.device))
+
+
+def post_dy_tensor_planes(cache: dict, dy: Tensor, planes: Tensor):
+    cache["dy_planes_of_tensor"] = (_dy_key(dy), planes, dy)
+
+
+def take_dy_tensor_planes(cache: dict, dy: Tensor) -> Optional[Tensor]:
+    hit = cache.pop("dy_planes_of_tensor", None)
+    if hit is not None and hit[0] == _dy_key(dy) and dy.is_contiguous():
+        return hit[1]
     return None
 
 
@@ -822,6 +837,47 @@
     return dx
 
 
+X6_PRODUCER_PLANES = os.environ.get("TE_X6_PRODUCER_PLANES", "1") not in ("", "0")
+X6_LN_BACKWARD_PLANES = os.environ.get("TE_X6_LN_BACKWARD_PLANES", "0") not in ("", "0")
+
+
+def layernorm_planes_supported(x: Tensor) -> bool:
+    return bool(X6_PRODUCER_PLANES and layernorm_supported(x)
+                and _lib.load().te_layernorm_planes_supported(int(x.shape[-1])))
+
+
+def layernorm_forward_planes(x: Tensor, weight: Tensor, bias: Optional[Tensor], eps: float):
+    x = _c(x)
+    C = x.shape[-1]
+    T = x.numel() // C
+    y = torch.empty_like(x)
+    mean = torch.empty((T,), dtype=torch.float32, device=x.device)
+    rstd = torch.empty((T,), dtype=torch.float32, device=x.device)
+    with _on_device(x) as lib, _timed("layernorm_forward", 0.0, (4.0 * 2 + 12.0) * T * C):
+        nb = lib.te_linear_x6_planes_bytes(T, C)
+        xs, xa = _ws(nb, x), _ws(nb, x)
+        _lib.check(lib.te_layernorm_forward_x6_planes_f32(_ptr(x), _ptr(_c(weight)), _ptr(_c(bias)) if bias is not None else None,
+                                                          _ptr(y), _ptr(mean), _ptr(rstd), T, C, float(eps), _ptr(xs), _ptr(xa),
+                                                          nb, _stream(x)), "te_layernorm_forward_x6_planes_f32")
+    return y, mean, rstd, xs, xa
+
+
+def layernorm_backward_planes(dy: Tensor, x: Tensor, weight: Tensor, mean: Tensor, rstd: Tensor,
+                              add: Optional[Tensor] = None):
+    dy, x = _c(dy), _c(x)
+    C = x.shape[-1]
+    T = x.numel() // C
+    dx = torch.empty_like(x)
+    with _on_device(x) as lib, _timed("layernorm_backward", 0.0, (4.0 * (3 + (add is not None)) + 6.0) * T * C):
+        nb = lib.te_linear_x6_planes_bytes(T, C)
+        planes = _ws(nb, x)
+        _lib.check(lib.te_layernorm_backward_x6_planes_f32(_ptr(dy), _ptr(x), _ptr(_c(weight)), _ptr(mean), _ptr(rstd),
+                                                           _ptr(_c(add)) if add is not None else None, _ptr(dx), T, C,
+                                                           _ptr(planes), nb, _stream(x)),
+                   "te_layernorm_backward_x6_planes_f32")
+    return dx, planes
+
+
 def gelu_forward(x: Tensor) -> Tensor:
     x = _c(x)
     y = torch.empty_like(x)
diff --git a/transformer-explainability_amd/producers.py b/transformer-explainability_amd/producers.py
--- a/transformer-explainability_amd/producers.py
+++ b/transformer-explainability_amd/producers.py
@@ -19,33 +19,48 @@
             and tuple(norm.normalized_shape) == (x.shape[-1],))
 
 
+def _ln_forward(ctx, x, weight, bias, eps, feeds, source):
+    if feeds is not None:
+        y, mean, rstd, xs, xa = ops.layernorm_forward_planes(x, weight, bias, eps)
+        ops.post_x_planes(feeds, y, xs, xa)
+    else:
+        y, mean, rstd = ops.layernorm_forward(x, weight, bias, eps)
+    ctx.save_for_backward(x, weight, mean, rstd)
+    ctx.source = source
+    return y
+
+
+def _ln_backward(ctx, dy, add=None):
+    x, weight, mean, rstd = ctx.saved_tensors
+    if ctx.source is not None:
+        dx, planes = ops.layernorm_backward_planes(dy, x, weight, mean, rstd, add=add)
+        ops.post_dy_tensor_planes(ctx.source, dx, planes)
+        return dx
+    return ops.layernorm_backward(dy, x, weight, mean, rstd, add=add)
+
+
 class _LayerNorm(torch.autograd.Function):
     @staticmethod
-    def forward(ctx, x, weight, bias, eps):
-        y, mean, rstd = ops.layernorm_forward(x, weight, bias, eps)
-        ctx.save_for_backward(x, weight, mean, rstd)
-        return y
+    def forward(ctx, x, weight, bias, eps, feeds=None, source=None):
+        return _ln_forward(ctx, x, weight, bias, eps, feeds, source)
 
     @staticmethod
     def backward(ctx, dy):
-        x, weight, mean, rstd = ctx.saved_tensors
-        return ops.layernorm_backward(dy, x, weight, mean, rstd), None, None, None
+        return _ln_backward(ctx, dy), None, None, None, None, None
 
 
 class _ResidualLayerNorm(torch.autograd.Function):
 
     @staticmethod
-    def forward(ctx, x, weight, bias, eps):
-        y, mean, rstd = ops.layernorm_forward(x, weight, bias, eps)
-        ctx.save_for_backward(x, weight, mean, rstd)
+    def forward(ctx, x, weight, bias, eps, feeds=None, source=None):
+        y = _ln_forward(ctx, x, weight, bias, eps, feeds, source)
         return x.view_as(x), y
 
     @staticmethod
     def backward(ctx, d_bypass, dy):
-        x, weight, mean, rstd = ctx.saved_tensors
         if dy is None:
-            return d_bypass, None, None, None
-        return ops.layernorm_backward(dy, x, weight, mean, rstd, add=d_bypass), None, None, None
+            return d_bypass, None, None, None, None, None
+        return _ln_backward(ctx, dy, add=d_bypass), None, None, None, None, None
 
 
 class _Gelu(torch.autograd.Function):
@@ -82,8 +97,13 @@
     def backward(ctx, dy):
         w = ctx.weight
         if ctx.bwd_x6:
+            planes = ops.take_dy_planes(ctx.cache, dy)
+            if planes is None:
+                planes = ops.take_dy_tensor_planes(ctx.cache, dy)
+            else:
+                ctx.cache.pop("dy_planes_of_tensor", None)
             dx = ops.gemm_x6(dy, ops.x6_matrix_planes(w, True, ctx.cache), None, w.shape[1], "linear_backward_x6",
-                             x_planes=ops.take_dy_planes(ctx.cache, dy))
+                             x_planes=planes)
         else:
             dx = torch.matmul(dy, w)
         return dx, None, None, None, None, None
@@ -115,12 +135,37 @@
     return out
 
 
+def carry_bwd_cache(src, dst):
+    c = getattr(src, "_te_bwd_x6_cache", None)
+    if c is not None:
+        dst._te_bwd_x6_cache = c
+    return dst
+
+
+def _norm_plane_routes(x, norm):
+    feeds = source = None
+    from .rules import Linear, x6_cache
+    consumer = norm.__dict__.get("_te_feeds", (None,))[0]
+    if not isinstance(consumer, Linear):
+        consumer = None
+    consumer_cache = x6_cache(consumer) if consumer is not None else None
+    if ops.layernorm_planes_supported(x):
+        C = x.shape[-1]
+        if consumer is not None and takes_producer_planes(consumer, x.numel() // C, C):
+            feeds = consumer_cache
+        if ops.X6_LN_BACKWARD_PLANES:
+            source = getattr(x, "_te_bwd_x6_cache", None)
+    if feeds is None and consumer_cache is not None:
+        ops.drop_x_planes(consumer_cache)
+    return feeds, source
+
+
 def layer_norm(x, norm):
-    return _LayerNorm.apply(x, _d(norm.weight), _d(norm.bias), norm.eps)
+    return _LayerNorm.apply(x, _d(norm.weight), _d(norm.bias), norm.eps, *_norm_plane_routes(x, norm))
 
 
 def residual_layer_norm(x, norm):
-    return _ResidualLayerNorm.apply(x, _d(norm.weight), _d(norm.bias), norm.eps)
+    return _ResidualLayerNorm.apply(x, _d(norm.weight), _d(norm.bias), norm.eps, *_norm_plane_routes(x, norm))
 
 
 def gelu(x, consumer=None, consumer_cache=None):
diff --git a/transformer-explainability_amd/rules.py b/transformer-explainability_amd/rules.py
--- a/transformer-explainability_amd/rules.py
+++ b/transformer-explainability_amd/rules.py
@@ -86,6 +86,10 @@
 
 
 class LayerNorm(nn.LayerNorm, RelProp):
+    def feeds(self, linear):
+        self.__dict__["_te_feeds"] = (linear,)
+        return self
+
     def forward(self, x):
         from . import producers
         if producers.norm_usable(x, self):
diff --git a/transformer-explainability_amd/vit.py b/transformer-explainability_amd/vit.py
--- a/transformer-explainability_amd/vit.py
+++ b/transformer-explainability_amd/vit.py
@@ -221,12 +221,17 @@
             self.add2 = L.Add()
             self.clone1 = L.Clone()
             self.clone2 = L.Clone()
+            if hasattr(self.norm1, "feeds"):
+                self.norm1.feeds(self.attn.qkv)
+                self.norm2.feeds(self.mlp.fc1)
 
         def forward(self, x):
             x1, n = self._clone_norm(self.clone1, self.norm1, x)
-            x = self.add1([x1, self.attn(n)])
+            a = self.attn(n)
+            x = producers.carry_bwd_cache(a, self.add1([x1, a]))
             x1, n = self._clone_norm(self.clone2, self.norm2, x)
-            return self.add2([x1, self.mlp(n)])
+            m = self.mlp(n)
+            return producers.carry_bwd_cache(m, self.add2([x1, m]))
 
         @staticmethod
         def _clone_norm(clone, norm, x):
```
